# disanda/Deep-GAN-Encoders

Measured on AMD Instinct MI355X. Metric: encoder-train images/sec (E_align_s2 step, StyleGAN2 FFHQ-1024), higher is better.
Workload: dtype bf16; 1 GPU; E_align_s2 two-phase step, StyleGAN2-1024 G (train mode) + BE(startf=16, L=9) + LPIPS-VGG16 (seeded stand-in weights), batch 8/GPU; global_batch=8, img_size=1024, parallelism=dp1

## Files before the change

### deep-gan-encoders_amd/_lib.py

```python
import ctypes as C
import os

_HERE = os.path.dirname(os.path.abspath(__file__))
LIB_PATH = os.environ.get("DGE_LIB_PATH", os.path.join(_HERE, "libdge_hip.so"))


class DgeError(RuntimeError):
    pass


class ConvDesc(C.Structure):
    _fields_ = [
        ("x", C.c_void_p), ("w_packed", C.c_void_p), ("y", C.c_void_p), ("addend", C.c_void_p), ("dot_src", C.c_void_p),
        ("in_scale", C.c_void_p), ("in_shift", C.c_void_p), ("out_scale", C.c_void_p),
        ("bias", C.c_void_p), ("noise", C.c_void_p), ("noise_w", C.c_void_p), ("stats", C.c_void_p),
        ("B", C.c_int), ("H", C.c_int), ("W", C.c_int), ("Cin", C.c_int), ("Cout", C.c_int),
        ("ksize", C.c_int), ("up", C.c_int), ("in_s2d", C.c_int), ("noise_batch", C.c_int), ("noise_w_per_channel", C.c_int),
        ("act", C.c_int), ("bias_scale", C.c_float), ("gain", C.c_float), ("add_scale", C.c_float),
        ("dtype", C.c_int), ("in_up2", C.c_int), ("in_relu", C.c_int), ("stats_slots", C.c_int), ("w_layout", C.c_int),
        ("prep", C.c_int), ("prep_gain", C.c_float), ("prep_noise", C.c_void_p), ("prep_ns", C.c_void_p), ("prep_noise_batch", C.c_int),
        ("prep_stats", C.c_void_p), ("mask_relu", C.c_int), ("in_t2d", C.c_int),
        ("rgb_w", C.c_void_p), ("rgb_style", C.c_void_p), ("rgb_bias", C.c_void_p), ("rgb_out", C.c_void_p), ("rgb_wscale", C.c_float),
        ("rgb_skip_y", C.c_int), ("pool_out", C.c_int), ("pool_mask", C.c_void_p),
        ("prefetch_w", C.c_void_p), ("prefetch_ntot", C.c_int), ("prefetch_cin", C.c_int), ("in_bwd_coef", C.c_void_p),
        ("in_bwd_extra", C.c_void_p), ("in_bwd_extra_scale", C.c_float), ("fr_img4", C.c_void_p), ("fr_out", C.c_void_p),
    ]


class ConvPPDesc(C.Structure):
    _fields_ = [
        ("x", C.c_void_p), ("w_pp", C.c_void_p), ("y", C.c_void_p), ("w_bstride", C.c_longlong),
        ("out_scale", C.c_void_p), ("bias", C.c_void_p), ("noise", C.c_void_p), ("noise_w", C.c_void_p),
        ("B", C.c_int), ("H", C.c_int), ("W", C.c_int), ("Cin", C.c_int), ("Cout", C.c_int),
        ("noise_batch", C.c_int), ("noise_w_per_channel", C.c_int), ("act", C.c_int), ("bias_scale", C.c_float), ("gain", C.c_float),
        ("dgrad", C.c_int), ("in_s2d", C.c_int), ("stats_slots", C.c_int), ("prep", C.c_int), ("prep_noise_batch", C.c_int), ("mask_relu", C.c_int),
        ("in_t2d", C.c_int), ("add_scale", C.c_float), ("prep_gain", C.c_float),
        ("dot_src", C.c_void_p), ("addend", C.c_void_p), ("stats", C.c_void_p), ("prep_stats", C.c_void_p), ("prep_noise", C.c_void_p), ("prep_ns", C.c_void_p),
    ]


class DenseLayer(C.Structure):
    _fields_ = [("w", C.c_void_p), ("bias", C.c_void_p), ("I", C.c_int), ("O", C.c_int), ("wscale", C.c_float), ("bscale", C.c_float),
                ("add", C.c_float), ("act", C.c_int), ("gain", C.c_float)]


class S2GradEntry(C.Structure):
    _fields_ = [("P", C.c_void_p), ("st", C.c_void_p), ("d", C.c_void_p), ("s", C.c_void_p), ("bias", C.c_void_p), ("wsq", C.c_void_p),
                ("gs", C.c_void_p), ("wstyle", C.c_void_p),
                ("nslot_p", C.c_int), ("nslot_s", C.c_int), ("in_c", C.c_int), ("out_c", C.c_int), ("row", C.c_int), ("bscale", C.c_float)]


class SumPlanarEntry(C.Structure):
    _fields_ = [("partial", C.c_void_p), ("out", C.c_void_p), ("nslot", C.c_int), ("C", C.c_int), ("NS", C.c_int), ("pad", C.c_int)]


_P, _I, _F = C.c_void_p, C.c_int, C.c_float
SIGNATURES = {
    "dge_conv2d": [C.POINTER(ConvDesc), _P],
    "dge_fir_t2d": [_P, _P, _P, _I, _I, _I, _I, _I, _P],
    "dge_s2_style_grads": [C.POINTER(S2GradEntry), _I, _P, _I, _I, _I, _F, _P],
    "dge_conv_small_supported": [_I, _I, _I, _I, _I, _I, _I, _I],
    "dge_torgb_bwd_prep": [_P, _P, _P, _P, _P, _P, _I, _P, _P, _P, _I, _I, _I, _F, _F, _I, _P],
    "dge_demod_bwd_prep": [_P, _I, _P, _P, _P, _I, _I, _F, _P],
    "dge_sum_slots": [_P, _P, _I, _I, _I, _P],
    "dge_sum_slots_planar": [_P, _P, _I, _I, _I, _P],
    "dge_set_deterministic": [_I],
    "dge_get_deterministic": [],
    "dge_packed_n": [_I],
    "dge_pack_conv_weight": [_P, _P, _I, _I, _I, _I, _I, _F, _P],
    "dge_pack_conv_weights_multi": [_P, _P, _I, _I, _P],
    "dge_pack_desc_bytes": [],
    "dge_weight_sumsq": [_P, _P, _I, _I, _I, _F, _P],
    "dge_linear": [_P, _I, _P, _P, _P, _I, _I, _I, _I, _F, _F, _F, _I, _F, _I, _P],
    "dge_pixelnorm": [_P, _P, _I, _I, _F, _P],
    "dge_truncation": [_P, _P, _P, _I, _I, _I, _F, _I, _I, _P],
    "dge_torgb": [_P, _P, _P, _P, _P, _P, _I, _I, _I, _I, _F, _I, _P],
    "dge_conv_rgb_supported": [_I, _I, _I, _I, _I, _I, _I],
    "dge_conv_in_bwd_supported": [_I, _I, _I, _I, _I, _I, _I],
    "dge_conv_in_bwd_fromrgb_supported": [_I, _I, _I, _I, _I, _I, _I],
    "dge_conv_in_bwd_x_supported": [_I, _I, _I, _I, _I, _I, _I],
    "dge_conv_pool_supported": [_I, _I, _I, _I, _I, _I, _I],
    "dge_rgb_upsample_add": [_P, _P, _I, _I, _I, _P],
    "dge_nchw_to_nhwc": [_P, _P, _I, _I, _I, _I, _I, _P],
    "dge_nhwc_to_nchw": [_P, _P, _I, _I, _I, _I, _P],
    "dge_fromrgb": [_P, _P, _P, _P, _P, _I, _I, _I, _I, _P],
    "dge_fromrgb2": [_P, _P, _P, _P, _P, _P, _I, _I, _I, _I, _P],
    "dge_stats_finalize": [_P, _P, _P, _P, _I, _I, _I, _F, _P],
    "dge_stats_finalize_slots": [_P, _I, _P, _P, _P, _I, _I, _I, _F, _P],
    "dge_blend": [_P, _P, _P, _P, _P, _P, _I, _I, _I, _I, _I, _F, _F, _I, _P],
    "dge_loss_reduce": [_P, _P, _P, _I, _I, _I, _I, _I, _I, _I, _I, _P],
    "dge_crop_pool": [_P, _P, _I, _I, _I, _I, _I, _I, _I, _I, _P],
    "dge_ssim_fwd": [_P, _P, _P, _P, _I, _I, _I, _P],
    "dge_ssim_box7": [_P, _P, _P, _I, _I, _I, _F, _F, _F, _P],
    "dge_ssim_bwd": [_P, _P, _P, _P, _I, _I, _I, _F, _I, _P],
    "dge_space_loss_finalize": [_P, _P, _P, _P, _F, _F, _I, _P],
    "dge_space_loss_bwd": [_P, _P, _P, _P, _P, _I, _I, _I, _I, _I, _I, _I, _I, _F, _F, _I, _P],
    "dge_axpy_scalar": [_P, _P, _P, C.c_long, _F, _I, _P],
    "dge_lreq_adam_multi": [_I, _P, _P, _P, _P, _P, _F, _F, _P, _P, _P],
    "dge_modconv_bwd_prep": [_P, _P, _P, _P, _P, _P, _I, _I, _I, _I, _F, _I, _P],
    "dge_demod_bwd": [_P, _P, _P, _P, _P, _I, _I, _F, _P],
    "dge_linear_t": [_P, _I, _I, _P, _P, _P, _I, _I, _I, _I, _I, _F, _I, _P],
    "dge_torgb_bwd": [_P, _P, _P, _P, _P, _P, _I, _I, _I, _F, _I, _P],
    "dge_up2_bwd": [_P, _P, _I, _I, _I, _P],
    "dge_conv_wgrad": [_P, _P, _P, _P, _P, _I, _I, _I, _I, _I, _I, _I, _P],
    "dge_act_bwd": [_P, _P, _P, _P, _P, _I, _I, _I, _I, _I, _I, _F, _F, _I, _P],
    "dge_in_bwd_coef": [_P, _P, _P, _P, _P, _P, _I, _I, _I, _P],
    "dge_in_bwd_coef_slots": [_P, _I, _P, _P, _P, _P, _P, _I, _I, _I, _P],
    "dge_in_bwd": [_P, _P, _P, _P, _P, _P, _P, _I, _I, _I, _I, _I, _F, _I, _I, _P],
    "dge_chan_sum": [_P, _P, _I, _I, _I, _F, _I, _P],
    "dge_fromrgb_bwd": [_P, _P, _P, _P, _I, _I, _I, _I, _P],
    "dge_head_entry_size": [],
    "dge_heads_bwd": [_P, _I, _I, _P, _I, _P, _P, _P, _P, _I, _I, _P],
    "dge_dense_wgrad": [_P, _I, _P, _I, _P, _P, _I, _I, _I, _I, _P],
    "dge_lpips_prep": [_P, _P, _I, _I, _I, _P, _P, _I, _P],
    "dge_lpips_prep_bwd": [_P, _P, _I, _I, _I, _P, _F, _I, _I, _P],
    "dge_maxpool2": [_P, _P, _I, _I, _I, _I, _I, _P],
    "dge_maxpool2_bwd": [_P, _P, _P, _P, _I, _I, _I, _I, _I, _P],
    "dge_lpips_head": [_P, _P, _P, _P, _I, _I, _I, _F, _I, _P],
    "dge_mean": [_P, _P, _I, _P],
    "dge_blur_noise_act": [_P, _P, _P, _P, _P, _P, _I, _I, _I, _I, _I, _I, _I, _I, _P],
    "dge_affine_compose": [_P, _P, _P, _P, _P, _I, _I, _P],
    "dge_lerp_layers": [_P, _P, _I, _P, _P, _I, _I, _I, _P],
    "dge_linear_rows": [_P, _I, _P, _P, _P, _P, _P, _P, _I, _I, _I, _F, _F, _F, _P],
    "dge_demod_rows": [_P, _P, _P, _P, _P, _P, _P, _P, _I, _I, _F, _P],
    "dge_fromrgb_dgrad": [_P, _P, _P, _P, _I, _I, _I, _I, _P],
    "dge_nearest_up2": [_P, _P, _I, _I, _I, _I, _F, _I, _P],
    "dge_sg1_in_bwd_coef": [_P, _P, _P, _P, _P, _P, _I, _I, _I, _P],
    "dge_dot_stats": [_P, _P, _P, _I, _I, _I, _I, _P],
    "dge_nearest_up2_bwd": [_P, _P, _P, _P, _I, _I, _I, _I, _I, _P],
    "dge_pixelnorm_nhwc": [_P, _P, C.c_long, _I, _F, _I, _P],
    "dge_pixelnorm_nhwc_bwd": [_P, _P, _P, C.c_long, _I, _F, _I, _P],
    "dge_affine_relu_bwd": [_P, _P, _P, _P, _P, _P, _I, _I, _I, _I, _P],
    "dge_slice_up_bwd": [_P, _P, _I, _I, _I, _I, _I, _I, _I, _P],
    "dge_softmax_rows": [_P, C.c_long, _I, _I, _P],
    "dge_softmax_rows_bwd": [_P, _P, C.c_long, _I, _I, _P],
    "dge_rgb_tanh_bwd": [_P, _P, _P, _I, _I, _I, _I, _P],
    "dge_sn_group": [_P, _I, _I, _I, _P, _F, _I, _P],
    "dge_sn_entry_size": [],
    "dge_cbn_sn_wgrad_entry_size": [],
    "dge_cbn_sn_wgrad_group": [_P, _I, C.c_longlong, _I, _P, _I, _I, _P, _P],
    "dge_upconv_supported": [_I, _I, _I],
    "dge_pack_upconv_weight": [_P, _P, _I, _I, _F, _I, _P],
    "dge_upconv_fir": [_P, _P, _P, _P, _P, _P, _I, _P, _I, _P, _F, _F, _I, _I, _I, _I, _I, _I, _I, _P],
    "dge_cbn_affine": [_P, _P, _I, _P, _P, _F, _P, _P, _I, _I, _P],
    "dge_slice_up": [_P, _P, _I, _I, _I, _I, _I, _I, _I, _P],
    "dge_attention": [_P, _P, _P, _P, _I, _I, _I, _I, _I, _I, _P],
    "dge_rgb_tanh": [_P, _P, _I, _I, _I, _I, _P],
    "dge_guided_relu_bwd": [_P, _P, _P, C.c_long, _I, _I, _P],
    "dge_maxpool2_relu_bwd": [_P, _P, _P, _I, _I, _I, _I, _I, _I, _P],
    "dge_maxpool2_bwd_relu": [_P, _P, _P, _P, _I, _I, _I, _I, _I, _P],
    "dge_adaptive_pool7": [_P, _P, _I, _I, _I, _I, _I, _P],
    "dge_adaptive_pool7_bwd": [_P, _P, _I, _I, _I, _I, _I, _P],
    "dge_class_target": [_P, _P, _P, _P, _I, _I, _P],
    "dge_gather_row": [_P, _P, _P, _I, _I, _F, _P],
    "dge_campp_map": [_P, _P, _P, _P, _P, _I, _I, _I, _I, _I, _P],
    "dge_cam_resize": [_P, _P, _P, _I, _I, _I, _I, _I, _P],
    "dge_mask2cam_blocks": [_I],
    "dge_mask2cam": [_P, _P, _P, _P, _P, _P, _P, _I, _I, _P],
    "dge_randn": [_P, _I, _P, _P, _P, _P, C.c_ulonglong, _P, _P],
    "dge_version": [],
# ... 59 lines not shown
```

### deep-gan-encoders_amd/autograd_s2.py

```python
import math

import torch

from . import ops
from .stylegan2_generator import _dt
from .weight_cache import lookup, store, version


def _layer_fwd(L, x, w_row, randomize_noise):
    dt = ops.dtype_of(x)
    packed, wsq = L._prepared(dt)
    s = L.style(w_row)
    d = ops.linear(s, wsq, None, 1.0, 1.0, L.eps, ops.LIN_RSQRT, 1.0, square_input=True)
    if randomize_noise:
        noise = ops.randn((x.shape[0], L.res, L.res), x.device)
    else:
        noise = L.noise.reshape(1, L.res, L.res)
    y = ops.conv2d(x, packed, L.out_c, 3, up=L.up, in_scale=s, out_scale=d, bias=L.bias, bias_scale=L.bscale,
                   noise=noise, noise_w=L.noise_strength.detach().reshape(1), act=L.act, gain=L.gain)
    return y, s, d, noise


def _style_tables(mod, B, dt):
    nl = mod.num_layers
    groups = [(getattr(mod, f"layer{i}"), i) for i in range(nl - 1)] + [(getattr(mod, f"output{k}"), 2 * k + 1) for k in range(nl // 2)]
    key = (B, str(dt)) + tuple(version(p) for L, _ in groups for p in (L.style.weight, L.style.bias, L.weight))
    hit = mod.__dict__.get("_style_tab")
    if hit is not None and hit[0] == key:
        return hit[1]
    dev = groups[0][0].weight.device
    K = mod.w_space_dim
    Wc = torch.cat([L.style.weight.detach() for L, _ in groups]).contiguous()
    bc = torch.cat([L.style.bias.detach() for L, _ in groups]).contiguous()
    xoff, ybase, ybs, s_off = [], [], [], []
    off = 0
    for L, row in groups:
        C = L.in_c
        s_off.append(B * off)
        xoff += [row * K] * C
        ybase += [B * off + c for c in range(C)]
        ybs += [C] * C
        off += C
    woff, sbase, cin, dbase, dbs, d_off, wsq = [], [], [], [], [], [], []
    doff, wpos = 0, 0
    for gi, (L, _) in enumerate(groups[:nl - 1]):
        _, wq = L._prepared(dt)
        wsq.append(wq.reshape(-1))
        d_off.append(B * doff)
        for o in range(L.out_c):
            woff.append(wpos + o * L.in_c); sbase.append(s_off[gi]); cin.append(L.in_c)
            dbase.append(B * doff + o); dbs.append(L.out_c)
        doff += L.out_c
        wpos += L.out_c * L.in_c
    i32 = lambda v: torch.tensor(v, dtype=torch.int32, device=dev)
    st0 = groups[0][0].style
    for L, _ in groups:
        assert L.style.wscale == st0.wscale and L.style.bscale == st0.bscale and L.style.additional_bias == st0.additional_bias
    tab = dict(groups=groups, Wc=Wc, bc=bc, xoff=i32(xoff), ybase=i32(ybase), ybs=i32(ybs), s_off=s_off, s_total=B * off,
               wsq=torch.cat(wsq).contiguous(), woff=i32(woff), sbase=i32(sbase), cin=i32(cin), dbase=i32(dbase), dbs=i32(dbs),
               d_off=d_off, d_total=B * doff, wscale=st0.wscale, bscale=st0.bscale, add=st0.additional_bias, eps=groups[0][0].eps)
    mod.__dict__["_style_tab"] = (key, tab)
    return tab


def synthesis_run(mod, wp, randomize_noise=False, save=False):
    dt = _dt(mod.compute_dtype)
    B = wp.shape[0]
    results = {"wp": wp}
    nl = mod.num_layers
    tab = _style_tables(mod, B, dt)
    wpc = wp if (wp.dtype == torch.float32 and wp.is_contiguous()) else wp.float().contiguous()
    s_all = torch.empty(tab["s_total"], dtype=torch.float32, device=wp.device)
    ops.linear_rows(wpc, nl * mod.w_space_dim, tab["xoff"], tab["Wc"], tab["bc"], s_all, tab["ybase"], tab["ybs"], B,
                    tab["wscale"], tab["bscale"], tab["add"])
    d_all = torch.empty(tab["d_total"], dtype=torch.float32, device=wp.device)
    ops.demod_rows(s_all, tab["wsq"], tab["woff"], tab["sbase"], tab["cin"], d_all, tab["dbase"], tab["dbs"], B, tab["eps"])
    s_of = lambda g, C: s_all[tab["s_off"][g]:tab["s_off"][g] + B * C].view(B, C)
    x = ops.nchw_to_nhwc(mod.early_layer.const.detach(), B, dt)
    saved = {"const": x, "layers": [], "rgb": []} if save else None
    image = None
    for i in range(nl - 1):
        L = getattr(mod, f"layer{i}")
        s = s_of(i, L.in_c)
        d = d_all[tab["d_off"][i]:tab["d_off"][i] + B * L.out_c].view(B, L.out_c)
        if randomize_noise:
            noise = ops.randn((x.shape[0], L.res, L.res), x.device)
        else:
            noise = L.noise.reshape(1, L.res, L.res)
        fuse_rgb = (i % 2 == 0 and image is not None and not L.up and L.bias is not None and
                    ops.conv_rgb_supported(B, L.res, L.res, L.in_c, L.out_c, 3, dt))
        rgb = None
        if fuse_rgb:
            O_ = getattr(mod, f"output{i // 2}")
            srgb = s_of(nl - 1 + i // 2, O_.in_c)
            rgb = dict(w=O_.weight.detach().reshape(3, -1), style=srgb, bias=O_.bias.detach(), wscale=O_.wscale,
                       out=torch.empty((B, 3, L.res, L.res), dtype=torch.float32, device=x.device), skip_y=(not save) and i == nl - 2)
        y = L.conv(x, s, d, noise, dt, rgb=rgb)
        results[f"style{i:02d}"] = s
        if save:
            saved["layers"].append(dict(y=y, s=s, d=d, noise=noise))
        x = y
        if fuse_rgb:
            image = ops.rgb_upsample_add(rgb["out"], image)
            results[f"output_style{i // 2}"] = srgb
            if save:
                saved["rgb"].append(dict(s=srgb))
        elif i % 2 == 0:
            O_ = getattr(mod, f"output{i // 2}")
            srgb = s_of(nl - 1 + i // 2, O_.in_c)
            image = ops.torgb(x, O_.weight, srgb, O_.bias, image, O_.wscale)
            results[f"output_style{i // 2}"] = srgb
            if save:
                saved["rgb"].append(dict(s=srgb))
    results["image"] = image
    return results, saved


def _up_phase_form(L):
    import os
    return L.up and 32 <= L.res // 2 <= 128 and L.in_c >= 64 and L.in_c % 32 == 0 and L.out_c % 8 == 0 and not os.environ.get("DGE_NO_T2D")


def _dgrad_weight(L, dtype):
    hg = L.res // 2 if L.up else L.res
    if _up_phase_form(L):
        mode = ops.PACK_UPT2D_DGRAD
    else:
        mode = ops.pack_mode_for(L.weight, ops.PACK_UPFOLD_DGRAD if L.up else ops.PACK_DGRAD, hg, hg, dtype)
    c = lookup(L._cache, ("dg", dtype, mode), L.weight)
    return c if c is not None else store(L._cache, ("dg", dtype, mode), L.weight, ops.pack_conv_weight(L.weight, mode, dtype, L.wscale))


def _pp_dgrad(L, B, hg, dtype):
    import os
    K = 4 * L.out_c if L.up else L.out_c
    return (not L.up or L.out_c % 32 == 0) and ops.conv_pp_supported(B, hg, hg, K, L.in_c, dtype) and not os.environ.get("DGE_NO_PP_DG")


def _dgrad_weight_pp(L, d, t2d=False):
    if not L.up:
        return ops.pack_conv_pp(L.weight, L.wscale, in_scale=d, dgrad=True)
    name = "dgpp_t2d" if t2d else "dgpp"
    c = lookup(L._cache, name, L.weight)
    if c is None:
        rows = ops.pack_conv_weight(L.weight, ops.PACK_UPT2D_DGRAD if t2d else ops.PACK_UPFOLD_DGRAD, ops.F32, L.wscale)
        c = store(L._cache, name, L.weight, ops.pack_conv_pp_rows(rows, L.in_c, t2d=True) if t2d else rows)
    return c if t2d else ops.pack_conv_pp_rows(c, L.in_c, in_scale=d, in_period=L.out_c)


def synthesis_backward(mod, wp, saved, g_image):
    B = wp.shape[0]
    dev = wp.device
    nl = mod.num_layers
    g_wp = ops.zeros((B, nl, mod.w_space_dim), dev)
    layers = saved["layers"]
    dt = ops.dtype_of(saved["const"])
    g_img = g_image.float().contiguous()
    fused = not ops.is_deterministic()
    top = nl - 2
    Lt, Ot = getattr(mod, f"layer{top}"), getattr(mod, f"output{top // 2}")
    P = None
    if fused:
        g_x, g_srgb, P = ops.torgb_bwd_prep(g_img, layers[top]["y"], Ot.weight.detach().reshape(3, -1), saved["rgb"][top // 2]["s"], Ot.wscale,
                                            layers[top]["noise"], Lt.noise_strength.detach().reshape(1), Lt.gain)
    else:
        g_x, g_srgb = ops.torgb_bwd(g_img, layers[top]["y"], Ot.weight.detach().reshape(3, -1), saved["rgb"][top // 2]["s"], Ot.wscale)
    blocks = [] if fused else None
    if fused:
        blocks.append(dict(gs=g_srgb, wstyle=Ot.style.weight.detach(), row=top + 1))
    else:
        ops.linear_t(g_srgb, Ot.style.weight.detach(), g_wp[:, top + 1], scale=Ot.style.wscale, accumulate=True)
    if top // 2 > 0:
        g_img = ops.up2_bwd(g_img)
    for i in range(top, -1, -1):
        L = getattr(mod, f"layer{i}")
        rec = layers[i]
        if P is not None:
            g_y, d_in = g_x, rec["d"]
        else:
            R = ops.zeros((B, L.out_c, 3), dev)
            g_y, d_in = ops.modconv_bwd_prep(g_x, rec["y"], rec["d"], rec["noise"], L.gain, R), None
        x_in = saved["const"] if i == 0 else layers[i - 1]["y"]
        addend = None
        if i >= 1 and (i - 1) % 2 == 0:
            kp = (i - 1) // 2
            Op = getattr(mod, f"output{kp}")
            addend, g_srgb = ops.torgb_bwd(g_img, x_in, Op.weight.detach().reshape(3, -1), saved["rgb"][kp]["s"], Op.wscale)
            if fused:
                blocks.append(dict(gs=g_srgb, wstyle=Op.style.weight.detach(), row=i))
            else:
                ops.linear_t(g_srgb, Op.style.weight.detach(), g_wp[:, i], scale=Op.style.wscale, accumulate=True)
            if kp > 0:
                g_img = ops.up2_bwd(g_img)
        st = ops.SlotStats(B, L.in_c, dev) if fused else ops.zeros((B, L.in_c, 2), dev)
        prep, P_next = None, None
        t2d = _up_phase_form(L)
        if fused and i >= 1 and (t2d or not (L.up and L.in_c < 128)):
            Lp = getattr(mod, f"layer{i - 1}")
            P_next = ops.SlotStats(B, L.in_c, dev)
            prep = dict(gain=Lp.gain, noise=layers[i - 1]["noise"], ns=Lp.noise_strength.detach().reshape(1), stats=P_next)
        hg = L.res // 2 if L.up else L.res
        if fused and d_in is not None and not t2d and _pp_dgrad(L, B, hg, dt):
            g_xprev = ops.conv_pp(g_y, _dgrad_weight_pp(L, d_in), L.in_c, dgrad=True, in_s2d=L.up, out_scale=rec["s"], addend=addend,
                                  add_scale=1.0, stats=st, dot_src=x_in, prep=prep)
        elif t2d and fused and prep is not None and _pp_dgrad(L, B, hg, dt):
            g_xprev = ops.conv_pp(ops.fir_t2d(g_y, d_in), _dgrad_weight_pp(L, None, t2d=True), L.in_c, dgrad=True, in_t2d=True, out_scale=rec["s"],
                                  addend=addend, add_scale=1.0, stats=st, dot_src=x_in, prep=prep)
        elif t2d:
            g_xprev = ops.conv2d(ops.fir_t2d(g_y, d_in), _dgrad_weight(L, dt), L.in_c, 3, in_t2d=True, out_scale=rec["s"], addend=addend,
                                 add_scale=1.0, stats=st, dot_src=x_in, prep=prep)
        else:
            g_xprev = ops.conv2d(g_y, _dgrad_weight(L, dt), L.in_c, 3, in_s2d=L.up, in_scale=d_in, out_scale=rec["s"], addend=addend,
                                 add_scale=1.0, stats=st, dot_src=x_in, prep=prep)
        _, wsq = L._prepared(dt)
        if fused and P is not None:
            blocks.append(dict(P=P, st=st, d=rec["d"], s=rec["s"], bias=L.bias.detach(), wsq=wsq, bscale=L.bscale,
                               wstyle=L.style.weight.detach(), row=i))
            g_x, P = g_xprev, P_next
            continue
        if fused:
            st_t = ops.zeros((B, L.in_c, 2), dev)
            ops.check(ops.lib().dge_sum_slots(ops._p(st.buf), ops._p(st_t), st.nslot, st_t.numel(), 0, ops._stream()), "dge_sum_slots")
            st = st_t
        if P is not None:
            t = ops.demod_bwd_prep(P, rec["d"], L.bias.detach(), L.bscale)
        else:
            t = ops.demod_bwd(R, rec["d"], L.bias.detach(), L.noise_strength.detach().reshape(1), L.bscale)
        gs_view = st.view(B, -1)
        ops.linear_t(t, wsq, gs_view, mul=rec["s"], accumulate=True, incy=2, ldy=2 * L.in_c)
        ops.linear_t(gs_view, L.style.weight.detach(), g_wp[:, i], scale=L.style.wscale, accumulate=True, incx=2,
                     ldx=2 * L.in_c, O=L.in_c)
        g_x, P = g_xprev, P_next
    if blocks:
        ops.s2_style_grads(blocks, g_wp, getattr(mod, "layer0").style.wscale)
    return g_wp


class SynthesisFunction(torch.autograd.Function):
    @staticmethod
    def forward(ctx, mod, wp, randomize_noise):
        need = ctx.needs_input_grad[1]
        results, saved = synthesis_run(mod, wp.detach(), randomize_noise, save=need)
        ctx.mod, ctx.saved_acts, ctx.wp = mod, saved, wp.detach()
        ctx.keys = [k for k in results if k not in ("wp", "image")]
        outs = [results[k] for k in ctx.keys]
        ctx.mark_non_differentiable(*outs)
        return (results["image"], *outs)

    @staticmethod
    def backward(ctx, g_image, *unused):
        if ctx.saved_acts is None:
            raise RuntimeError("synthesis was run without saved activations")
        g_wp = synthesis_backward(ctx.mod, ctx.wp, ctx.saved_acts, g_image)
        return None, g_wp, None


def synthesis_forward(mod, wp, randomize_noise=False):
    wp = wp if (wp.dtype == torch.float32 and wp.is_contiguous()) else wp.float().contiguous()
    if wp.requires_grad and torch.is_grad_enabled():
        outs = SynthesisFunction.apply(mod, wp, randomize_noise)
        keys = [f"style{i:02d}" for i in range(mod.num_layers - 1)]
        results = {"wp": wp}
        names = []
        for i in range(mod.num_layers - 1):
            names.append(f"style{i:02d}")
            if i % 2 == 0:
                names.append(f"output_style{i // 2}")
        for n, t in zip(names, outs[1:]):
            results[n] = t
        results["image"] = outs[0]
        return results
    results, _ = synthesis_run(mod, wp, randomize_noise, save=False)
    return results
```

### deep-gan-encoders_amd/csrc/capi.hip

```cpp
#include <stdarg.h>
#include <stdio.h>
#include "common.h"
#include "conv_params.h"
#include "../../include/dge_hip.h"

static thread_local char g_err[512] = "";
void dge_set_error(const char* fmt, ...) {
    va_list ap; va_start(ap, fmt); vsnprintf(g_err, sizeof(g_err), fmt, ap); va_end(ap);
}
extern "C" const char* dge_last_error(void) { return g_err; }
static thread_local char g_kernel[160] = "";
void dge_note_kernel(const char* fmt, ...) {
    va_list ap; va_start(ap, fmt); vsnprintf(g_kernel, sizeof(g_kernel), fmt, ap); va_end(ap);
}
extern "C" const char* dge_last_kernel(void) { return g_kernel; }
extern "C" int dge_version(void) { return 100; }

#include <vector>
static std::vector<void (*)(const DgeDet*)>& det_setters() { static std::vector<void (*)(const DgeDet*)> v; return v; }
void dge_det_register(void (*setter)(const DgeDet*)) { det_setters().push_back(setter); }
static DgeDet g_det_host = {0, nullptr, nullptr, 0, 0};
int dge_det_upload_failed = 0;
bool dge_det_fits(long long ndomains, long long nslots, long long L) {
    return !g_det_host.enabled || (ndomains * nslots * L <= g_det_host.ws_floats && ndomains <= (long long)g_det_host.ncounters);
// ... 17 lines not shown
}
extern "C" int dge_get_deterministic(void) { return g_det_host.enabled; }

static DgeEnv g_env;
static bool g_env_loaded = false;
static int env_int(const char* name, int dflt) { const char* e = getenv(name); return e ? atoi(e) : dflt; }
static void env_load() {
    g_env.force_stream = getenv("DGE_FORCE_STREAM") ? 1 : 0;
    g_env.no_stream = getenv("DGE_NO_STREAM") ? 1 : 0;
    g_env.no_pw = getenv("DGE_NO_PW") ? 1 : 0;
    g_env.stream_nseg = env_int("DGE_STREAM_NSEG", 0);
    g_env.conv_dbg = env_int("DGE_CONV_DBG", 0);
    g_env.conv_bn = env_int("DGE_CONV_BN", 0);
    g_env.conv_kc = env_int("DGE_CONV_KC", 0);
    g_env.conv_small = env_int("DGE_CONV_SMALL", -1);
    g_env.conv_nok4 = getenv("DGE_CONV_NOK4") ? 1 : 0;
    g_env.conv_nok2 = getenv("DGE_CONV_NOK2") ? 1 : 0;
    g_env.torgb_thread = getenv("DGE_TORGB_THREAD") ? 1 : 0;
    g_env.wgrad_th8 = getenv("DGE_WGRAD_TH8") ? 1 : 0;
    g_env.wgrad_groups = env_int("DGE_WGRAD_GROUPS", 0);
    if (g_env.wgrad_groups < 0) g_env.wgrad_groups = 0;
    g_env.up_dbg = env_int("DGE_UP_DBG", 0);
    { const char* v = getenv("DGE_UP_VARIANT"); g_env.up_variant = !v ? 0 : (v[0] == 's' ? 2 : 1); }
    g_env_loaded = true;
}
#include <mutex>
static std::once_flag g_env_once;
const DgeEnv& dge_env() { std::call_once(g_env_once, [] { if (!g_env_loaded) env_load(); }); return g_env; }
extern "C" void dge_env_reload(void) { env_load(); }

extern "C" int dge_conv2d(const dge_conv_desc* d, hipStream_t s) {
    DGE_CHECK(d && d->x && d->w_packed && d->y, "conv2d: null tensor");
    DGE_CHECK(d->B > 0 && d->H > 0 && d->W > 0 && d->Cin > 0 && d->Cout > 0, "conv2d: bad shape");
    DGE_CHECK(d->dtype == DGE_F32 || d->dtype == DGE_BF16, "conv2d: bad dtype %d", d->dtype);
    DGE_CHECK(!(d->up && d->stats), "conv2d: stats are not available in up mode");
    DGE_CHECK(!(d->up && d->in_s2d), "conv2d: up and in_s2d are exclusive");
    DGE_CHECK(!d->in_up2 || (!d->in_s2d && d->H % 2 == 0 && d->W % 2 == 0), "conv2d: in_up2 needs even H, W and no in_s2d");
    DGE_CHECK(!d->in_s2d || d->Cin % 4 == 0, "conv2d: in_s2d needs Cin %% 4 == 0");
    DGE_CHECK(!d->dot_src || d->stats || d->mask_relu || d->in_bwd_coef, "conv2d: dot_src needs a stats buffer");
    DGE_CHECK(!d->mask_relu || (d->dot_src && !d->prep && !d->up), "conv2d: mask_relu needs dot_src and excludes prep / up");
    DGE_CHECK(!d->in_relu || d->in_scale || d->in_shift, "conv2d: in_relu is applied together with the prologue affine");
    DGE_CHECK(d->gain > 0.f, "conv2d: gain must be positive (it is folded through the activation)");
    DGE_CHECK((((uintptr_t)d->in_scale | (uintptr_t)d->in_shift) & 15) == 0, "conv2d: in_scale/in_shift must be 16-byte aligned");
    DGE_CHECK(!d->noise || d->noise_w, "conv2d: noise without noise_w");
    ConvParams p;
    p.x = d->x; p.w = d->w_packed; p.y = d->y; p.addend = d->addend; p.dot_src = d->dot_src;
    p.in_scale = d->in_scale; p.in_shift = d->in_shift; p.out_scale = d->out_scale;
    p.bias = d->bias; p.noise = d->noise; p.noise_w = d->noise_w; p.stats = d->stats;
    p.B = d->B; p.H = d->H; p.W = d->W; p.Cin = d->Cin; p.Cout = d->Cout;
    p.Ntot_valid = d->up ? 4 * d->Cout : d->Cout;
    p.Ntot = dge_packed_n(p.Ntot_valid);
    p.up = d->up; p.in_s2d = d->in_s2d; p.in_up2 = d->in_up2; p.in_relu = d->in_relu;
    const int OH = d->up ? 2 * d->H : d->H, OW = d->up ? 2 * d->W : d->W;
    p.noise_bstride = d->noise_batch > 1 ? OH * OW : 0;
    p.noise_w_stride = d->noise_w_per_channel ? 1 : 0;
    p.act = d->act; p.bias_scale = d->bias_scale; p.gain = d->gain; p.add_scale = d->add_scale;
    p.tiles_x = p.tiles_y = 0;
    p.w_frag = d->w_layout == 1 ? 1 : 0;
    p.prep = d->prep ? 1 : 0;
    p.mask_relu = d->mask_relu ? 1 : 0;
    p.in_t2d = d->in_t2d ? 1 : 0;
    DGE_CHECK(!d->in_t2d || (d->ksize == 3 && !d->up && !d->in_s2d && !d->in_up2 && !d->in_scale && !d->in_shift && d->w_layout == 0),
              "conv2d: in_t2d is a plain 3x3 launch (no other read mode, no prologue affine, row-major weights)");
    p.prep_gain = d->prep_gain; p.prep_noise = d->prep_noise; p.prep_ns = d->prep_ns; p.prep_stats = d->prep_stats;
    p.prep_noise_bstride = d->prep_noise_batch > 1 ? OH * OW : 0;
    DGE_CHECK(!d->prep || (d->dot_src && d->prep_stats && d->prep_gain > 0.f && !d->up), "conv2d: prep needs dot_src, prep_stats, a positive prep_gain and no up mode");
    DGE_CHECK(!d->prep || !dge_get_deterministic(), "conv2d: the fused tail backward (prep) is not offered in deterministic mode; run dge_modconv_bwd_prep");
    DGE_CHECK(d->w_layout == 0 || d->w_layout == 1, "conv2d: bad w_layout %d", d->w_layout);
    p.stats_slots = d->stats_slots > 0 ? d->stats_slots : 1;
    p.rgb_w = d->rgb_out ? d->rgb_w : nullptr; p.rgb_style = d->rgb_style; p.rgb_bias = d->rgb_bias; p.rgb_out = d->rgb_out;
    p.rgb_wscale = d->rgb_wscale; p.rgb_skip_y = (d->rgb_out && d->rgb_skip_y) ? 1 : 0;
    p.pool_out = d->pool_out ? 1 : 0; p.pool_mask = d->pool_out ? (unsigned*)d->pool_mask : nullptr;
    const bool pf = d->w_layout == 1 && d->prefetch_w && d->prefetch_ntot >= 64 && d->prefetch_ntot % 64 == 0 &&
                    (d->prefetch_cin == 512 || d->prefetch_cin == 256);
    p.pf_w = pf ? d->prefetch_w : nullptr; p.pf_ntot = pf ? d->prefetch_ntot : 0; p.pf_cin = pf ? d->prefetch_cin : 0;
    p.in_coef = d->in_bwd_coef;
    p.in_extra = d->in_bwd_coef ? d->in_bwd_extra : nullptr; p.in_extra_scale = d->in_bwd_extra_scale;
    p.fr_img4 = d->in_bwd_coef ? d->fr_img4 : nullptr; p.fr_out = d->in_bwd_coef ? d->fr_out : nullptr;
    if (d->in_bwd_coef) {
        DGE_CHECK(!dge_get_deterministic(), "conv2d: in_bwd_coef is not offered in deterministic mode; run dge_in_bwd");
        DGE_CHECK(d->ksize == 3 && !d->up && dge_conv_stream_eligible(p, d->dtype, d->ksize), "conv2d: in_bwd_coef is offered where "
                  "dge_conv_in_bwd_supported() says so, with dot_src and prep_stats, without stats / prep");
    }
    if (d->pool_out)
        DGE_CHECK(!d->up && dge_conv_pool_ok(p, d->dtype, d->ksize), "conv2d: the pooled epilogue is offered where dge_conv_pool_supported() "
                  "says so (conv_2 of the first encoder blocks on the streaming kernel)");
    if (d->rgb_out) {
        DGE_CHECK(d->rgb_w && d->rgb_style && d->rgb_bias, "conv2d: rgb_out needs rgb_w, rgb_style, rgb_bias");
        DGE_CHECK(dge_conv_rgb_ok(p, d->dtype, d->ksize), "conv2d: the fused toRGB is offered where dge_conv_rgb_supported() says so "
                  "(bf16 3x3 32 -> 32 launches of the streaming kernel)");
    }
    return dge_conv_launch(p, d->dtype, d->ksize, s);
}

extern "C" int dge_conv_pool_supported(int B, int H, int W, int Cin, int Cout, int ksize, int dtype) {
    ConvParams p = {};
    p.B = B; p.H = H; p.W = W; p.Cin = Cin; p.Cout = Cout; p.Ntot_valid = Cout; p.Ntot = dge_packed_n(Cout);
    p.in_shift = (const float*)16; p.noise_w_stride = 1;
    return dge_conv_pool_ok(p, dtype, ksize) ? 1 : 0;
}

extern "C" int dge_conv_in_bwd_supported(int B, int H, int W, int Cin, int Cout, int ksize, int dtype) {
    ConvParams p = {};
    p.B = B; p.H = H; p.W = W; p.Cin = Cin; p.Cout = Cout; p.Ntot_valid = Cout; p.Ntot = dge_packed_n(Cout);
    p.dot_src = (const void*)16; p.prep_stats = (float*)16; p.in_coef = (const float*)16;
    return (ksize == 3 && !dge_get_deterministic() && dge_conv_stream_eligible(p, dtype, ksize)) ? 1 : 0;
}
extern "C" int dge_conv_in_bwd_x_supported(int B, int H, int W, int Cin, int Cout, int ksize, int dtype) {
    ConvParams p = {};
    p.B = B; p.H = H; p.W = W; p.Cin = Cin; p.Cout = Cout; p.Ntot_valid = Cout; p.Ntot = dge_packed_n(Cout);
    p.dot_src = (const void*)16; p.in_coef = (const float*)16;
    return (ksize == 3 && !dge_get_deterministic() && dge_conv_stream_eligible(p, dtype, ksize)) ? 1 : 0;
}
extern "C" int dge_conv_in_bwd_fromrgb_supported(int B, int H, int W, int Cin, int Cout, int ksize, int dtype) {
    ConvParams p = {};
    p.B = B; p.H = H; p.W = W; p.Cin = Cin; p.Cout = Cout; p.Ntot_valid = Cout; p.Ntot = dge_packed_n(Cout);
    p.dot_src = (const void*)16; p.in_coef = (const float*)16; p.fr_img4 = (const float*)16; p.fr_out = (float*)16;
    return (ksize == 3 && !dge_get_deterministic() && dge_conv_stream_eligible(p, dtype, ksize)) ? 1 : 0;
}

extern "C" int dge_conv_rgb_supported(int B, int H, int W, int Cin, int Cout, int ksize, int dtype) {
    ConvParams p = {};
    p.B = B; p.H = H; p.W = W; p.Cin = Cin; p.Cout = Cout; p.Ntot_valid = Cout; p.Ntot = dge_packed_n(Cout);
    return dge_conv_rgb_ok(p, dtype, ksize) ? 1 : 0;
}

__global__ void sum_slots_kernel(const float* __restrict__ partial, float* __restrict__ out, int nslot, int n, int accumulate) {
    const int i = blockIdx.x * blockDim.x + threadIdx.x;
    if (i >= n) return;
    float s = 0.f;
    int k = 0;
    for (; k + 8 <= nslot; k += 8) {
        float v[8];
#pragma unroll
        for (int j = 0; j < 8; j++) v[j] = partial[(size_t)(k + j) * n + i];
#pragma unroll
        for (int j = 0; j < 8; j++) s += v[j];
    }
    for (; k < nslot; k++) s += partial[(size_t)k * n + i];
    out[i] = accumulate ? out[i] + s : s;
}
__global__ void sum_slots_planar_kernel(const float* __restrict__ partial, float* __restrict__ out, int nslot, int C, int NS) {
    const int i = blockIdx.x * blockDim.x + threadIdx.x;
    if (i >= C * NS) return;
    float s = 0.f;
    int k = 0;
    for (; k + 8 <= nslot; k += 8) {
        float v[8];
#pragma unroll
        for (int j = 0; j < 8; j++) v[j] = partial[(size_t)(k + j) * C * NS + i];
#pragma unroll
        for (int j = 0; j < 8; j++) s += v[j];
    }
    for (; k < nslot; k++) s += partial[(size_t)k * C * NS + i];
    out[(size_t)(i % NS) * C + i / NS] = s;
}
extern "C" int dge_sum_slots_planar(const float* partial, float* out, int nslot, int C, int NS, hipStream_t s) {
    DGE_CHECK(nslot >= 1 && C >= 1 && NS >= 1, "sum_slots_planar: bad sizes");
    hipLaunchKernelGGL(sum_slots_planar_kernel, dim3((C * NS + 255) / 256), dim3(256), 0, s, partial, out, nslot, C, NS);
    DGE_LAUNCH_CHECK("sum_slots_planar");
    return 0;
}
struct SumPlanarTable { dge_sum_planar_entry e[32]; };
__global__ void sum_slots_planar_multi_kernel(SumPlanarTable tab) {
    const dge_sum_planar_entry e = tab.e[blockIdx.y];
    const int n = e.C * e.NS;
    for (int i = blockIdx.x * blockDim.x + threadIdx.x; i < n; i += gridDim.x * blockDim.x) {
        float s = 0.f;
        int k = 0;
        for (; k + 8 <= e.nslot; k += 8) {
            float v[8];
#pragma unroll
            for (int j = 0; j < 8; j++) v[j] = e.partial[(size_t)(k + j) * n + i];
#pragma unroll
            for (int j = 0; j < 8; j++) s += v[j];
        }
        for (; k < e.nslot; k++) s += e.partial[(size_t)k * n + i];
        e.out[(size_t)(i % e.NS) * e.C + i / e.NS] = s;
    }
}
extern "C" int dge_sum_slots_planar_multi(const dge_sum_planar_entry* entries, int n, hipStream_t s) {
    DGE_CHECK(entries && n >= 1 && n <= 32, "sum_slots_planar_multi: 1..32 entries");
    SumPlanarTable tab;
    int maxn = 1;
    for (int i = 0; i < n; i++) {
        const dge_sum_planar_entry& e = entries[i];
        DGE_CHECK(e.partial && e.out && e.nslot >= 1 && e.C >= 1 && e.NS >= 1, "sum_slots_planar_multi: bad entry %d", i);
        tab.e[i] = e;
        if (e.C * e.NS > maxn) maxn = e.C * e.NS;
    }
    hipLaunchKernelGGL(sum_slots_planar_multi_kernel, dim3((maxn + 255) / 256, n), dim3(256), 0, s, tab);
    DGE_LAUNCH_CHECK("sum_slots_planar_multi");
    return 0;
}
extern "C" int dge_sum_slots(const float* partial, float* out, int nslot, int n, int accumulate, hipStream_t s) {
    hipLaunchKernelGGL(sum_slots_kernel, dim3((n + 255) / 256), dim3(256), 0, s, partial, out, nslot, n, accumulate);
    DGE_LAUNCH_CHECK("sum_slots");
    return 0;
}
```

### deep-gan-encoders_amd/csrc/common.h

```cpp
#pragma once
#include <hip/hip_runtime.h>
#include <stdint.h>

typedef uint16_t bf16_t;
typedef __attribute__((ext_vector_type(8))) __bf16 bf16x8_t;
typedef __attribute__((ext_vector_type(16))) float f32x16_t;
typedef __attribute__((ext_vector_type(4))) float f32x4_t;

enum { DGE_F32 = 0, DGE_BF16 = 1 };
enum { DGE_ACT_NONE = 0, DGE_ACT_LRELU = 1, DGE_ACT_RELU = 2 };

__device__ __forceinline__ float bf2f(bf16_t h) { return __uint_as_float(((uint32_t)h) << 16); }
__device__ __forceinline__ bf16_t f2bf(float f) {
    uint32_t u = __float_as_uint(f);
    if ((u & 0x7fffffffu) > 0x7f800000u) return (bf16_t)((u >> 16) | 0x40);
    u += 0x7fffu + ((u >> 16) & 1u);
    return (bf16_t)(u >> 16);
}
typedef __attribute__((ext_vector_type(2))) __bf16 bf16x2_t;
typedef __attribute__((ext_vector_type(2))) float f32x2_t;
__device__ __forceinline__ uint32_t pack2bf(float lo, float hi) {
#ifdef DGE_SOFT_BF16
    return (uint32_t)f2bf(lo) | ((uint32_t)f2bf(hi) << 16);
#endif
    f32x2_t v = {lo, hi};
    bf16x2_t h = __builtin_convertvector(v, bf16x2_t);
    return *(uint32_t*)&h;
}

#include <type_traits>
template <int N, int I = 0> struct StaticFor {
    template <class F> __device__ static __forceinline__ void run(F&& f) { f(std::integral_constant<int, I>{}); StaticFor<N, I + 1>::run(f); }
};
template <int N> struct StaticFor<N, N> { template <class F> __device__ static __forceinline__ void run(F&&) {} };

template <typename T> struct Elem;
template <> struct Elem<float> {
    static constexpr int PER16 = 4;
    __device__ static float ld(const float* p) { return *p; }
    __device__ static void st(float* p, float v) { *p = v; }
};
template <> struct Elem<bf16_t> {
    static constexpr int PER16 = 8;
    __device__ static float ld(const bf16_t* p) { return bf2f(*p); }
    __device__ static void st(bf16_t* p, float v) { *p = f2bf(v); }
};

__device__ __forceinline__ void unpack16(const uint4& v, float (&f)[4], float*) {
    f[0] = __uint_as_float(v.x); f[1] = __uint_as_float(v.y); f[2] = __uint_as_float(v.z); f[3] = __uint_as_float(v.w);
}
__device__ __forceinline__ void unpack16(const uint4& v, float (&f)[8], bf16_t*) {
    f[0] = __uint_as_float(v.x << 16); f[1] = __uint_as_float(v.x & 0xffff0000u);
    f[2] = __uint_as_float(v.y << 16); f[3] = __uint_as_float(v.y & 0xffff0000u);
    f[4] = __uint_as_float(v.z << 16); f[5] = __uint_as_float(v.z & 0xffff0000u);
    f[6] = __uint_as_float(v.w << 16); f[7] = __uint_as_float(v.w & 0xffff0000u);
}
__device__ __forceinline__ uint4 pack16(const float (&f)[4], float*) {
    return make_uint4(__float_as_uint(f[0]), __float_as_uint(f[1]), __float_as_uint(f[2]), __float_as_uint(f[3]));
}
__device__ __forceinline__ uint4 pack16(const float (&f)[8], bf16_t*) {
    return make_uint4(pack2bf(f[0], f[1]), pack2bf(f[2], f[3]), pack2bf(f[4], f[5]), pack2bf(f[6], f[7]));
}

__device__ __forceinline__ float act_apply(float v, int act) {
    if (act == DGE_ACT_LRELU) return v > 0.f ? v : 0.2f * v;
    if (act == DGE_ACT_RELU) return v > 0.f ? v : 0.f;
    return v;
}

__device__ __forceinline__ float wave_sum(float v) {
#pragma unroll
    for (int o = 32; o > 0; o >>= 1) v += __shfl_xor(v, o, 64);
    return v;
}

struct DgeDet {
    int enabled;
    float* ws;
    unsigned* counters;
    long long ws_floats;
    int ncounters;
};
static __device__ DgeDet g_det = {0, nullptr, nullptr, 0, 0};
void dge_det_register(void (*setter)(const DgeDet*));
extern int dge_det_upload_failed;
bool dge_det_fits(long long ndomains, long long nslots, long long L);
static void dge_det_set_this_tu(const DgeDet* v) {
    if (hipMemcpyToSymbol(HIP_SYMBOL(g_det), v, sizeof(DgeDet), 0, hipMemcpyHostToDevice) != hipSuccess) dge_det_upload_failed = 1;
}
namespace { struct DgeDetReg { DgeDetReg() { dge_det_register(&dge_det_set_this_tu); } }; static DgeDetReg dge_det_reg_instance; }

__device__ __forceinline__ bool det_on() { return g_det.enabled != 0; }
__device__ __forceinline__ float* det_slot(int domain, int ndomains, int slot, int nslots, int L) {
    if ((long long)ndomains * nslots * L > g_det.ws_floats || ndomains > g_det.ncounters) __builtin_trap();
    return g_det.ws + ((size_t)domain * nslots + slot) * L;
}
__device__ __forceinline__ bool det_arrive_wg(int domain, int arrivals) {
    __shared__ int s_last;
    asm volatile("s_waitcnt vmcnt(0)" ::: "memory");
    __syncthreads();
    if (threadIdx.x == 0) {
        __builtin_amdgcn_fence(__ATOMIC_RELEASE, "agent");
        asm volatile("s_waitcnt vmcnt(0)" ::: "memory");
        const unsigned t = atomicAdd(&g_det.counters[domain], 1u);
        const int last = (t == (unsigned)(arrivals - 1));
        if (last) { __builtin_amdgcn_fence(__ATOMIC_ACQUIRE, "agent"); g_det.counters[domain] = 0u; }
        s_last = last;
    }
    __syncthreads();
    return s_last != 0;
}
__device__ __forceinline__ bool det_arrive_wave(int domain, int arrivals) {
    int last = 0;
// ... 107 lines not shown
```

### deep-gan-encoders_amd/csrc/conv_params.h

```cpp
#pragma once
#include <hip/hip_runtime.h>

struct ConvParams {
    const void* x;
    const void* w;
    void* y;
    const void* addend;
    const void* dot_src;
    const float* in_scale;
    const float* in_shift;
    const float* out_scale;
    const float* bias;
    const float* noise;
    const float* noise_w;
    float* stats;
    int stats_slots;
    int B, H, W, Cin, Cout;
    int Ntot;
    int Ntot_valid;
    int up;
    int in_s2d;
    int in_relu;
    int in_up2;
    int noise_bstride;
    int noise_w_stride;
    int act;
    float bias_scale, gain, add_scale;
    int tiles_x, tiles_y;
    int dbg;
    int w_frag;
    int prep;
    float prep_gain;
    const float* prep_noise;
    const float* prep_ns;
    int prep_noise_bstride;
    float* prep_stats;
    int mask_relu;
    int in_t2d;
    const float* rgb_w;
    const float* rgb_style;
    const float* rgb_bias;
    float* rgb_out;
    float rgb_wscale;
    int rgb_skip_y;
    int pool_out;
    unsigned* pool_mask;
    const void* pf_w;
    int pf_ntot, pf_cin;
    const float* in_coef;
    const void* in_extra; float in_extra_scale; const float* fr_img4; float* fr_out;
};

int dge_conv_launch(const ConvParams& p, int dtype, int ksize, hipStream_t s);
extern "C" int dge_conv_ntile(int ntot);

bool dge_conv_stream_eligible(const ConvParams& p, int dtype, int ksize);
int dge_conv_stream_launch(const ConvParams& p, hipStream_t s);
bool dge_conv_rgb_ok(const ConvParams& p, int dtype, int ksize);
bool dge_conv_pool_ok(const ConvParams& p, int dtype, int ksize);
bool dge_conv_small_shape_ok(int H, int W, int cin, int ntot, int ksize, int in_s2d, int in_up2, int dtype);
int dge_conv_small_launch(const ConvParams& p, hipStream_t s);
bool dge_conv_pw_eligible(const ConvParams& p, int dtype, int ksize);
int dge_conv_pw_launch(const ConvParams& p, hipStream_t s);
```

### deep-gan-encoders_amd/csrc/conv_stream.hip

```cpp
#include <type_traits>
#include "common.h"
#include <stdlib.h>
#include "conv_params.h"

namespace {

typedef __attribute__((ext_vector_type(4))) unsigned rsrc_t;
#define DGE_LDS " lds\n\t"

__device__ __forceinline__ unsigned rfl(unsigned v) { return __builtin_amdgcn_readfirstlane(v); }
__device__ __forceinline__ unsigned lds_off(const void* p) {
    return (unsigned)(size_t)(const __attribute__((address_space(3))) unsigned char*)p;
}
constexpr int ilog2(int v) { return v <= 1 ? 0 : 1 + ilog2(v >> 1); }

__device__ __forceinline__ rsrc_t make_rsrc(unsigned long long base, unsigned bytes) {
    rsrc_t r;
    r[0] = rfl((unsigned)base); r[1] = rfl((unsigned)(base >> 32) & 0xffffu); r[2] = rfl(bytes); r[3] = 0x00020000u;
    return r;
}

#define DGE_P(off) "buffer_load_dwordx4 %1, %3, 0 offen offset:" #off " lds\n\t"
#define DGE_PB(off) "buffer_load_dwordx4 %4, %3, 0 offen offset:" #off " lds\n\t"
#define DGE_M0 "s_mov_b32 m0, %2\n\ts_nop 0\n\t"
#define DGE_MASK(m) "s_mov_b64 %0, exec\n\ts_mov_b64 exec, " #m "\n\t"
#define DGE_UNMASK "s_mov_b64 exec, %0"
template <int CIN, int TEAM>
__device__ __forceinline__ void dma_row(int wave, unsigned voff, unsigned voff_b, unsigned voff_c, rsrc_t rs, rsrc_t rs_null,
                                        unsigned m0v, unsigned m0_dummy) {
    unsigned long long keep;
    if constexpr (CIN == 16 && TEAM == 1) {
        asm volatile(DGE_M0 DGE_P(0) DGE_MASK(0xf) DGE_P(1024) DGE_UNMASK : "=&s"(keep) : "v"(voff), "s"(m0v), "s"(rs) : "memory");
    } else if constexpr (CIN == 16 && TEAM == 2) {
        if (wave == 0) asm volatile(DGE_M0 DGE_P(0) : "=&s"(keep) : "v"(voff), "s"(m0v), "s"(rs) : "memory");
        else asm volatile(DGE_M0 DGE_MASK(0xf) DGE_P(1024) DGE_UNMASK : "=&s"(keep) : "v"(voff), "s"(m0v), "s"(rs) : "memory");
    } else if constexpr (CIN == 32 && TEAM == 1) {
        asm volatile(DGE_M0 DGE_P(0) DGE_P(1024) DGE_MASK(0xff) DGE_P(2048) DGE_UNMASK : "=&s"(keep) : "v"(voff), "s"(m0v), "s"(rs) : "memory");
    } else if constexpr (CIN == 32 && TEAM == 2) {
        if (wave == 0) asm volatile(DGE_M0 DGE_P(0) DGE_MASK(0xff) DGE_P(2048) DGE_UNMASK : "=&s"(keep) : "v"(voff), "s"(m0v), "s"(rs) : "memory");
        else asm volatile(DGE_M0 DGE_P(1024) "s_mov_b32 m0, %5\n\ts_nop 0\n\tbuffer_load_dwordx4 %1, %4, 0 offen lds"
                          : "=&s"(keep) : "v"(voff), "s"(m0v), "s"(rs), "s"(rs_null), "s"(m0_dummy) : "memory");
    } else if constexpr (CIN == 64 && TEAM == 1) {
        asm volatile(DGE_M0 DGE_P(0) DGE_PB(1024) DGE_P(2048) DGE_PB(3072)
                     "s_mov_b32 m0, %6\n\t" DGE_MASK(0xffff) "buffer_load_dwordx4 %5, %3, 0 offen lds\n\t" DGE_UNMASK
                     : "=&s"(keep) : "v"(voff), "s"(m0v), "s"(rs), "v"(voff_b), "v"(voff_c), "s"(m0v + 4096u) : "memory");
    } else {
        if (wave == 0)
            asm volatile(DGE_M0 DGE_P(0) DGE_P(2048)
                         "s_mov_b32 m0, %5\n\t" DGE_MASK(0xffff) "buffer_load_dwordx4 %4, %3, 0 offen lds\n\t" DGE_UNMASK
                         : "=&s"(keep) : "v"(voff), "s"(m0v), "s"(rs), "v"(voff_c), "s"(m0v + 4096u) : "memory");
        else
            asm volatile(DGE_M0 DGE_P(1024) DGE_P(3072) "s_mov_b32 m0, %5\n\ts_nop 0\n\tbuffer_load_dwordx4 %1, %4, 0 offen lds"
                         : "=&s"(keep) : "v"(voff_b), "s"(m0v), "s"(rs), "s"(rs_null), "s"(m0_dummy) : "memory");
    }
}
__device__ __forceinline__ void dma_piece(unsigned voff, rsrc_t rs, unsigned m0v) {
    asm volatile("s_mov_b32 m0, %1\n\ts_nop 0\n\tbuffer_load_dwordx4 %0, %2, 0 offen lds" : : "v"(voff), "s"(m0v), "s"(rs) : "memory");
}
template <int NP> __device__ __forceinline__ void dma_dot(unsigned voff, unsigned voff1, rsrc_t rs, unsigned m0v) {
    if constexpr (NP == 1)
        asm volatile("s_mov_b32 m0, %1\n\ts_nop 0\n\tbuffer_load_dwordx4 %0, %2, 0 offen lds" : : "v"(voff), "s"(m0v), "s"(rs) : "memory");
    else
        asm volatile("s_mov_b32 m0, %1\n\ts_nop 0\n\tbuffer_load_dwordx4 %0, %2, 0 offen lds\n\t"
                     "buffer_load_dwordx4 %3, %2, 0 offen offset:1024 lds" : : "v"(voff), "s"(m0v), "s"(rs), "v"(voff1) : "memory");
}

enum { FL_GEN = 0, FL_ENC = 1, FL_ENC_STATS = 2, FL_DOT = 3, FL_DOT_PREP = 4, FL_GEN_RGB = 5, FL_ENC_POOL = 6, FL_DOT_IN = 7, FL_DOT_FR = 8, FL_DOT_INX = 9 };

template <int CIN, int COUT, int FL>
struct SC {
    static constexpr int PXB = CIN * 2, CH = PXB / 16, LOGCH = ilog2(CH), KS = CIN / 16;
    static constexpr int TEAM = COUT == 64 ? 2 : 1;
    static constexpr int TPW = 4 / TEAM;
    static constexpr int MT = COUT / 32 > 0 ? COUT / 32 : 1;
    static constexpr int MTW = MT / TEAM;
    static constexpr int HW = 34, RB = HW * PXB;
    static constexpr int PIECES = (RB + 1023) / 1024;
    static constexpr bool PREP = FL == FL_DOT_PREP, RGB = FL == FL_GEN_RGB, POOL = FL == FL_ENC_POOL, FRB = FL == FL_DOT_FR, INX = FL == FL_DOT_INX, INB = FL == FL_DOT_IN || FRB || INX;
    static_assert(!RGB || COUT == 32 || (COUT == 64 && TEAM == 2), "fused toRGB: 32 output channels per wave, one wave or a 2-wave team per pixel");
    static constexpr bool DOT = FL == FL_DOT || PREP || INB, STATS = FL == FL_ENC_STATS, ENC = FL == FL_ENC || FL == FL_ENC_STATS || POOL;
    static constexpr bool NOISE = !DOT || PREP || (INB && !FRB && !INX);
    static constexpr int NR = 6;
    static constexpr int dot_depth(int nr) { for (int d = 4; d >= 1; d--) if (d <= nr - 3 && nr % (d + 1) == 0) return d; return 1; }
    static constexpr int D = DOT ? dot_depth(6) : 2;
    static constexpr int DR = DOT ? D + 1 : NR;
    static_assert(NR % DR == 0, "dot ring period");
    static constexpr int CPB = COUT * 2;
    static constexpr int CW = COUT / TEAM >= 32 ? 32 : 16;
    static constexpr int DCH = CW * MTW * 2 / 16;
    static constexpr int LOGDCH = ilog2(DCH);
    static constexpr int DROWB = 32 * DCH * 16, DPIECES = DROWB / 1024;
    static_assert(!DOT || MTW == 1, "data-gradient mode: one M tile per wave");
    static constexpr int XPW = TEAM == 2 ? (PIECES + 1) / 2 : PIECES;
    static constexpr int LPR = XPW + (DOT ? DPIECES : 0) + (FRB ? 2 : 0) + (INX ? 1 : 0);
    static constexpr int X_OFF = 0;
    static constexpr int XRING = NR * RB;
    static constexpr int N_OFF = (XRING + 1023) / 1024 * 1024;
    static constexpr int NRING = NOISE ? 2048 : 0;
    static_assert(NR <= 8, "a noise piece holds 8 rows");
    static constexpr int D_OFF = N_OFF + TEAM * NRING;
    static constexpr int DRING = DOT ? DR * DROWB : 0;
    static constexpr int E_OFF = D_OFF + TEAM * DRING;
    static constexpr int ERING = FRB ? 2 * DR * 512 : (INX ? DR * 1024 : 0);
    static_assert(!INX || (CIN == COUT && CIN >= 32), "block-input flavour: 32 -> 32, 64 -> 64");
    static_assert(!FRB || (CIN == 16 && COUT == 16 && TEAM == 1), "FromRGB reduction flavour: 16 -> 16");
    static constexpr int T_OFF = E_OFF + TEAM * ERING;
    static constexpr int TBYTES = 32 * MTW * 16 * 4;
    static constexpr int DUMMY_OFF = T_OFF + TEAM * TBYTES;
    static constexpr int RGBX_OFF = DUMMY_OFF + (TEAM == 2 ? 1024 : 0);
    static constexpr int LDS_BYTES = RGBX_OFF + (RGB && TEAM == 2 ? 1024 : 0);
    static constexpr int NEED = 4 * 9 * KS * MTW + 32 * MTW + 16 + (ENC ? 16 * MTW : 0) + (STATS || DOT ? 32 * MTW : 0) + (DOT ? 16 : 0) + (PREP ? 16 : 0) + (RGB ? 11 : 0) + (POOL ? 20 * MTW : 0) + 36;
    static constexpr int WPE = ((PREP || INB) && CIN == 64) ? 1 : (NEED <= 128 ? 4 : (NEED <= 168 ? 3 : 2));
    static_assert(D <= NR - 3, "the slot of the row being fetched must be dead");
    static_assert((D - 1) * LPR + 1 < 64, "vmcnt range");
};

template <int LOGC> __device__ __forceinline__ int chunk_swz(int px) { return (px >> (4 - LOGC)) & ((1 << LOGC) - 1); }

template <int CW> __device__ __forceinline__ int chan_of_row(int m) {
    const int j = m >> 3, k = (m >> 2) & 1, i = m & 3;
    if (CW == 16) return j < 2 ? 8 * k + 4 * j + i : -1;
    return 16 * (j >> 1) + 8 * k + 4 * (j & 1) + i;
}

template <int CIN, int COUT, int FL>
__global__ __launch_bounds__((64 * SC<CIN, COUT, FL>::TEAM * SC<CIN, COUT, FL>::TPW), (SC<CIN, COUT, FL>::WPE))
void conv_stream_kernel(ConvParams p, int nstrips, int nseg, int seg_rows, int njobs, int jobs_per_xcd) {
    using C = SC<CIN, COUT, FL>;
    extern __shared__ __attribute__((aligned(1024))) unsigned char lds_all[];
#ifdef DGE_SC_TIMING
    const long long tj0 = __builtin_readcyclecounter();
#endif
    const int lane = threadIdx.x & 63;
    const int wid = (int)rfl(threadIdx.x >> 6);
    const int team = wid / C::TEAM;
    const int wave = wid % C::TEAM;
    unsigned char* __restrict__ lds = lds_all + team * C::LDS_BYTES;
    const unsigned lds0 = lds_off(lds_all) + team * C::LDS_BYTES;
    const int n31 = lane & 31, kh = lane >> 5;

    int job = ((blockIdx.x & 7) * jobs_per_xcd + (blockIdx.x >> 3)) * C::TPW + team;
    if ((blockIdx.x >> 3) >= jobs_per_xcd || job >= njobs) return;
    const int strip = job % nstrips; job /= nstrips;
    const int seg = job % nseg;
    const int b = job / nseg;
    const int x0 = strip * 32;
    const int r0 = seg * seg_rows;
    const int rows = min(seg_rows, p.H - r0);
    const bool full_strip = x0 + 32 <= p.W;
    const bool edge_strip = x0 == 0 || x0 + 32 >= p.W;

    const unsigned xrow_bytes = (unsigned)p.W * C::PXB, yrow_bytes = (unsigned)p.W * C::CPB;
    const unsigned long long Xb = (unsigned long long)p.x + (unsigned long long)b * p.H * xrow_bytes;
    unsigned char* __restrict__ Yb = (unsigned char*)p.y + (size_t)b * p.H * yrow_bytes;
    const float* __restrict__ nzsrc = (C::PREP || C::INB) ? p.prep_noise : p.noise;
    const unsigned long long NZb = nzsrc ? (unsigned long long)(nzsrc + (size_t)b * ((C::PREP || C::INB) ? p.prep_noise_bstride : p.noise_bstride)) : Xb;
    const unsigned nzrow_bytes = nzsrc ? (unsigned)p.W * 4 : 0;
    const unsigned long long DOTb = C::DOT ? (unsigned long long)p.dot_src + (unsigned long long)b * p.H * yrow_bytes : Xb;

    unsigned voff, voff_b = 0, voff_c = 0;
    {
        const int px = lane >> C::LOGCH, cs = lane & (C::CH - 1);
        const int gx = x0 - 1 + px;
        voff = (unsigned)(gx * C::PXB + ((cs ^ chunk_swz<C::LOGCH>(px)) << 4));
        if constexpr (CIN == 64) {
            voff_b = (unsigned)(gx * C::PXB + ((cs ^ chunk_swz<C::LOGCH>(px + 8)) << 4));
            voff_c = voff + 4096;
        }
    }
    const unsigned nvoff = (unsigned)(((lane >> 3) * p.W + x0 + (lane & 7) * 4) * 4);
    unsigned dvoff = 0, dvoff1 = 0;
    if constexpr (C::DOT) {
        const int px = lane >> C::LOGDCH, cs = lane & (C::DCH - 1);
        const int chunk0 = wave * 4;
        dvoff = (unsigned)((x0 + px) * C::CPB + ((chunk0 + (cs ^ chunk_swz<C::LOGDCH>(px))) << 4));
        constexpr int PPP = 64 / C::DCH;
        dvoff1 = (unsigned)((x0 + px + PPP) * C::CPB + ((chunk0 + (cs ^ chunk_swz<C::LOGDCH>(px + PPP))) << 4)) - 1024u;
    }
    const rsrc_t rs_null = make_rsrc(Xb, 0);
    const unsigned exrow_bytes = (C::FRB || C::INX) ? (unsigned)(p.W >> 1) * C::CPB : 0u, imrow_bytes = C::FRB ? (unsigned)p.W * 16u : 0u;
    const unsigned long long EXb = ((C::FRB || C::INX) && p.in_extra) ? (unsigned long long)p.in_extra + (unsigned long long)b * (p.H >> 1) * exrow_bytes : Xb;
    const unsigned long long IMb = C::FRB ? (unsigned long long)p.fr_img4 + (unsigned long long)b * p.H * imrow_bytes : Xb;
    const unsigned evoff = C::INX ? (unsigned)(((x0 >> 1) + (lane >> 2)) * C::CPB + wave * 64 + (((lane & 3) ^ chunk_swz<2>(lane >> 2)) << 4))
                                  : (unsigned)((x0 >> 1) * 32 + (lane & 31) * 16);
    const unsigned ivoff = (unsigned)((x0 + (lane & 31)) * 16);

    unsigned long long xptr = Xb + (unsigned long long)(long long)(r0 - 1) * xrow_bytes;
    unsigned long long dptr = DOTb + (unsigned long long)(long long)(r0 - 2) * yrow_bytes;
    auto issue = [&](int h, int slot, int slot_d) {
        const int gy = r0 - 1 + h;
        const bool xv = (unsigned)gy < (unsigned)p.H && h <= rows + 1;
        const rsrc_t rx = make_rsrc(xptr, xv ? xrow_bytes : 0u);
        xptr += xrow_bytes;
        const unsigned m0x = lds0 + C::X_OFF + slot * C::RB;
        dma_row<CIN, C::TEAM>(wave, voff, voff_b, voff_c, rx, rs_null, m0x, lds0 + C::DUMMY_OFF);
        const bool ov = h >= 2 && h <= rows + 1;
        if constexpr (C::DOT) {
            const rsrc_t rd = make_rsrc(dptr, ov ? yrow_bytes : 0u);
            dptr += yrow_bytes;
            dma_dot<C::DPIECES>(dvoff, dvoff1, rd, lds0 + C::D_OFF + wave * C::DRING + slot_d * C::DROWB);
        }
        if constexpr (C::INX) {
            const int oy = gy - 1;
            const rsrc_t re = make_rsrc(EXb + (unsigned long long)(ov ? (oy >> 1) : 0) * exrow_bytes, (ov && p.in_extra) ? exrow_bytes : 0u);
            dma_piece(evoff, re, lds0 + C::E_OFF + wave * C::ERING + slot_d * 1024);
        }
        if constexpr (C::FRB) {
            const int oy = gy - 1;
            const rsrc_t re = make_rsrc(EXb + (unsigned long long)(ov ? (oy >> 1) : 0) * exrow_bytes, (ov && p.in_extra) ? exrow_bytes : 0u);
            const rsrc_t ri = make_rsrc(IMb + (unsigned long long)(ov ? oy : 0) * imrow_bytes, ov ? imrow_bytes : 0u);
            unsigned long long keep;
            asm volatile(DGE_MASK(0xffffffff) "s_mov_b32 m0, %2\n\ts_nop 0\n\tbuffer_load_dwordx4 %1, %3, 0 offen lds\n\t"
                         "s_mov_b32 m0, %4\n\ts_nop 0\n\tbuffer_load_dwordx4 %5, %6, 0 offen lds\n\t" DGE_UNMASK
                         : "=&s"(keep) : "v"(evoff), "s"(lds0 + C::E_OFF + slot_d * 512), "s"(re), "s"(lds0 + C::E_OFF + C::DR * 512 + slot_d * 512), "v"(ivoff), "s"(ri) : "memory");
        }
    };
    auto issue_noise = [&](int q, unsigned buf_off) {
        const int gy = r0 + q;
        const bool v = nzsrc != nullptr && gy < p.H && q < rows;
        const rsrc_t rn = make_rsrc(NZb + (unsigned long long)(v ? gy : 0) * nzrow_bytes, v ? (unsigned)(p.H - gy) * nzrow_bytes : 0u);
        dma_piece(nvoff, rn, lds0 + C::N_OFF + wave * C::NRING + buf_off);
    };
    asm volatile("s_waitcnt vmcnt(0)" ::: "memory");
    if constexpr (C::NOISE) issue_noise(0, 0u);
    StaticFor<C::D + 2>::run([&](auto hc) { constexpr int h = decltype(hc)::value; issue(h, h % C::NR, (h + C::NR - 2) % C::NR % C::DR); });

    uint4 wf[C::MTW][9][C::KS];
    float* __restrict__ TT = (float*)(lds + C::T_OFF + wave * C::TBYTES);
    {
        const bf16_t* __restrict__ Wp = (const bf16_t*)p.w;
        float sc[C::KS][8], rt[C::KS][8];
#pragma unroll
        for (int ks = 0; ks < C::KS; ks++) {
            const int k0 = ks * 16 + kh * 8;
#pragma unroll
            for (int e = 0; e < 8; e++) {
                sc[ks][e] = p.in_scale ? p.in_scale[b * CIN + k0 + e] : 1.f;
                const float sh = (C::ENC && p.in_shift) ? p.in_shift[b * CIN + k0 + e] : 0.f;
                rt[ks][e] = sc[ks][e] != 0.f ? sh / sc[ks][e] : 0.f;
            }
        }
#pragma unroll
        for (int mt = 0; mt < C::MTW; mt++) {
            const int cl = chan_of_row<C::CW>(n31);
            const int o = (wave * C::MTW + mt) * 32 + cl;
            const bool ov = cl >= 0 && o < COUT;
            float osc = p.gain;
            if (!C::DOT && p.out_scale && ov) osc *= p.out_scale[b * COUT + o];
            if (C::INB && ov) osc *= p.in_coef[((size_t)b * COUT + o) * 3];
            const int oc = ov ? o : 0;
            float c_bias = (!C::DOT && p.bias) ? p.bias[oc] : 0.f;
            float c_nw = (C::NOISE && p.noise) ? p.noise_w[oc * p.noise_w_stride] : 0.f;
            float c_osc = (C::DOT && !C::INB && p.out_scale) ? p.out_scale[b * COUT + oc] : 1.f;
            float c_in1 = 0.f, c_in2 = 0.f;
            if constexpr (C::INB) { c_in1 = p.in_coef[((size_t)b * COUT + oc) * 3 + 1]; c_in2 = p.in_coef[((size_t)b * COUT + oc) * 3 + 2]; }
            float tall = 0.f, tleft = 0.f, tright = 0.f;
            {
                const bf16_t* __restrict__ wrow = Wp + (size_t)(ov ? o : 0) * CIN + kh * 8;
#pragma unroll
                for (int tap = 0; tap < 9; tap++)
#pragma unroll
                    for (int ks = 0; ks < C::KS; ks++) wf[mt][tap][ks] = *(const uint4*)(wrow + (size_t)tap * p.Ntot * CIN + ks * 16);
            }
#pragma unroll
            for (int tap = 0; tap < 9; tap++) {
                float tt = 0.f;
#pragma unroll
                for (int ks = 0; ks < C::KS; ks++) {
                    uint4 v = ov ? wf[mt][tap][ks] : make_uint4(0, 0, 0, 0);
                    float f[8];
                    unpack16(v, f, (bf16_t*)nullptr);
#pragma unroll
                    for (int e = 0; e < 8; e++) f[e] *= sc[ks][e] * osc;
                    v = pack16(f, (bf16_t*)nullptr);
                    if constexpr (C::ENC) {
                        unpack16(v, f, (bf16_t*)nullptr);
#pragma unroll
                        for (int e = 0; e < 8; e++) tt += f[e] * rt[ks][e];
                    }
                    wf[mt][tap][ks] = v;
                }
                if constexpr (C::ENC) {
                    tt += __shfl_xor(tt, 32, 64);
// ... 40 lines not shown
    const float slope = p.act == DGE_ACT_LRELU ? 0.2f : (p.act == DGE_ACT_RELU ? 0.f : 1.f);

    uint4 rgbA[C::RGB ? 2 : 1];
    float rgbb[3] = {0.f, 0.f, 0.f};
    if constexpr (C::RGB) {
        const int row = n31 & 7, part = n31 >> 3;
        const bool live = row < 3 && part < 2;
#pragma unroll
        for (int ks = 0; ks < 2; ks++) {
            float f[8];
#pragma unroll
            for (int e = 0; e < 8; e++) {
                const int c = wave * 32 + 16 * ks + 8 * kh + e;
                const float wv = live ? p.rgb_w[row * COUT + c] * p.rgb_wscale * p.rgb_style[b * COUT + c] : 0.f;
                const float hi = __uint_as_float(__float_as_uint(wv) & 0xffff0000u);
                f[e] = part == 0 ? hi : wv - hi;
            }
            rgbA[ks] = pack16(f, (bf16_t*)nullptr);
        }
#pragma unroll
        for (int k = 0; k < 3; k++) rgbb[k] = wave == 0 ? p.rgb_bias[k] : 0.f;
    }
    float rgbh[3] = {0.f, 0.f, 0.f};
    typedef __attribute__((address_space(3))) float* lds_wfp;
    auto rgb_flush = [&](int srow) {
        if (kh == 0 && x0 + n31 < p.W) {
            const unsigned a = lds0 + C::RGBX_OFF + (unsigned)(srow & 1) * 384 + n31 * 4;
            float* __restrict__ ro = p.rgb_out + ((size_t)b * 3 * p.H + (r0 + srow)) * p.W + x0 + n31;
            const size_t plane = (size_t)p.H * p.W;
#pragma unroll
            for (int k = 0; k < 3; k++) ro[k * plane] = rgbh[k] + *(const __attribute__((address_space(3))) float*)(a + k * 128);
        }
    };

    unsigned loff[3][C::KS];
#pragma unroll
    for (int dx = 0; dx < 3; dx++)
#pragma unroll
        for (int ks = 0; ks < C::KS; ks++) {
            const int px = n31 + dx;
            loff[dx][ks] = lds0 + C::X_OFF + px * C::PXB + (((ks * 2 + kh) ^ chunk_swz<C::LOGCH>(px)) << 4);
        }
    const unsigned nzoff = lds0 + C::N_OFF + wave * C::NRING + n31 * 4;
    unsigned doff[2] = {0, 0};
    if constexpr (C::DOT) {
#pragma unroll
        for (int q = 0; q < 2; q++)
            doff[q] = lds0 + C::D_OFF + wave * C::DRING + n31 * C::DCH * 16 + (((2 * q + kh) ^ chunk_swz<C::LOGDCH>(n31)) << 4);
    }
    typedef unsigned u32x4_t __attribute__((ext_vector_type(4)));
    typedef const __attribute__((address_space(3))) u32x4_t* lds_u4p;
    typedef const __attribute__((address_space(3))) float* lds_fp;
    auto lds_u4 = [&](unsigned a) { const u32x4_t t = *(lds_u4p)a; return make_uint4(t[0], t[1], t[2], t[3]); };
    auto lds_f = [&](unsigned a) { return *(lds_fp)a; };

    const int gx = x0 + n31;
    const bool pv = gx < p.W;
    const unsigned yoff = (unsigned)gx * C::CPB + (unsigned)(wave * C::MTW * 32 * 2) + kh * 16;
    const bool pool_lane = C::POOL && (n31 & 1) == 0 && pv;
    const unsigned py_voff = pool_lane ? (unsigned)(gx >> 1) * C::CPB + (unsigned)(wave * C::MTW * 64) + kh * 16 : 0x80000000u;
    const unsigned pm_voff = pool_lane ? ((unsigned)(gx >> 1) * (COUT / 8) + (unsigned)(wave * C::MTW * 4) + kh) * 4u : 0x80000000u;
    const unsigned pool_px = C::POOL ? (unsigned)(p.H >> 1) * (unsigned)(p.W >> 1) : 0u;
    const __amdgpu_buffer_rsrc_t rs_pool = __builtin_amdgcn_make_buffer_rsrc((unsigned char*)p.y + (size_t)b * pool_px * C::CPB, 0, (int)(pool_px * C::CPB), 0x00020000);
    const __amdgpu_buffer_rsrc_t rs_mask = __builtin_amdgcn_make_buffer_rsrc((C::POOL && p.pool_mask) ? (unsigned char*)p.pool_mask + (size_t)b * pool_px * (COUT / 8) * 4 : (unsigned char*)p.y, 0,
                                                                               (C::POOL && p.pool_mask) ? (int)(pool_px * (COUT / 8) * 4) : 0, 0x00020000);

    float s0[C::MTW][(C::STATS || C::DOT) ? 16 : 1], s1[C::MTW][(C::STATS || C::DOT) ? 16 : 1], s2[(C::PREP || C::INB) ? 16 : 1];
    if constexpr (C::STATS || C::DOT) {
#pragma unroll
        for (int mt = 0; mt < C::MTW; mt++)
#pragma unroll
            for (int r = 0; r < 16; r++) { s0[mt][r] = 0.f; s1[mt][r] = 0.f; }
    }
    if constexpr (C::PREP || C::INB) {
#pragma unroll
        for (int r = 0; r < 16; r++) s2[r] = 0.f;
    }
    float prow[C::POOL ? C::MTW : 1][C::POOL ? 16 : 1];
    unsigned psign[C::POOL ? C::MTW : 1];
    const float pg_pos = p.prep_gain, pg_neg = 0.2f * p.prep_gain, pz_pos = 1.f / p.prep_gain, pz_neg = 1.f / (0.2f * p.prep_gain);
    const float pns = (C::PREP && p.prep_noise && p.prep_ns) ? p.prep_ns[0] : 0.f;
    const float fr_es = (C::FRB || C::INX) ? p.in_extra_scale : 0.f;

#define DGE_T(k)
    auto step = [&](auto ic, int s, unsigned npar) {
        constexpr int I = decltype(ic)::value;
        DGE_T(0);
        constexpr int NAFTER = (C::D - 1) * C::LPR + ((C::NOISE && I >= 1 && I <= C::D - 1) ? 1 : 0);
        asm volatile("s_waitcnt vmcnt(%0)" :: "i"(NAFTER) : "memory");
        if constexpr (C::RGB && C::TEAM == 2) asm volatile("s_waitcnt lgkmcnt(0)" ::: "memory");
        if constexpr (C::TEAM == 2) __builtin_amdgcn_s_barrier();
        if constexpr (C::RGB && C::TEAM == 2) { if (wave == 0 && s > 0) rgb_flush(s - 1); }
        DGE_T(1);
        if constexpr (C::NOISE && I == 0) issue_noise(s + C::NR, npar ^ 1024u);
        issue(s + 2 + C::D, (I + 2 + C::D) % C::NR, (I + C::D) % C::DR);
        DGE_T(2);

        const int gy = r0 + s;
        constexpr int NQ = 9 * C::KS;
        constexpr int PF = NQ < 6 ? NQ : 6;
        auto frag_addr = [&](auto qc) {
            constexpr int q = decltype(qc)::value;
            constexpr int tap = q / C::KS, ks = q % C::KS, dy = tap / 3, dx = tap % 3;
            return loff[dx][ks] + (unsigned)(((I + dy) % C::NR) * C::RB);
        };
        float nz = 0.f;
        if constexpr (C::NOISE) nz = lds_f(nzoff + npar + I * 128);
        uint4 bq[PF];
        StaticFor<PF>::run([&](auto qc) { bq[decltype(qc)::value] = lds_u4(frag_addr(qc)); });
        f32x16_t acc[C::MTW];
        StaticFor<NQ>::run([&](auto qc) {
            constexpr int q = decltype(qc)::value;
            constexpr int tap = q / C::KS, ks = q % C::KS;
            const bf16x8_t bf = *(const bf16x8_t*)&bq[q % PF];
#pragma unroll
            for (int mt = 0; mt < C::MTW; mt++) {
                acc[mt] = __builtin_amdgcn_mfma_f32_32x32x16_bf16(*(const bf16x8_t*)&wf[mt][tap][ks], bf, q == 0 ? ((C::DOT && !C::INB) ? zero16 : biasv[mt]) : acc[mt], 0, 0, 0);
            }
            if constexpr (q + PF < NQ) bq[q % PF] = lds_u4(frag_addr(std::integral_constant<int, q + PF>{}));
        });

        __builtin_amdgcn_sched_group_barrier(0x100, PF + (C::NOISE ? 1 : 0), 0);
        StaticFor<NQ - PF>::run([&](auto) {
            __builtin_amdgcn_sched_group_barrier(0x008, C::MTW, 0);
            __builtin_amdgcn_sched_group_barrier(0x100, 1, 0);
        });
        __builtin_amdgcn_sched_group_barrier(0x008, PF * C::MTW, 0);
        DGE_T(3);
        unsigned char* __restrict__ yrow = Yb + (size_t)gy * yrow_bytes;
#pragma unroll
        for (int mt = 0; mt < C::MTW; mt++) {
            float v[16];
#pragma unroll
            for (int r = 0; r < 16; r++) v[r] = acc[mt][r];
            if constexpr (C::ENC) {
                const bool top = gy == 0, bot = gy == p.H - 1;
                if (top | bot) {
                    const float cl = gx == 0 ? 1.f : 0.f, cr = gx == p.W - 1 ? 1.f : 0.f;
#pragma unroll
                    for (int r = 0; r < NREG; r++) {
                        const float* __restrict__ T = TT + chan_of_reg(mt, r) * 16;
                        float corr = 0.f;
                        if (top) corr += T[0] + T[1] + T[2] - cl * T[0] - cr * T[2];
                        if (bot) corr += T[6] + T[7] + T[8] - cl * T[6] - cr * T[8];
                        v[r] -= corr;
                    }
                }
            }
            if constexpr (C::DOT) {
                uint4 dd[2];
                dd[0] = lds_u4(doff[0] + (I % C::DR) * C::DROWB);
                if constexpr (NREG == 16) dd[1] = lds_u4(doff[1] + (I % C::DR) * C::DROWB);
                const float nzs = C::PREP ? pns * nz : 0.f;
                float exf[8], exx[C::INX ? 2 : 1][8];
                if constexpr (C::INX) {
#pragma unroll
                    for (int q = 0; q < NREG / 8; q++)
                        unpack16(lds_u4(lds0 + C::E_OFF + wave * C::ERING + (I % C::DR) * 1024 + (n31 >> 1) * 64 + (((2 * q + kh) ^ chunk_swz<2>(n31 >> 1)) << 4)), exx[q], (bf16_t*)nullptr);
                }
                float4 fr_im = make_float4(0.f, 0.f, 0.f, 0.f);
                if constexpr (C::FRB) {
                    unpack16(lds_u4(lds0 + C::E_OFF + (I % C::DR) * 512 + (n31 >> 1) * 32 + kh * 16), exf, (bf16_t*)nullptr);
                    const uint4 t4 = lds_u4(lds0 + C::E_OFF + C::DR * 512 + (I % C::DR) * 512 + n31 * 16);
                    fr_im = make_float4(__uint_as_float(t4.x), __uint_as_float(t4.y), __uint_as_float(t4.z), __uint_as_float(t4.w));
                }
#pragma unroll
                for (int q = 0; q < NREG / 8; q++) {
                    float d[8];
                    unpack16(dd[q], d, (bf16_t*)nullptr);
#pragma unroll
                    for (int e = 0; e < 8; e++) {
                        const int r = 8 * q + e;
                        if constexpr (C::INX) {
                            v[r] = fmaf(fr_es, exx[C::INX ? q : 0][e], fmaf(oscv[r], d[e], v[r]));
                            continue;
                        }
                        if constexpr (C::FRB) {
                            const float gp = (fmaf(oscv[r], d[e], v[r]) + fr_es * exf[e]) * (d[e] > 0.f ? 1.f : 0.2f);
// ... 29 lines not shown
                    v[r] = fmaxf(t, t * slope);
                }
                if constexpr (C::STATS) {
#pragma unroll
                    for (int r = 0; r < NREG; r++) { s0[mt][r] += v[r]; s1[mt][r] = fmaf(v[r], v[r], s1[mt][r]); }
                }
            }
            if constexpr (C::POOL) {
                unsigned sb = 0;
#pragma unroll
                for (int r = 0; r < NREG; r++) sb |= (v[r] > 0.f ? 1u : 0u) << r;
                static_assert(!C::POOL || C::NR % 2 == 0, "pooled flavour: even ring period");
                if constexpr ((I & 1) == 0) {
#pragma unroll
                    for (int r = 0; r < NREG; r++) prow[mt][r] = v[r];
                    psign[mt] = sb;
                    continue;
                }
#pragma unroll
                for (int r = 0; r < NREG; r++) {
                    const float cs = prow[mt][r] + v[r];
                    v[r] = 0.25f * (cs + __builtin_bit_cast(float, __builtin_amdgcn_mov_dpp(__builtin_bit_cast(unsigned, cs), 0xB1, 0xf, 0xf, true)));
                }
                const unsigned prow_i = (unsigned)(gy >> 1);
                if (p.pool_mask) {
                    const unsigned own = (psign[mt] & 0xffffu) | (sb << 16);
                    const unsigned nbr = __builtin_amdgcn_mov_dpp(own, 0xB1, 0xf, 0xf, true);
                    const unsigned msoff = prow_i * (unsigned)(p.W >> 1) * (unsigned)(COUT / 8) * 4u;
                    __builtin_amdgcn_raw_buffer_store_b32((own & 0xffu) | ((nbr & 0xffu) << 8) | (((own >> 16) & 0xffu) << 16) | (((nbr >> 16) & 0xffu) << 24),
                                                          rs_mask, pm_voff + (unsigned)mt * 16u, msoff, 0);
                    if constexpr (NREG == 16)
                        __builtin_amdgcn_raw_buffer_store_b32(((own >> 8) & 0xffu) | (((nbr >> 8) & 0xffu) << 8) | (((own >> 24) & 0xffu) << 16) | (((nbr >> 24) & 0xffu) << 24),
                                                              rs_mask, pm_voff + (unsigned)mt * 16u + 8u, msoff, 0);
                }
                {
                    const unsigned ysoff = prow_i * (unsigned)(p.W >> 1) * (unsigned)C::CPB;
                    u32x4_t q0, q1;
                    q0[0] = pack2bf(v[0], v[1]); q0[1] = pack2bf(v[2], v[3]); q0[2] = pack2bf(v[4], v[5]); q0[3] = pack2bf(v[6], v[7]);
                    __builtin_amdgcn_raw_buffer_store_b128(q0, rs_pool, py_voff + (unsigned)mt * 64u, ysoff, 0);
                    if constexpr (NREG == 16) {
                        q1[0] = pack2bf(v[8], v[9]); q1[1] = pack2bf(v[10], v[11]); q1[2] = pack2bf(v[12], v[13]); q1[3] = pack2bf(v[14], v[15]);
                        __builtin_amdgcn_raw_buffer_store_b128(q1, rs_pool, py_voff + (unsigned)mt * 64u + 32u, ysoff, 0);
                    }
                }
                continue;
            }
            if constexpr (C::FRB) continue;
            uint4 o0 = make_uint4(pack2bf(v[0], v[1]), pack2bf(v[2], v[3]), pack2bf(v[4], v[5]), pack2bf(v[6], v[7]));
            uint4 o1 = make_uint4(pack2bf(v[8], v[9]), pack2bf(v[10], v[11]), pack2bf(v[12], v[13]), pack2bf(v[14], v[15]));
            unsigned char* dst = yrow + yoff + mt * 64;
            if constexpr (C::RGB) {
                f32x16_t t = __builtin_amdgcn_mfma_f32_32x32x16_bf16(*(const bf16x8_t*)&rgbA[0], *(const bf16x8_t*)&o0, zero16, 0, 0, 0);
                t = __builtin_amdgcn_mfma_f32_32x32x16_bf16(*(const bf16x8_t*)&rgbA[1], *(const bf16x8_t*)&o1, t, 0, 0, 0);
                if constexpr (C::TEAM == 2) {
                    if (wave == 0) { rgbh[0] = t[0] + t[4] + rgbb[0]; rgbh[1] = t[1] + t[5] + rgbb[1]; rgbh[2] = t[2] + t[6] + rgbb[2]; }
                    else if (kh == 0) {
                        const unsigned a = lds0 + C::RGBX_OFF + (unsigned)(s & 1) * 384 + n31 * 4;
                        *(lds_wfp)(a) = t[0] + t[4]; *(lds_wfp)(a + 128) = t[1] + t[5]; *(lds_wfp)(a + 256) = t[2] + t[6];
                    }
                } else if (kh == 0 && pv) {
                    float* __restrict__ ro = p.rgb_out + ((size_t)b * 3 * p.H + gy) * p.W + gx;
                    const size_t plane = (size_t)p.H * p.W;
                    ro[0] = t[0] + t[4] + rgbb[0]; ro[plane] = t[1] + t[5] + rgbb[1]; ro[2 * plane] = t[2] + t[6] + rgbb[2];
                }
                if (p.rgb_skip_y) continue;
            }
            if (full_strip) {
                *(uint4*)dst = o0;
                if constexpr (NREG == 16) *(uint4*)(dst + 32) = o1;
            } else if (pv) {
                *(uint4*)dst = o0;
                if constexpr (NREG == 16) *(uint4*)(dst + 32) = o1;
            }
        }
        DGE_T(4);
    };

#ifdef DGE_SC_TIMING
    const int tjob_id = ((blockIdx.x & 7) * jobs_per_xcd + (blockIdx.x >> 3)) * C::TPW + team;
    __builtin_amdgcn_sched_barrier(0);
    const long long tj1 = __builtin_readcyclecounter();
    __builtin_amdgcn_sched_barrier(0);
#endif
    unsigned npar = 0;
    for (int s0_ = 0; s0_ < rows; s0_ += C::NR, npar ^= 1024u) {
        bool done = false;
        StaticFor<C::NR>::run([&](auto ic) {
            constexpr int I = decltype(ic)::value;
            if (!done) {
                if ((C::POOL && (I & 1)) || s0_ + I < rows) step(ic, s0_ + I, npar);
                else done = true;
            }
        });
    }
    if constexpr (C::RGB && C::TEAM == 2) {
        asm volatile("s_waitcnt lgkmcnt(0)" ::: "memory");
        __builtin_amdgcn_s_barrier();
        if (wave == 0 && rows > 0) rgb_flush(rows - 1);
    }
    asm volatile("s_waitcnt vmcnt(0)" ::: "memory");
#ifdef DGE_SC_TIMING
    if (lane == 0 && wave == 0) {
        long long* tl = (long long*)p.y + (size_t)tjob_id * 4;
        tl[0] = tj0; tl[1] = tj1; tl[2] = __builtin_readcyclecounter(); tl[3] = ((long long)rows << 40) | (long long)(__builtin_amdgcn_s_memrealtime() & 0xffffffffffll);
    }
#endif

    if constexpr (C::FRB) {
        float va = 0.f, vc = 0.f;
#pragma unroll
        for (int r = 0; r < 16; r++) {
            float a = pv ? s0[0][r] : 0.f, c = pv ? s1[0][r] : 0.f;
#pragma unroll
            for (int m = 1; m < 32; m <<= 1) { a += __shfl_xor(a, m, 64); c += __shfl_xor(c, m, 64); }
            if (n31 == r) { va = a; vc = c; }
        }
        if (n31 < 16) {
            float* __restrict__ FR = p.fr_out + ((size_t)(blockIdx.x % p.stats_slots) * p.B + b) * COUT * 4 + (8 * kh + (n31 & 7)) * 4 + (n31 >> 3);
            atomicAdd(FR, va); atomicAdd(FR + 2, vc);
        }
    } else
    if constexpr (C::STATS || C::DOT) {
        if (p.stats || (C::INB && p.prep_stats)) {
#pragma unroll
            for (int mt = 0; mt < C::MTW; mt++)
#pragma unroll
                for (int r = 0; r < 16; r++) { if (!pv) { s0[mt][r] = 0.f; s1[mt][r] = 0.f; if constexpr (C::PREP || C::INB) s2[r] = 0.f; } }
            float* __restrict__ ST = p.stats ? p.stats + (size_t)(blockIdx.x % p.stats_slots) * p.B * COUT * 2 + (size_t)b * COUT * 2 : nullptr;
            float* __restrict__ PST = ((C::PREP || C::INB) && p.prep_stats) ? p.prep_stats + (size_t)(blockIdx.x % p.stats_slots) * p.B * COUT * 2 + (size_t)b * COUT * 2 : nullptr;
            const bool det = det_on();
            float* dvec = det ? det_slot(b, p.B, seg * nstrips + strip, nseg * nstrips, COUT * 2) : nullptr;
#pragma unroll
            for (int mt = 0; mt < C::MTW; mt++) {
                float va = 0.f, vc = 0.f, vt = 0.f;
#pragma unroll
                for (int r = 0; r < NREG; r++) {
                    float a = s0[mt][r], c = s1[mt][r], t2 = (C::PREP || C::INB) ? s2[r] : 0.f;
#pragma unroll
                    for (int m = 1; m < 32; m <<= 1) {
                        a += __shfl_xor(a, m, 64); c += __shfl_xor(c, m, 64);
                        if constexpr (C::PREP || C::INB) t2 += __shfl_xor(t2, m, 64);
                    }
                    if (n31 == r) { va = a; vc = c; vt = t2; }
                }
                if (n31 < NREG) {
                    const int ch = wave * C::MTW * 32 + chan_of_reg(mt, n31);
                    if constexpr (C::INB) {
                        if (PST) { atomicAdd(PST + ch * 2, vc); atomicAdd(PST + ch * 2 + 1, vt); }
                    } else if constexpr (C::PREP) {
                        atomicAdd(ST + ch * 2, va);
                        if (PST) { atomicAdd(PST + ch * 2, vt); atomicAdd(PST + ch * 2 + 1, vc); }
                    } else if (det) { dvec[ch * 2] = va; dvec[ch * 2 + 1] = vc; }
                    else { atomicAdd(ST + ch * 2, va); atomicAdd(ST + ch * 2 + 1, vc); }
                }
            }
            if (!C::PREP && !C::INB && det && det_arrive_wave(b, nseg * nstrips * C::TEAM)) {
                for (int idx = lane; idx < COUT * 2; idx += 64)
                    p.stats[(size_t)b * COUT * 2 + idx] = det_sum(b, nseg * nstrips, COUT * 2, idx);
            }
        }
    }
}

template <int CIN, int COUT, int FL>
int launch_stream(const ConvParams& p0, hipStream_t s) {
    using C = SC<CIN, COUT, FL>;
    ConvParams p = p0;
    auto kern = conv_stream_kernel<CIN, COUT, FL>;
    static int caps[16] = {0};
    int dev = 0;
    (void)hipGetDevice(&dev);
    int& cap = caps[dev >= 0 && dev < 16 ? dev : 0];
    if (!cap) {
        (void)hipFuncSetAttribute((const void*)kern, hipFuncAttributeMaxDynamicSharedMemorySize, C::LDS_BYTES * C::TPW);
        int occ = 0, ncu = 256;
        (void)hipDeviceGetAttribute(&ncu, hipDeviceAttributeMultiprocessorCount, dev);
        if (hipOccupancyMaxActiveBlocksPerMultiprocessor(&occ, (const void*)kern, 64 * C::TEAM * C::TPW, C::LDS_BYTES * C::TPW) != hipSuccess || occ < 1) occ = 1;
        cap = occ * ncu * C::TPW;
    }
    const int nstrips = (p.W + 31) / 32;
    int nseg = cap / (p.B * nstrips);
    if (dge_env().stream_nseg > 0) nseg = dge_env().stream_nseg;
    int maxseg = p.H / 16; if (maxseg < 1) maxseg = 1;
    if (nseg > maxseg) nseg = maxseg;
    if (nseg < 1) nseg = 1;
    int seg_rows = (p.H + nseg - 1) / nseg;
    if (C::POOL) seg_rows += seg_rows & 1;
    nseg = (p.H + seg_rows - 1) / seg_rows;
    const int njobs = p.B * nstrips * nseg;
    const int nwg = (njobs + C::TPW - 1) / C::TPW;
    const int jobs_per_xcd = (nwg + 7) / 8;
    const char* fl = FL == FL_GEN ? "gen" : (FL == FL_ENC ? "enc" : (FL == FL_ENC_STATS ? "enc_stats" : (FL == FL_DOT ? "dot" : (FL == FL_DOT_PREP ? "dot_prep" : (FL == FL_GEN_RGB ? "gen_rgb" : (FL == FL_DOT_IN ? "dot_in" : (FL == FL_DOT_FR ? "dot_fromrgb" : (FL == FL_DOT_INX ? "dot_inx" : "enc_pool"))))))));
    dge_note_kernel("conv_stream<bf16,%d,%d,%s>", CIN, COUT, fl);
    hipLaunchKernelGGL(kern, dim3((unsigned)(jobs_per_xcd * 8)), dim3(64 * C::TEAM * C::TPW), C::LDS_BYTES * C::TPW, s, p, nstrips, nseg, seg_rows, njobs, jobs_per_xcd);
    DGE_LAUNCH_CHECK("conv_stream");
    return 0;
}

template <int CIN, int COUT>
int launch_flavour(const ConvParams& p, hipStream_t s) {
    if (p.in_coef && p.fr_out) {
        if constexpr (CIN == 16 && COUT == 16) return launch_stream<CIN, COUT, FL_DOT_FR>(p, s);
        dge_set_error("conv_stream: the FromRGB reduction epilogue is built for 16 -> 16 only");
        return -1;
    }
    if (p.in_coef && !p.prep_stats) {
        if constexpr (CIN == COUT && CIN >= 32) return launch_stream<CIN, COUT, FL_DOT_INX>(p, s);
        dge_set_error("conv_stream: the block-input instance-norm backward epilogue is built for 32 -> 32 and 64 -> 64 only");
        return -1;
    }
    if (p.in_coef) {
        if constexpr ((CIN == 32 && COUT == 16) || (CIN == 64 && COUT == 32)) return launch_stream<CIN, COUT, FL_DOT_IN>(p, s);
        dge_set_error("conv_stream: the instance-norm backward epilogue is built for 32 -> 16 and 64 -> 32 only");
        return -1;
    }
    if (p.dot_src) {
        if constexpr (CIN == COUT && CIN >= 32) {
            if (p.prep) return launch_stream<CIN, COUT, FL_DOT_PREP>(p, s);
        }
        if (p.prep) { dge_set_error("conv_stream: the fused tail backward is built for 32->32 and 64->64 only"); return -1; }
        return launch_stream<CIN, COUT, FL_DOT>(p, s);
    }
    const bool enc = p.stats || p.in_shift || (p.noise && p.noise_w_stride != 0);
    if (p.rgb_out) {
        if constexpr ((CIN == 32 && COUT == 32) || (CIN == 64 && COUT == 64)) { if (!enc) return launch_stream<CIN, COUT, FL_GEN_RGB>(p, s); }
        dge_set_error("conv_stream: the fused toRGB is built for the generator flavour of 32 -> 32 and 64 -> 64 only");
        return -1;
    }
    if (p.pool_out) {
        if constexpr ((CIN == 16 && COUT == 32) || (CIN == 32 && COUT == 64)) { if (!p.stats) return launch_stream<CIN, COUT, FL_ENC_POOL>(p, s); }
        dge_set_error("conv_stream: the pooled epilogue is built for the encoder's 16 -> 32 and 32 -> 64 layers without statistics");
        return -1;
    }
    if constexpr (CIN == 64) {
        if (enc) { dge_set_error("conv_stream: encoder flavour with Cin = 64 is not built"); return -1; }
    } else {
        if (p.stats) return launch_stream<CIN, COUT, FL_ENC_STATS>(p, s);
        if (enc) return launch_stream<CIN, COUT, FL_ENC>(p, s);
    }
    return launch_stream<CIN, COUT, FL_GEN>(p, s);
}

}

bool dge_conv_stream_eligible(const ConvParams& p, int dtype, int ksize) {
    if (dtype != DGE_BF16 || ksize != 3 || p.up || p.in_s2d || p.in_up2 || p.in_relu || p.addend || p.mask_relu || p.in_t2d) return false;
    if (!(p.Cin == 16 || p.Cin == 32 || p.Cin == 64) || !(p.Cout == 16 || p.Cout == 32 || p.Cout == 64)) return false;
    if (p.W % 4 != 0 || p.W < 64 || p.H < 32) return false;
    if ((long)p.H * p.W < 128L * 128) return false;
    {
        const long px = (long)p.B * p.H * p.W;
        const bool enc = p.stats || p.in_shift || (p.noise && p.noise_w_stride != 0);
        if (!dge_env().force_stream) {
            if (!p.dot_src && px < (enc ? (1L << 20) : (1L << 18))) return false;
            if (p.dot_src && px < (1L << 16)) return false;
        }
    }
    if ((long)p.W * p.Cin * 2 >= (1L << 31) || (long)p.H * p.W * 64 * 2 >= (1L << 40)) return false;
    if (p.dot_src && !p.stats && !p.in_coef) return false;
    if (p.in_coef && !p.fr_out && p.prep_stats && !(p.dot_src && !p.prep && !p.stats && ((p.Cin == 32 && p.Cout == 16) || (p.Cin == 64 && p.Cout == 32)))) return false;
    if (p.in_coef && !p.fr_out && !p.prep_stats && !(p.dot_src && !p.prep && !p.stats && p.Cin == p.Cout && p.Cin >= 32 && p.H % 2 == 0 && p.W % 2 == 0)) return false;
    if (p.fr_out && !(p.in_coef && p.dot_src && p.fr_img4 && !p.prep && !p.stats && p.Cin == 16 && p.Cout == 16 && p.H % 2 == 0 && p.W % 2 == 0)) return false;
    if (p.prep && !(p.Cin == p.Cout && p.Cin >= 32)) return false;
    if (p.Cin == 64 && !p.dot_src && (p.stats || p.in_shift || (p.noise && p.noise_w_stride != 0))) return false;
    if (p.dot_src && (p.bias || p.noise || p.in_shift || p.act != DGE_ACT_NONE)) return false;
    if (p.noise && p.noise_w == nullptr) return false;
    if (dge_env().no_stream) return false;
    return true;
}

bool dge_conv_pool_ok(const ConvParams& p, int dtype, int ksize) {
    return ((p.Cin == 16 && p.Cout == 32) || (p.Cin == 32 && p.Cout == 64)) && !p.dot_src && !p.stats && !p.rgb_out && p.H % 2 == 0 && p.W % 2 == 0 &&
           dge_conv_stream_eligible(p, dtype, ksize);
}

bool dge_conv_rgb_ok(const ConvParams& p, int dtype, int ksize) {
    return ((p.Cin == 32 && p.Cout == 32) || (p.Cin == 64 && p.Cout == 64)) && !p.dot_src && !p.stats && !p.in_shift && !(p.noise && p.noise_w_stride != 0) &&
           dge_conv_stream_eligible(p, dtype, ksize);
}

int dge_conv_stream_launch(const ConvParams& p, hipStream_t s) {
#define GO(CI, CO) if (p.Cin == CI && p.Cout == CO) return launch_flavour<CI, CO>(p, s)
#ifdef DGE_SC_ONLY
#define GO2(...) GO(__VA_ARGS__)
    GO2(DGE_SC_ONLY);
#undef GO2
#else
    GO(16, 16); GO(16, 32); GO(16, 64); GO(32, 16); GO(32, 32); GO(32, 64); GO(64, 16); GO(64, 32); GO(64, 64);
#endif
#undef GO
    dge_set_error("conv_stream: unsupported channel configuration %d -> %d", p.Cin, p.Cout);
    return -1;
}
```

### deep-gan-encoders_amd/csrc/s2_bwd_kernels.hip

```cpp
#include "common.h"
#include "../../include/dge_hip.h"

template <typename T>
__global__ __launch_bounds__(256) void modconv_bwd_prep_kernel(const T* __restrict__ gx, const T* __restrict__ x,
                                                                const float* __restrict__ d, const float* __restrict__ noise,
                                                                T* __restrict__ gy, float* __restrict__ R, int HW, int C,
                                                                int noise_bstride, float gain) {
    constexpr int EP = Elem<T>::PER16;
    __shared__ float red[256 * 3 * EP];
    const int b = blockIdx.y;
    const int cpt = C / EP, ppi = 256 / cpt;
    const int chunk = threadIdx.x % cpt, slot = threadIdx.x / cpt;
    float s[3][EP], dd[EP];
#pragma unroll
    for (int e = 0; e < EP; e++) { s[0][e] = s[1][e] = s[2][e] = 0.f; dd[e] = d ? d[(size_t)b * C + chunk * EP + e] : 1.f; }
    for (int p0 = blockIdx.x * ppi; p0 < HW; p0 += gridDim.x * ppi) {
        const int p = p0 + slot;
        if (slot < ppi && p < HW) {
            const size_t o = ((size_t)b * HW + p) * C + chunk * EP;
            float g[EP], xv[EP];
            unpack16(*(const uint4*)(gx + o), g, (T*)nullptr);
            unpack16(*(const uint4*)(x + o), xv, (T*)nullptr);
            const float nz = noise ? noise[(size_t)b * noise_bstride + p] : 0.f;
#pragma unroll
            for (int e = 0; e < EP; e++) {
                const bool pos = xv[e] > 0.f;
                const float gz = g[e] * gain * (pos ? 1.f : 0.2f);
                const float z = pos ? xv[e] / gain : xv[e] / (0.2f * gain);
                s[0][e] += gz * z; s[1][e] += gz * nz; s[2][e] += gz;
                g[e] = gz * dd[e];
            }
            *(uint4*)(gy + o) = pack16(g, (T*)nullptr);
        }
    }
    if (R) block_chan_flush<EP, 3>(s, cpt, ppi, R + (size_t)b * C * 3, C, red);
}

__global__ void demod_bwd_kernel(const float* __restrict__ R, const float* __restrict__ d, const float* __restrict__ bias,
                                 const float* __restrict__ ns, float* __restrict__ t, int B, int C, float bscale) {
    const int idx = blockIdx.x * blockDim.x + threadIdx.x;
    if (idx >= B * C) return;
    const int o = idx % C;
    const float dv = d[idx];
    t[idx] = -(R[(size_t)idx * 3] - (ns ? ns[0] : 0.f) * R[(size_t)idx * 3 + 1] - bias[o] * bscale * R[(size_t)idx * 3 + 2]) * dv * dv;
}

__global__ void demod_bwd_prep_kernel(const float* __restrict__ P, int nslot, const float* __restrict__ d, const float* __restrict__ bias,
                                      float* __restrict__ t, int B, int C, float bscale) {
    const int idx = blockIdx.x * blockDim.x + threadIdx.x;
    if (idx >= B * C) return;
    const float2 pp = sum_slot_pairs(P + (size_t)idx * 2, (size_t)B * C * 2, nslot);
    const float dv = d[idx];
    t[idx] = -(pp.x - bias[idx % C] * bscale * pp.y) * dv * dv;
}

template <typename T>
__global__ __launch_bounds__(256) void torgb_bwd_prep_kernel(const float* __restrict__ gimg, const T* __restrict__ x,
                                                              const float* __restrict__ wrgb, const float* __restrict__ sty,
                                                              const float* __restrict__ noise, const float* __restrict__ nsp,
                                                              T* __restrict__ gz_out, float* __restrict__ gs, float* __restrict__ P,
                                                              int HW, int C, float wscale, float gain, int noise_bstride) {
    constexpr int EP = Elem<T>::PER16;
    __shared__ float red[256 * 2 * EP];
    const int b = blockIdx.y;
    const int cpt = C / EP, ppi = 256 / cpt;
    const int chunk = threadIdx.x % cpt, slot = threadIdx.x / cpt;
    float w0[EP], w1[EP], w2[EP], sv[EP], sg[1][EP], sp[2][EP];
#pragma unroll
    for (int e = 0; e < EP; e++) {
        const int i = chunk * EP + e;
        w0[e] = wrgb[i] * wscale; w1[e] = wrgb[C + i] * wscale; w2[e] = wrgb[2 * C + i] * wscale;
        sv[e] = sty[(size_t)b * C + i]; sg[0][e] = 0.f; sp[0][e] = 0.f; sp[1][e] = 0.f;
    }
    const float ns = (noise && nsp) ? nsp[0] : 0.f;
    const float gpos = gain, gneg = 0.2f * gain, zpos = 1.f / gain, zneg = 1.f / (0.2f * gain);
    const float* gb = gimg + (size_t)b * 3 * HW;
    for (int p0 = blockIdx.x * ppi; p0 < HW; p0 += gridDim.x * ppi) {
        const int p = p0 + slot;
        if (slot < ppi && p < HW) {
            const float g0 = gb[p], g1 = gb[HW + p], g2 = gb[2 * HW + p];
            const float nzs = noise ? ns * noise[(size_t)b * noise_bstride + p] : 0.f;
            const size_t o = ((size_t)b * HW + p) * C + chunk * EP;
            float xv[EP], out[EP];
            unpack16(*(const uint4*)(x + o), xv, (T*)nullptr);
#pragma unroll
            for (int e = 0; e < EP; e++) {
                const float t = g0 * w0[e] + g1 * w1[e] + g2 * w2[e];
                sg[0][e] += t * xv[e];
                const bool pos = xv[e] > 0.f;
                const float gz = t * sv[e] * (pos ? gpos : gneg);
                const float zt = xv[e] * (pos ? zpos : zneg) - nzs;
                sp[0][e] = fmaf(gz, zt, sp[0][e]); sp[1][e] += gz;
                out[e] = gz;
            }
            *(uint4*)(gz_out + o) = pack16(out, (T*)nullptr);
        }
    }
    block_chan_flush<EP, 1>(sg, cpt, ppi, gs + (size_t)b * C, C, red);
    block_chan_flush<EP, 2>(sp, cpt, ppi, P + (size_t)b * C * 2, C, red);
}

__global__ __launch_bounds__(1024) void linear_t_kernel(const float* __restrict__ x, int ldx, int incx, const float* __restrict__ W,
                                const float* __restrict__ mul, float* __restrict__ y, int ldy, int incy, int B, int O, int K,
                                float scale, int accumulate) {
    __shared__ float part[16][64];
    const int lane = threadIdx.x & 63, wave = threadIdx.x >> 6;
    const int k = blockIdx.x * 64 + lane, b = blockIdx.y;
    const int per = (O + 15) / 16, o0 = wave * per, o1 = min(O, o0 + per);
    float acc[8];
#pragma unroll
    for (int j = 0; j < 8; j++) acc[j] = 0.f;
    if (k < K) {
        const float* xr = x + (size_t)b * ldx;
        int o = o0;
        for (; o + 7 < o1; o += 8) {
#pragma unroll
            for (int j = 0; j < 8; j++) acc[j] += xr[(size_t)(o + j) * incx] * W[(size_t)(o + j) * K + k];
        }
        for (; o < o1; o++) acc[0] += xr[(size_t)o * incx] * W[(size_t)o * K + k];
    }
    part[wave][lane] = ((acc[0] + acc[1]) + (acc[2] + acc[3])) + ((acc[4] + acc[5]) + (acc[6] + acc[7]));
    __syncthreads();
    if (wave == 0 && k < K) {
        float s = 0.f;
#pragma unroll
        for (int j = 0; j < 16; j++) s += part[j][lane];
        s *= scale;
        if (mul) s *= mul[(size_t)b * K + k];
        float* yp = y + (size_t)b * ldy + (size_t)k * incy;
        *yp = accumulate ? *yp + s : s;
    }
}

template <typename T>
__global__ __launch_bounds__(256) void torgb_bwd_kernel(const float* __restrict__ gimg, const T* __restrict__ x,
                                                         const float* __restrict__ wrgb, const float* __restrict__ sty,
                                                         T* __restrict__ gx, float* __restrict__ gs, int HW, int C, float wscale) {
    constexpr int EP = Elem<T>::PER16;
    __shared__ float red[256 * EP];
    const int b = blockIdx.y;
    const int cpt = C / EP, ppi = 256 / cpt;
    const int chunk = threadIdx.x % cpt, slot = threadIdx.x / cpt;
    float w0[EP], w1[EP], w2[EP], sv[EP], s[1][EP];
#pragma unroll
    for (int e = 0; e < EP; e++) {
        const int i = chunk * EP + e;
        w0[e] = wrgb[i] * wscale; w1[e] = wrgb[C + i] * wscale; w2[e] = wrgb[2 * C + i] * wscale;
        sv[e] = sty[(size_t)b * C + i]; s[0][e] = 0.f;
    }
    const float* gb = gimg + (size_t)b * 3 * HW;
    for (int p0 = blockIdx.x * ppi; p0 < HW; p0 += gridDim.x * ppi) {
        const int p = p0 + slot;
        if (slot < ppi && p < HW) {
            const float g0 = gb[p], g1 = gb[HW + p], g2 = gb[2 * HW + p];
            const size_t o = ((size_t)b * HW + p) * C + chunk * EP;
            float xv[EP], out[EP];
            unpack16(*(const uint4*)(x + o), xv, (T*)nullptr);
#pragma unroll
            for (int e = 0; e < EP; e++) {
                const float t = g0 * w0[e] + g1 * w1[e] + g2 * w2[e];
                s[0][e] += t * xv[e];
                out[e] = t * sv[e];
            }
            *(uint4*)(gx + o) = pack16(out, (T*)nullptr);
        }
    }
    block_chan_flush<EP, 1>(s, cpt, ppi, gs + (size_t)b * C, C, red);
}

__global__ void up2_bwd_kernel(const float* __restrict__ g, float* __restrict__ gprev, int BC, int h, int w) {
// ... 260 lines not shown
```

### deep-gan-encoders_amd/ops.py

```python
import ctypes as C
import math

import torch

from ._lib import lib, check, ConvDesc, ConvPPDesc, DgeError, last_kernel

F32, BF16 = 0, 1
ACT_NONE, ACT_LRELU, ACT_RELU, LIN_RSQRT = 0, 1, 2, 3
PACK_FWD, PACK_UPFOLD, PACK_DGRAD, PACK_UPFOLD_DGRAD, PACK_SG1_UP, PACK_SG1_UP_DGRAD, PACK_UPT2D_DGRAD = 0, 1, 2, 3, 4, 5, 6
PACK_FRAG = 0x100
import os as _os
import weakref as _weakref
_PF = {"on": not _os.environ.get("DGE_NO_PREFETCH"), "prev": {}, "next": {}}
KERNEL_LOG = None
PROFILE = None


class _ZeroArena:

    def __init__(self):
        self.buf, self.off, self.high, self.active = None, 0, 0, False


_ARENA = _ZeroArena()
# ... 215 lines not shown
    check(lib().dge_weight_sumsq(_f32(w.detach().contiguous()), _p(out), cout, cin, k, float(scale), _stream()),
          "dge_weight_sumsq")
    return out


def linear(x, w, bias=None, wscale=1.0, bscale=1.0, add=0.0, act=ACT_NONE, gain=1.0, square_input=False, out=None):
    B, I = x.shape
    O = w.shape[0]
    if x.stride(1) != 1:
        raise DgeError("linear: inner stride must be 1")
    if out is None:
        out = torch.empty((B, O), dtype=torch.float32, device=x.device)
    if not x.is_cuda:
        raise DgeError("tensor is not on the GPU: the HIP path has no CPU fallback")
    check(lib().dge_linear(C.c_void_p(x.data_ptr()), x.stride(0), _f32(w), _f32(bias), C.c_void_p(out.data_ptr()),
                           out.stride(0), B, I, O, float(wscale), float(bscale), float(add), act, float(gain),
                           1 if square_input else 0, _stream()), "dge_linear")
    return out


def _dense_layers(layers):
    from ._lib import DenseLayer
    arr = (DenseLayer * len(layers))()
    for e, L in zip(arr, layers):
        e.w, e.bias = _p(L.weight.detach()), _p(L.bias.detach())
        e.O, e.I = L.weight.shape
        e.wscale, e.bscale, e.add, e.act, e.gain = float(L.wscale), float(L.bscale), float(L.additional_bias), int(L.act), float(L.gain)
    return arr


def mapping_bwd(z, layers, g, coefs=None, acts=None, pixelnorm=True, eps=1e-8):
    B, L = g.shape[0], g.shape[1]
    if not z.is_cuda or z.stride(1) != 1:
        raise DgeError("mapping_bwd: z must be a CUDA tensor with unit inner stride")
    if z.shape[1] != layers[0].weight.shape[1] or z.shape[0] != B:
        raise DgeError(f"mapping_bwd: z {tuple(z.shape)} does not match B = {B}, first layer width {layers[0].weight.shape[1]}")
    g = g.float().contiguous()
    if g.shape[2] != layers[-1].weight.shape[0]:
        raise DgeError(f"mapping_bwd: gradient width {g.shape[2]} != last layer width {layers[-1].weight.shape[0]}")
    if coefs is not None and coefs.numel() != L:
        raise DgeError(f"mapping_bwd: {coefs.numel()} coefficients for {L} rows")
    arr = arr_p = None
    if acts is not None:
        if len(acts) != len(layers) or any(tuple(a.shape) != (B, Ly.weight.shape[0]) for a, Ly in zip(acts, layers)):
            raise DgeError("mapping_bwd: acts must hold one [B, O_l] output per layer")
        arr = (C.c_void_p * len(acts))(*[_f32(a).value for a in acts])
        arr_p = C.cast(arr, C.c_void_p)
    dz = torch.empty((B, z.shape[1]), dtype=torch.float32, device=z.device)
    check(lib().dge_mapping_bwd(_f32(z), z.stride(0), _dense_layers(layers), len(layers), arr_p, _p(g), L,
                                _f32(None if coefs is None else coefs.contiguous()), _p(dz), dz.stride(0), B, 1 if pixelnorm else 0,
                                float(eps), _stream()), "dge_mapping_bwd")
    return dz


def dense_chain(x, layers, pixelnorm=False, eps=1e-8):
    B = x.shape[0]
    arr = _dense_layers(layers)
    y = torch.empty((B, layers[-1].weight.shape[0]), dtype=torch.float32, device=x.device)
    if not x.is_cuda or x.stride(1) != 1:
        raise DgeError("dense_chain: x must be a CUDA tensor with unit inner stride")
    check(lib().dge_dense_chain(_f32(x), x.stride(0), arr, len(layers), _p(y), y.stride(0), B, 1 if pixelnorm else 0, float(eps), _stream()),
          "dge_dense_chain")
    return y


def pixelnorm(x, eps=1e-8):
    y = torch.empty_like(x)
    check(lib().dge_pixelnorm(_f32(x), _p(y), x.shape[0], x.shape[1], eps, _stream()), "dge_pixelnorm")
    return y


def truncation(w, w_avg, num_layers, psi, layers):
    w_is_wp = (w.ndim == 3)
    B, D = w.shape[0], w.shape[-1]
    wp = torch.empty((B, num_layers, D), dtype=torch.float32, device=w.device)
    check(lib().dge_truncation(_f32(w.contiguous()), _f32(w_avg), _p(wp), B, num_layers, D, float(psi), int(layers),
                               1 if w_is_wp else 0, _stream()), "dge_truncation")
    return wp


def conv2d(x, w_packed, cout, ksize=3, up=False, in_scale=None, in_shift=None, out_scale=None, bias=None,
           bias_scale=1.0, noise=None, noise_w=None, act=ACT_NONE, gain=1.0, addend=None, add_scale=1.0, stats=None,
           out=None, in_s2d=False, dot_src=None, in_up2=False, in_relu=False, prep=None, relu_mask=None, in_t2d=False, rgb=None, pool_out=False, pool_mask=False,
           in_bwd=None):
    B, H, W, Cin = x.shape
    if in_s2d:
        H, W, Cin = H // 2, W // 2, Cin * 4
    if in_up2:
        H, W = 2 * H, 2 * W
    if in_t2d:
        H, W = H - 1, W - 1
    dt = dtype_of(x)
    OH, OW = (2 * H, 2 * W) if up else (H, W)
    mask = None
    if pool_out:
        if out is not None or up:
            raise DgeError("conv2d: pool_out allocates its own result and excludes up")
        out = torch.empty((B, OH // 2, OW // 2, cout), dtype=x.dtype, device=x.device)
        if pool_mask:
            mask = torch.empty((B, (OH // 2) * (OW // 2), cout // 8), dtype=torch.int32, device=x.device)
    if out is None:
        out = torch.empty((B, OH, OW, cout), dtype=x.dtype, device=x.device)
    d = ConvDesc()
    d.pool_out, d.pool_mask = 1 if pool_out else 0, _p(mask)
    if relu_mask is not None:
        if dot_src is not None or prep is not None:
            raise DgeError("conv2d: relu_mask excludes dot_src / prep")
        dot_src = relu_mask
    d.mask_relu = 0 if relu_mask is None else 1
    d.in_t2d = 1 if in_t2d else 0
    d.x, d.w_packed, d.y, d.addend, d.dot_src = _p(x), _p(w_packed), _p(out), _p(addend), _p(dot_src)
    d.in_scale, d.in_shift, d.out_scale = _f32(in_scale), _f32(in_shift), _f32(out_scale)
    partial, nslot = None, 1
    lazy = isinstance(stats, SlotStats)
    if stats is not None:
        nblk = ((H + 15) // 16) * ((W + 15) // 16) * B
        nslot = max(1, min(64, nblk // 16))
        if lazy:
            partial = stats.alloc(nslot)
        elif nslot > 1:
            partial = zeros((nslot,) + tuple(stats.shape), x.device)
    d.bias, d.noise, d.noise_w, d.stats = _f32(bias), _f32(noise), _f32(noise_w), _f32(partial if partial is not None else stats)
    d.stats_slots = nslot
    d.B, d.H, d.W, d.Cin, d.Cout = B, H, W, Cin, cout
    d.ksize, d.up, d.in_s2d, d.in_up2 = ksize, 1 if up else 0, 1 if in_s2d else 0, 1 if in_up2 else 0
    d.in_relu = 1 if in_relu else 0
    d.w_layout = 1 if getattr(w_packed, "_dge_frag", False) else 0
    if d.w_layout and _PF["on"]:
        sk = (_stream().value or 0)
        key = w_packed.data_ptr()
        prev = _PF["prev"].get(sk) if isinstance(_PF["prev"], dict) else None
        if not isinstance(_PF["prev"], dict):
            _PF["prev"] = {}
        if prev is not None and prev != key:
            if len(_PF["next"]) > 512:
                _PF["next"].clear()
            _PF["next"][(sk, prev)] = (key, w_packed.shape[1], w_packed.shape[2], _weakref.ref(w_packed))
        _PF["prev"][sk] = key
        nxt = _PF["next"].get((sk, key))
        if nxt is not None:
            t = nxt[3]()
            if t is None or t.data_ptr() != nxt[0]:
                del _PF["next"][(sk, key)]
            else:
                d.prefetch_w, d.prefetch_ntot, d.prefetch_cin = C.c_void_p(nxt[0]), int(nxt[1]), int(nxt[2])
    if prep is not None:
        if stats is None or dot_src is None:
            raise DgeError("conv2d: prep needs stats and dot_src")
        pn = prep.get("noise")
        d.prep, d.prep_gain = 1, float(prep["gain"])
        d.prep_noise, d.prep_ns = _f32(pn), _f32(prep.get("ns") if pn is not None else None)
        d.prep_noise_batch = 1 if pn is None else pn.shape[0]
        d.prep_stats = _f32(prep["stats"].alloc(nslot))
    if in_bwd is not None:
        if dot_src is None or stats is not None or prep is not None:
            raise DgeError("conv2d: in_bwd needs dot_src and excludes stats / prep")
        nblk = ((H + 15) // 16) * ((W + 15) // 16) * B
        d.stats_slots = max(1, min(64, nblk // 16))
        pn = in_bwd.get("noise")
        d.in_bwd_coef = _f32(in_bwd["coef"])
        d.prep_noise, d.prep_noise_batch = _f32(pn), 1 if pn is None else pn.shape[0]
        if in_bwd.get("fr") is not None:
            d.fr_img4, d.in_bwd_extra, d.in_bwd_extra_scale = _f32(in_bwd["img4"]), _p(in_bwd.get("extra")), float(in_bwd.get("extra_scale", 1.0))
            in_bwd["fr"].buf = zeros((d.stats_slots, B, cout, 4), x.device)
            d.fr_out = _f32(in_bwd["fr"].buf)
        elif in_bwd.get("red") is not None:
            d.prep_stats = _f32(in_bwd["red"].alloc(d.stats_slots))
        else:
            d.prep_noise = None
            d.in_bwd_extra, d.in_bwd_extra_scale = _p(in_bwd.get("extra")), float(in_bwd.get("extra_scale", 1.0))
    if rgb is not None:
        d.rgb_w, d.rgb_style, d.rgb_bias, d.rgb_out = _f32(rgb["w"]), _f32(rgb["style"]), _f32(rgb["bias"]), _f32(rgb["out"])
        d.rgb_wscale, d.rgb_skip_y = float(rgb["wscale"]), 1 if rgb.get("skip_y") else 0
    d.noise_batch = 1 if noise is None else noise.shape[0]
    d.noise_w_per_channel = 0 if (noise_w is None or noise_w.numel() == 1) else 1
    d.act, d.bias_scale, d.gain, d.add_scale, d.dtype = act, bias_scale, gain, add_scale, dt
    if w_packed.dtype != x.dtype:
        raise DgeError("conv2d: packed weight dtype differs from activation dtype")
    if PROFILE is not None:
        e0, e1 = torch.cuda.Event(enable_timing=True), torch.cuda.Event(enable_timing=True)
        e0.record()
        check(lib().dge_conv2d(C.byref(d), _stream()), "dge_conv2d")
        e1.record()
        if up:
            macs = 9.0 * Cin * cout * H * W
        elif in_s2d or in_t2d:
            macs = 9.0 * (Cin // 4) * cout * H * W
        else:
            macs = float(ksize * ksize) * Cin * cout * H * W
        skip_y = rgb is not None and rgb.get("skip_y")
        abytes = sum(t.numel() * t.element_size() for t in (x, None if skip_y else out, addend, dot_src, w_packed,
                                                            rgb["out"] if rgb is not None else None) if t is not None)
        PROFILE.append((e0, e1, 2.0 * macs * B, (B, H, W, Cin, cout, ksize, up, in_s2d), abytes))
    else:
        check(lib().dge_conv2d(C.byref(d), _stream()), "dge_conv2d")
    if partial is not None and not lazy:
        check(lib().dge_sum_slots(_p(partial), _p(stats), nslot, stats.numel(), 1, _stream()), "dge_sum_slots")
    if rgb is not None and rgb.get("skip_y"):
        return None
    if pool_out and pool_mask:
        return out, mask
    return out


def conv_in_bwd_supported(B, H, W, cin, cout, dtype):
    return bool(lib().dge_conv_in_bwd_supported(int(B), int(H), int(W), int(cin), int(cout), 3, int(dtype)))


def conv_in_bwd_x_supported(B, H, W, cin, cout, dtype):
    return bool(lib().dge_conv_in_bwd_x_supported(int(B), int(H), int(W), int(cin), int(cout), 3, int(dtype)))


def conv_in_bwd_fromrgb_supported(B, H, W, cin, cout, dtype):
    return bool(lib().dge_conv_in_bwd_fromrgb_supported(int(B), int(H), int(W), int(cin), int(cout), 3, int(dtype)))


def up_pp_supported(B, H, W, cin, cout, dtype):
    return bool(lib().dge_up_pp_supported(int(B), int(H), int(W), int(cin), int(cout), int(dtype)))


def pack_up_pp(w_units, cout, cin, in_scale=None, out_scale=None, gain=1.0, out=None):
    if w_units.dtype != torch.bfloat16:
        raise DgeError("pack_up_pp: expects the bf16 units of pack_upconv_weight")
    nb = 1
    for t in (in_scale, out_scale):
        if t is not None:
            nb = t.shape[0]
    if out is None:
        out = torch.empty((nb, 9 * cin * cout), dtype=torch.bfloat16, device=w_units.device)
    check(lib().dge_pack_up_pp(_p(w_units), _p(out), int(cout), int(cin), _f32(in_scale), _f32(out_scale), float(gain), nb, _stream()),
          "dge_pack_up_pp")
    return out


def up_pp(x, w_img, cout, bias=None, bias_scale=1.0, noise=None, noise_w=None, act=ACT_NONE, gain=1.0):
    B, H, W, Cin = x.shape
    if x.dtype != torch.bfloat16 or not x.is_cuda:
        raise DgeError("up_pp: bf16 CUDA activations only (the HIP path has no CPU fallback)")
    y = torch.empty((B, 2 * H, 2 * W, cout), dtype=x.dtype, device=x.device)
    nbs = 0 if (noise is None or noise.shape[0] == 1) else 4 * H * W
    if noise_w is not None and noise_w.numel() != 1:
        raise DgeError("up_pp: one noise strength per layer (stylegan2_generator.py:911-916)")
    wbs = 0 if w_img.shape[0] == 1 else w_img.stride(0)

    def launch():
        check(lib().dge_up_pp(_p(x), _p(w_img), int(wbs), _p(y), _f32(noise), nbs, _f32(noise_w), _f32(bias), float(bias_scale),
                              float(gain), int(act), B, H, W, Cin, int(cout), _stream()), "dge_up_pp")
    if PROFILE is not None:
        e0, e1 = torch.cuda.Event(enable_timing=True), torch.cuda.Event(enable_timing=True)
        e0.record(); launch(); e1.record()
        abytes = sum(t.numel() * t.element_size() for t in (x, y)) + 18 * Cin * cout * B
        PROFILE.append((e0, e1, 2.0 * 9.0 * Cin * cout * H * W * B, (B, H, W, Cin, cout, 3, "upfir", False), abytes))
    else:
        launch()
    if KERNEL_LOG is not None:
        KERNEL_LOG.append((last_kernel(), _stream()))
    return y


def conv_pp_supported(B, H, W, cin, cout, dtype):
    return bool(lib().dge_conv_pp_supported(int(B), int(H), int(W), int(cin), int(cout), int(dtype)))


def pack_conv_pp(w, wscale=1.0, in_scale=None, out_scale=None, gain=1.0, dgrad=False, out=None):
    cout, cin = w.shape[0], w.shape[1]
    N, K = (cin, cout) if dgrad else (cout, cin)
    nb = 1
    for t in (in_scale, out_scale):
        if t is not None:
            nb = t.shape[0]
    if out is None:
        out = torch.empty((nb, 9 * N * K), dtype=torch.bfloat16, device=w.device)
    check(lib().dge_pack_conv_pp(_f32(w.detach().contiguous()), _p(out), N, K, float(wscale), _f32(in_scale), _f32(out_scale), float(gain),
                                 nb, 1 if dgrad else 0, _stream()), "dge_pack_conv_pp")
    return out


def pack_conv_pp_rows(w_rows, N, in_scale=None, in_period=None, out_scale=None, gain=1.0, out=None, t2d=False):
# ... 58 lines not shown
        e0, e1 = torch.cuda.Event(enable_timing=True), torch.cuda.Event(enable_timing=True)
        e0.record()
        check(lib().dge_conv_pp(C.byref(d), _stream()), "dge_conv_pp")
        e1.record()
        abytes = sum(t.numel() * t.element_size() for t in (x, out, w_pp, dot_src, addend) if t is not None)
        macs = 9.0 * (Cin // 4 if (in_s2d or in_t2d) else Cin) * cout * H * W
        PROFILE.append((e0, e1, 2.0 * macs * B, (B, H, W, Cin, cout, 3, False, bool(in_s2d or in_t2d)), abytes))
    else:
        check(lib().dge_conv_pp(C.byref(d), _stream()), "dge_conv_pp")
    if KERNEL_LOG is not None:
        KERNEL_LOG.append((last_kernel(), _stream()))
    return out


def torgb(x, wrgb, style, bias, prev, wscale):
    B, H, W, Cin = x.shape
    img = torch.empty((B, 3, H, W), dtype=torch.float32, device=x.device)
    check(lib().dge_torgb(_p(x), _f32(wrgb), _f32(style), _f32(bias), _f32(prev), _p(img), B, H, W, Cin, float(wscale),
                          dtype_of(x), _stream()), "dge_torgb")
    return img


def nchw_to_nhwc(src, B, dtype):
    sB, Cc, H, W = src.shape
    dst = torch.empty((B, H, W, Cc), dtype=tdtype(dtype), device=src.device)
    check(lib().dge_nchw_to_nhwc(_f32(src.contiguous()), _p(dst), B, Cc, H * W, sB, dtype, _stream()), "dge_nchw_to_nhwc")
    return dst


def nhwc_to_nchw(src):
    B, H, W, Cc = src.shape
    dst = torch.empty((B, Cc, H, W), dtype=torch.float32, device=src.device)
    check(lib().dge_nhwc_to_nchw(_p(src), _p(dst), B, Cc, H * W, dtype_of(src), _stream()), "dge_nhwc_to_nchw")
    return dst


def fromrgb(img, w, bias, dtype, stats=None, img4=False):
    B, _, H, W = img.shape
    Cc = w.shape[0]
    y = torch.empty((B, H, W, Cc), dtype=tdtype(dtype), device=img.device)
    i4 = torch.empty((B, H, W, 4), dtype=torch.float32, device=img.device) if img4 else None
    check(lib().dge_fromrgb2(_f32(img.contiguous()), _f32(w.reshape(Cc, 3)), _f32(bias), _p(y), _f32(stats), _f32(i4), B, H * W, Cc,
                             dtype, _stream()), "dge_fromrgb")
    return (y, i4) if img4 else y


def stats_finalize(stats, npix, eps=1e-8, musig_out=None):
    nslot = 1
    if isinstance(stats, SlotStats):
        B, Cc, nslot, stats = stats.B, stats.C, stats.nslot, stats.buf
    else:
        B, Cc, _ = stats.shape
    musig = torch.empty((B, 2 * Cc), dtype=torch.float32, device=stats.device) if musig_out is None else musig_out
    sc = torch.empty((B, Cc), dtype=torch.float32, device=stats.device)
    sh = torch.empty((B, Cc), dtype=torch.float32, device=stats.device)
    check(lib().dge_stats_finalize_slots(_f32(stats), nslot, _p(musig), _p(sc), _p(sh), B, Cc, int(npix), float(eps), _stream()),
          "dge_stats_finalize")
    return musig, sc, sh


def blend(x, z=None, sc=None, sh=None, pool=False, alpha=1.0, beta=0.0, stats=None, mask=False):
    B, H, W, Cc = x.shape
    OH, OW = (H // 2, W // 2) if pool else (H, W)
    y = torch.empty((B, OH, OW, Cc), dtype=x.dtype, device=x.device)
    if mask:
        if not pool or sc is not None or sh is not None:
            raise DgeError("blend: the sign mask is offered for the plain pooling blend")
        ep = 8 if x.dtype == torch.bfloat16 else 4
        m = torch.empty((B, OH * OW, Cc // ep), dtype=torch.int32, device=x.device)
        check(lib().dge_blend_pool_mask(_p(x), _p(z), _p(y), _f32(stats), _p(m), B, OH, OW, Cc, float(alpha), float(beta), dtype_of(x),
                                        _stream()), "dge_blend_pool_mask")
        return y, m
    check(lib().dge_blend(_p(x), _p(z), _p(y), _f32(sc), _f32(sh), _f32(stats), B, OH, OW, Cc, 1 if pool else 0,
                          float(alpha), float(beta), dtype_of(x), _stream()), "dge_blend")
    return y


def modconv_bwd_prep(gx, x, d, noise, gain, R=None):
    B, H, W, Cc = x.shape
    gy = torch.empty_like(x)
    check(lib().dge_modconv_bwd_prep(_p(gx), _p(x), _f32(d), _f32(noise), _p(gy), _f32(R), B, H * W, Cc,
                                     1 if noise is None else noise.shape[0], float(gain), dtype_of(x), _stream()),
          "dge_modconv_bwd_prep")
    return gy


def torgb_bwd_prep(gimg, x, wrgb, style, wscale, noise, ns, gain):
    B, H, W, Cc = x.shape
    gz = torch.empty_like(x)
    gs = zeros((B, Cc), x.device)
    P = zeros((B, Cc, 2), x.device)
    check(lib().dge_torgb_bwd_prep(_f32(gimg), _p(x), _f32(wrgb), _f32(style), _f32(noise), _f32(ns if noise is not None else None),
                                   1 if noise is None else noise.shape[0], _p(gz), _p(gs), _p(P), B, H * W, Cc, float(wscale),
                                   float(gain), dtype_of(x), _stream()), "dge_torgb_bwd_prep")
    return gz, gs, P


def demod_bwd_prep(P, d, bias, bscale=1.0):
    B, Cc = d.shape
    nslot = 1
    if isinstance(P, SlotStats):
        nslot, P = P.nslot, P.buf
    t = torch.empty_like(d)
    check(lib().dge_demod_bwd_prep(_f32(P), nslot, _f32(d), _f32(bias), _p(t), B, Cc, float(bscale), _stream()), "dge_demod_bwd_prep")
    return t


def demod_bwd(R, d, bias, noise_strength, bscale=1.0):
    B, Cc = d.shape
    t = torch.empty_like(d)
    check(lib().dge_demod_bwd(_f32(R), _f32(d), _f32(bias), _f32(noise_strength), _p(t), B, Cc, float(bscale), _stream()),
          "dge_demod_bwd")
    return t


def linear_t(x, w, y, mul=None, scale=1.0, accumulate=False, incx=1, incy=1, ldx=None, ldy=None, B=None, O=None):
    O_, K = w.shape
    B = x.shape[0] if B is None else B
    O = O_ if O is None else O
    ldx = x.stride(0) if ldx is None else ldx
    ldy = y.stride(0) if ldy is None else ldy
    check(lib().dge_linear_t(C.c_void_p(x.data_ptr()), ldx, incx, _f32(w), _f32(mul), C.c_void_p(y.data_ptr()), ldy, incy,
                             B, O, K, float(scale), 1 if accumulate else 0, _stream()), "dge_linear_t")
    return y


def fir_t2d(g, scale=None):
    B, FH, FW, Cc = g.shape
    H, W = FH // 2, FW // 2
    z = torch.empty((B, H + 1, W + 1, 4 * Cc), dtype=g.dtype, device=g.device)
    check(lib().dge_fir_t2d(_p(g), _f32(scale), _p(z), B, H, W, Cc, dtype_of(g), _stream()), "dge_fir_t2d")
    return z


def s2_style_grads(blocks, g_wp, wscale):
    from ._lib import S2GradEntry
    arr = (S2GradEntry * len(blocks))()
    B, nrows, K = g_wp.shape
    for e, blk in zip(arr, blocks):
        e.wstyle, e.row = _f32(blk["wstyle"]), int(blk["row"])
        if "gs" in blk:
            e.gs, e.in_c = _f32(blk["gs"]), blk["gs"].shape[1]
            continue
        P, st = blk["P"], blk["st"]
        e.nslot_p, e.nslot_s = 1, 1
        if isinstance(P, SlotStats):
            e.nslot_p, P = P.nslot, P.buf
        if isinstance(st, SlotStats):
            e.nslot_s, st = st.nslot, st.buf
        e.P, e.st, e.d, e.s, e.bias, e.wsq = _f32(P), _f32(st), _f32(blk["d"]), _f32(blk["s"]), _f32(blk["bias"]), _f32(blk["wsq"])
        e.out_c, e.in_c = blk["d"].shape[1], blk["s"].shape[1]
        e.bscale = float(blk["bscale"])
    check(lib().dge_s2_style_grads(arr, len(blocks), _p(g_wp), B, nrows, K, float(wscale), _stream()), "dge_s2_style_grads")
    return g_wp


def torgb_bwd(gimg, x, wrgb, style, wscale):
    B, H, W, Cc = x.shape
    gx = torch.empty_like(x)
    gs = zeros((B, Cc), x.device)
    check(lib().dge_torgb_bwd(_f32(gimg), _p(x), _f32(wrgb), _f32(style), _p(gx), _p(gs), B, H * W, Cc, float(wscale),
                              dtype_of(x), _stream()), "dge_torgb_bwd")
    return gx, gs


def up2_bwd(g):
    B, Cc, H, W = g.shape
    out = torch.empty((B, Cc, H // 2, W // 2), dtype=torch.float32, device=g.device)
    check(lib().dge_up2_bwd(_f32(g), _p(out), B * Cc, H // 2, W // 2, _stream()), "dge_up2_bwd")
    return out


def conv_wgrad(g, x, dw, in_scale=None, in_shift=None):
    B, H, W, Cin = x.shape
    cout, _, k, _ = dw.shape
    check(lib().dge_conv_wgrad(_p(g), _p(x), _f32(in_scale), _f32(in_shift), _f32(dw), B, H, W, cout, Cin, k, dtype_of(x),
                               _stream()), "dge_conv_wgrad")
# ... 46 lines not shown
    check(lib().dge_sum_slots_planar(_p(part), _p(red), B, Cc, NS, _stream()), "dge_sum_slots_planar")
    return red


def act_bwd(gup, a, noise=None, pool=False, scale=1.0, red=None, slope=0.2, planar=False, defer=None):
    B, H, W, Cc = a.shape
    gpre = torch.empty_like(a)
    ncol = 2 if red is None else (red.shape[0] if planar else red.shape[-1])
    part = zeros((B, Cc, ncol), a.device) if red is not None else None
    check(lib().dge_act_bwd(_p(gup), _p(a), _f32(noise), _p(gpre), _f32(part), ncol, B, H, W, Cc,
                            1 if pool else 0, float(scale), float(slope), dtype_of(a), _stream()), "dge_act_bwd")
    if red is not None:
        _sum_planar(part, red, defer) if planar else _sum_over_batch(part, red)
    return gpre


def act_bwd_mask(gup, mask, noise, scale=1.0, red=None, slope=0.2, planar=False, defer=None):
    B, UH, UW, Cc = gup.shape
    H, W = 2 * UH, 2 * UW
    gpre = torch.empty((B, H, W, Cc), dtype=gup.dtype, device=gup.device)
    ncol = 2 if red is None else (red.shape[0] if planar else red.shape[-1])
    part = zeros((B, Cc, ncol), gup.device) if red is not None else None
    check(lib().dge_act_bwd_mask(_p(gup), _p(mask), _f32(noise), _p(gpre), _f32(part), ncol, B, H, W, Cc, float(scale), float(slope),
                                 dtype_of(gup), _stream()), "dge_act_bwd_mask")
    if red is not None:
        _sum_planar(part, red, defer) if planar else _sum_over_batch(part, red)
    return gpre


def in_bwd_coef(dots, gms, musig, sc, sh, npix):
    B, Cc = sc.shape
    coef = torch.empty((B, Cc, 3), dtype=torch.float32, device=sc.device)
    nslot = 1
    if isinstance(dots, SlotStats):
        nslot, dots = dots.nslot, dots.buf
    check(lib().dge_in_bwd_coef_slots(_f32(dots), nslot, _f32(gms), _f32(musig), _f32(sc), _f32(sh), _p(coef), B, Cc, int(npix),
                                      _stream()), "dge_in_bwd_coef")
    return coef


def in_bwd(gy, x, coef, extra=None, extra_pool=False, extra_scale=1.0, noise=None, act=False, red=None, planar=False, defer=None):
    B, H, W, Cc = x.shape
    gout = torch.empty_like(x)
    part = zeros((B, Cc, 2), x.device) if red is not None else None
    if isinstance(coef, tuple) and Cc > 512:
        coef = in_bwd_coef(*coef)
    if isinstance(coef, tuple):
        dots, gms, musig, sc, sh, npix = coef
        nslot = 1
        if isinstance(dots, SlotStats):
            nslot, dots = dots.nslot, dots.buf
        check(lib().dge_in_bwd_fused(_p(gy), _p(x), _f32(dots), nslot, _f32(gms), _f32(musig), _f32(sc), _f32(sh), int(npix), _p(extra),
                                     _f32(noise), _p(gout), _f32(part), B, H, W, Cc, 1 if extra_pool else 0, float(extra_scale),
                                     1 if act else 0, dtype_of(x), _stream()), "dge_in_bwd_fused")
    else:
        check(lib().dge_in_bwd(_p(gy), _p(x), _f32(coef), _p(extra), _f32(noise), _p(gout), _f32(part), B, H, W, Cc,
                               1 if extra_pool else 0, float(extra_scale), 1 if act else 0, dtype_of(x), _stream()), "dge_in_bwd")
    if red is not None:
        _sum_planar(part, red, defer) if planar else _sum_over_batch(part, red)
    return gout


def in_bwd_fromrgb(gy, x0, coef, img, extra=None, extra_pool=False, extra_scale=1.0, defer=None):
    B, H, W, Cc = x0.shape
    dots, gms, musig, sc, sh, npix = coef
    nslot = 1
    if isinstance(dots, SlotStats):
        nslot, dots = dots.nslot, dots.buf
    part = zeros((B, Cc, 4), x0.device)
    check(lib().dge_in_bwd_fromrgb(_p(gy), _p(x0), _f32(dots), nslot, _f32(gms), _f32(musig), _f32(sc), _f32(sh), int(npix), _p(extra),
                                   _f32(img.contiguous()), _p(part), B, H, W, Cc, 1 if extra_pool else 0, float(extra_scale),
                                   dtype_of(x0), _stream()), "dge_in_bwd_fromrgb")
    return _sum_planar(part, torch.empty((4, Cc), dtype=torch.float32, device=x0.device), defer)


def conv_pool_supported(B, H, W, cin, cout, ksize, dtype):
    return bool(lib().dge_conv_pool_supported(B, H, W, cin, cout, ksize, dtype))


def conv_rgb_supported(B, H, W, cin, cout, ksize, dtype):
    return bool(lib().dge_conv_rgb_supported(B, H, W, cin, cout, ksize, dtype))


def rgb_upsample_add(img, prev):
    B, Cc, H, W = img.shape
    check(lib().dge_rgb_upsample_add(_p(img), _f32(prev), B * Cc, H, W, _stream()), "dge_rgb_upsample_add")
    return img


def chan_sum(x, scale=1.0):
    B, H, W, Cc = x.shape
    part = zeros((B, Cc), x.device)
    check(lib().dge_chan_sum(_p(x), _p(part), B, H * W, Cc, float(scale), dtype_of(x), _stream()), "dge_chan_sum")
    return _sum_over_batch(part)


def fromrgb_bwd(gx, x0, img, planar=False, defer=None):
    B, H, W, Cc = x0.shape
    part = zeros((B, Cc, 4), x0.device)
    check(lib().dge_fromrgb_bwd(_p(gx), _p(x0), _f32(img.contiguous()), _p(part), B, H * W, Cc, dtype_of(x0), _stream()),
          "dge_fromrgb_bwd")
    if planar:
        return _sum_planar(part, torch.empty((4, Cc), dtype=torch.float32, device=x0.device), defer)
    return _sum_over_batch(part)


def dense_wgrad(gy, x, gw, gb=None, accumulate=False):
    B, O = gy.shape
    I = x.shape[1]
    check(lib().dge_dense_wgrad(C.c_void_p(gy.data_ptr()), gy.stride(0), C.c_void_p(x.data_ptr()), x.stride(0), _f32(gw),
                                _f32(gb), B, O, I, 1 if accumulate else 0, _stream()), "dge_dense_wgrad")
    return gw, gb


def scale_(t, factor):
    check(lib().dge_axpy_scalar(_f32(t), None, _p(t), t.numel(), float(factor), 0, _stream()), "dge_axpy_scalar")
    return t


def blur_noise_act(x, noise, noise_w, bias, blur=True, stats=None, act=True):
    B, H, W, Cc = x.shape
    y = torch.empty_like(x)
    check(lib().dge_blur_noise_act(_p(x), _f32(noise), _f32(noise_w), _f32(bias), _p(y), _f32(stats), B, H, W, Cc,
                                   1 if blur else 0, 1 if noise is None else noise.shape[0], 1 if act else 0, dtype_of(x),
                                   _stream()), "dge_blur_noise_act")
    return y


def affine_compose(sc, sh, style):
    B, Cc = sc.shape
    a = torch.empty_like(sc)
    b = torch.empty_like(sc)
    check(lib().dge_affine_compose(_f32(sc), _f32(sh), _f32(style), _p(a), _p(b), B, Cc, _stream()), "dge_affine_compose")
    return a, b


def lerp_layers(w, avg, coefs):
    B, D = w.shape
    L = coefs.numel()
    out = torch.empty((B, L, D), dtype=torch.float32, device=w.device)
    stride = D if avg.numel() == L * D else 0
    check(lib().dge_lerp_layers(_f32(w), _f32(avg.contiguous()), stride, _f32(coefs.contiguous()), _p(out), B, L, D, _stream()),
          "dge_lerp_layers")
    return out


def pixelnorm_nhwc(x, eps=1e-8):
    B, H, W, Cc = x.shape
    y = torch.empty_like(x)
    check(lib().dge_pixelnorm_nhwc(_p(x), _p(y), B * H * W, Cc, float(eps), dtype_of(x), _stream()), "dge_pixelnorm_nhwc")
    return y


def cbn_affine(scale, offset, mean, var, eps):
    B, Cc = scale.shape
    a = torch.empty((B, Cc), dtype=torch.float32, device=scale.device)
    b = torch.empty_like(a)
    ld = scale.stride(0) if B > 1 else Cc
    if scale.dtype != torch.float32 or offset.dtype != torch.float32 or scale.stride(1) != 1 or offset.stride(1) != 1 or \
            (B > 1 and offset.stride(0) != ld):
        raise DgeError("cbn_affine: scale / offset must be float32 rows with unit inner stride and a common row stride")
    check(lib().dge_cbn_affine(C.c_void_p(scale.data_ptr()), C.c_void_p(offset.data_ptr()), ld, _f32(mean.contiguous()),
                               _f32(var.contiguous()), float(eps), _p(a), _p(b), B, Cc, _stream()), "dge_cbn_affine")
    return a, b


# ... 214 lines not shown
```

### include/dge_hip.h

```cpp
#ifndef DGE_HIP_H
#define DGE_HIP_H
#include <stddef.h>
#ifdef __cplusplus
extern "C" {
#endif

typedef struct ihipStream_t* dge_stream_t;

#define DGE_DTYPE_F32 0
#define DGE_DTYPE_BF16 1
#define DGE_ACT_LINEAR 0
#define DGE_ACT_LRELU02 1
#define DGE_ACT_RELU_ 2
#define DGE_LIN_RSQRT 3
#define DGE_PACK_FWD 0
#define DGE_PACK_UPFOLD 1
#define DGE_PACK_DGRAD 2
#define DGE_PACK_UPFOLD_DGRAD 3
#define DGE_PACK_SG1_UP 4
#define DGE_PACK_SG1_UP_DGRAD 5
#define DGE_PACK_UPT2D_DGRAD 6

const char* dge_last_error(void);
int dge_version(void);

typedef struct dge_conv_desc {
    const void* x;
    const void* w_packed;
    void* y;
    const void* addend;
    const void* dot_src;
    const float* in_scale;
    const float* in_shift;
    const float* out_scale;
    const float* bias;
    const float* noise;
    const float* noise_w;
    float* stats;
    int B, H, W, Cin, Cout;
    int ksize;
    int up;
    int in_s2d;
    int noise_batch;
    int noise_w_per_channel;
    int act;
    float bias_scale, gain, add_scale;
    int dtype;
    int in_up2;
    int in_relu;
    int stats_slots;
    int w_layout;
    int prep;
    float prep_gain;
    const float* prep_noise;
    const float* prep_ns;
    int prep_noise_batch;
    float* prep_stats;
    int mask_relu;
    int in_t2d;
    const float* rgb_w;
    const float* rgb_style;
    const float* rgb_bias;
    float* rgb_out;
    float rgb_wscale;
    int rgb_skip_y;
    int pool_out;
    void* pool_mask;
    const void* prefetch_w;
    int prefetch_ntot, prefetch_cin;
    const float* in_bwd_coef;
    const void* in_bwd_extra;
    float in_bwd_extra_scale;
    const float* fr_img4;
    float* fr_out;
} dge_conv_desc;
int dge_conv2d(const dge_conv_desc* d, dge_stream_t stream);
int dge_conv_small_supported(int H, int W, int cin, int ntot, int ksize, int in_s2d, int in_up2, int dtype);
#define DGE_PACK_FRAG 0x100
const char* dge_last_kernel(void);
void dge_env_reload(void);
int dge_sum_slots(const float* partial, float* out, int nslot, int n, int accumulate, dge_stream_t stream);
int dge_sum_slots_planar(const float* partial, float* out, int nslot, int C, int NS, dge_stream_t stream);
typedef struct dge_sum_planar_entry { const float* partial; float* out; int nslot, C, NS, pad; } dge_sum_planar_entry;
int dge_sum_slots_planar_multi(const dge_sum_planar_entry* entries, int n, dge_stream_t stream);

int dge_linear_rows(const float* x, int ldx_b, const int* row_xoff, const float* w, const float* bias, float* y,
                    const int* row_ybase, const int* row_ybstride, int B, int R, int K, float wscale, float bscale, float add,
                    dge_stream_t stream);
int dge_demod_rows(const float* s_all, const float* wsq_cat, const int* row_woff, const int* row_sbase, const int* row_cin,
                   float* d_all, const int* row_dbase, const int* row_dbstride, int B, int R, float eps, dge_stream_t stream);
int dge_set_deterministic(int on);
int dge_get_deterministic(void);
int dge_packed_n(int n_valid);
int dge_pack_conv_weight(const float* w_oihw, void* out, int cout, int cin, int ksize, int mode, int dtype,
                         float scale, dge_stream_t stream);
int dge_pack_conv_weights_multi(const long long* table_host, void* descs_dev, int n, int upload, dge_stream_t stream);
int dge_pack_desc_bytes(void);
int dge_weight_sumsq(const float* w_oihw, float* wsq, int cout, int cin, int ksize, float scale, dge_stream_t stream);

int dge_linear(const float* x, int ldx, const float* w, const float* bias, float* y, int ldy, int B, int I, int O,
               float wscale, float bscale, float add, int act, float gain, int square_input, dge_stream_t stream);
int dge_pixelnorm(const float* x, float* y, int B, int D, float eps, dge_stream_t stream);
typedef struct dge_dense_layer { const float* w; const float* bias; int I, O; float wscale, bscale, add; int act; float gain; } dge_dense_layer;
int dge_dense_chain(const float* x, int ldx, const dge_dense_layer* layers, int n, float* y, int ldy, int B, int pixelnorm, float eps,
                    dge_stream_t stream);
int dge_truncation(const float* w, const float* w_avg, float* wp, int B, int L, int D, float psi, int layers,
                   int w_is_wp, dge_stream_t stream);

int dge_torgb(const void* x, const float* wrgb, const float* style, const float* bias, const float* prev, float* img,
              int B, int H, int W, int cin, float wscale, int dtype, dge_stream_t stream);

int dge_conv_rgb_supported(int B, int H, int W, int Cin, int Cout, int ksize, int dtype);
int dge_conv_in_bwd_supported(int B, int H, int W, int Cin, int Cout, int ksize, int dtype);
int dge_conv_in_bwd_fromrgb_supported(int B, int H, int W, int Cin, int Cout, int ksize, int dtype);
int dge_conv_in_bwd_x_supported(int B, int H, int W, int Cin, int Cout, int ksize, int dtype);
int dge_conv_pool_supported(int B, int H, int W, int Cin, int Cout, int ksize, int dtype);
int dge_rgb_upsample_add(float* img, const float* prev, int BC, int H, int W, dge_stream_t stream);
int dge_nchw_to_nhwc(const float* src, void* dst, int B, int C, int HW, int src_B, int dtype, dge_stream_t stream);
int dge_nhwc_to_nchw(const void* src, float* dst, int B, int C, int HW, int dtype, dge_stream_t stream);

int dge_fromrgb(const float* img, const float* w, const float* bias, void* y, float* stats, int B, int HW, int C,
                int dtype, dge_stream_t stream);
int dge_fromrgb2(const float* img, const float* w, const float* bias, void* y, float* stats, float* img4, int B, int HW, int C,
                 int dtype, dge_stream_t stream);
int dge_stats_finalize(const float* stats, float* musig, float* sc, float* sh, int B, int C, int npix, float eps,
                       dge_stream_t stream);
int dge_stats_finalize_slots(const float* stats, int nslot, float* musig, float* sc, float* sh, int B, int C, int npix, float eps,
                             dge_stream_t stream);
int dge_blend(const void* x, const void* z, void* y, const float* sc, const float* sh, float* stats, int B, int OH,
              int OW, int C, int pool, float alpha, float beta, int dtype, dge_stream_t stream);

int dge_loss_reduce(const float* a, const float* b, float* sums7, int B, int C, int H, int W, int y0, int x0, int h, int w,
                    dge_stream_t stream);
int dge_crop_pool(const float* src, float* dst, int BC, int H, int W, int y0, int x0, int h, int w, int k, dge_stream_t stream);
int dge_ssim_fwd(const float* a, const float* b, float* ssim_sum, float* dmap, int BC, int h, int w, dge_stream_t stream);
int dge_ssim_box7(const float* a, const float* b, float* sums, int BC, int h, int w, float scale, float shift, float data_range,
                  dge_stream_t stream);
int dge_ssim_bwd(const float* a, const float* b, const float* dmap, float* g, int BC, int h, int w, float scale,
                 int accumulate, dge_stream_t stream);
int dge_space_loss_finalize(const float* sums7, const float* ssim_sum, const float* lpips, float* out8, float n,
                            float n_pooled, int image_space, dge_stream_t stream);
int dge_space_loss_bwd(const float* a, const float* b, const float* sums7, const float* g_pooled, float* g, int BC, int H,
                       int W, int y0, int x0, int h, int w, int k, float n, float weight, int accumulate, dge_stream_t stream);
int dge_loss_reduce3(const float* a, const float* b, float* sums, int B, int C, int H, int W, const int* wins, int nwin, dge_stream_t stream);
int dge_crop_pool_multi(const float* const* src, float* const* dst, const int* wins, const int* ks, int n, int BC, int H, int W,
                        dge_stream_t stream);
int dge_space_loss_bwd3(const float* a, const float* b, const float* const* sums7, const float* const* g_pooled, float* g, int BC, int H,
                        int W, const int* wins, const int* ks, const float* n, const float* weight, int nwin, dge_stream_t stream);
int dge_axpy_scalar(const float* x, const float* scalar, float* y, long n, float extra, int accumulate, dge_stream_t stream);

int dge_lreq_adam_multi(int ntensors, float* const* host_p, const float* const* host_g, float* const* host_v,
                        const long* host_n, const float* host_step, float beta2, float eps, const float* gscale,
                        const float* step_mult, dge_stream_t stream);

int dge_modconv_bwd_prep(const void* gx, const void* x, const float* d, const float* noise, void* gy, float* R, int B,
                         int HW, int C, int noise_batch, float gain, int dtype, dge_stream_t stream);
int dge_demod_bwd(const float* R, const float* d, const float* bias, const float* noise_strength, float* t, int B, int C,
                  float bscale, dge_stream_t stream);
int dge_linear_t(const float* x, int ldx, int incx, const float* w, const float* mul, float* y, int ldy, int incy, int B,
                 int O, int K, float scale, int accumulate, dge_stream_t stream);
int dge_torgb_bwd(const float* gimg, const void* x, const float* wrgb, const float* style, void* gx, float* gs, int B,
                  int HW, int C, float wscale, int dtype, dge_stream_t stream);
int dge_torgb_bwd_prep(const float* gimg, const void* x, const float* wrgb, const float* style, const float* noise,
                       const float* noise_strength, int noise_batch, void* gz, float* gs, float* P, int B, int HW, int C,
                       float wscale, float gain, int dtype, dge_stream_t stream);
int dge_fir_t2d(const void* g, const float* scale, void* z, int B, int H, int W, int C, int dtype, dge_stream_t stream);
typedef struct dge_s2_grad_entry {
    const float* P; const float* st; const float* d; const float* s; const float* bias; const float* wsq;
    const float* gs; const float* wstyle;
    int nslot_p, nslot_s, in_c, out_c, row;
    float bscale;
} dge_s2_grad_entry;
int dge_s2_style_grads(const dge_s2_grad_entry* entries, int n, float* g_wp, int B, int nrows, int K, float wscale, dge_stream_t stream);
int dge_demod_bwd_prep(const float* P, int nslot, const float* d, const float* bias, float* t, int B, int C, float bscale,
                       dge_stream_t stream);
int dge_up2_bwd(const float* g, float* gprev, int BC, int h, int w, dge_stream_t stream);

int dge_conv_wgrad(const void* g, const void* x, const float* in_scale, const float* in_shift, float* dw, int B, int H, int W,
                   int cout, int cin, int ksize, int dtype, dge_stream_t stream);
int dge_conv_wgrad_dots(const void* g, const void* x, const float* in_scale, const float* in_shift, float* dw, const float* w,
                        float* dots, int dots_slots, int B, int H, int W, int cout, int cin, int dtype, dge_stream_t stream);
int dge_act_bwd(const void* gup, const void* a, const float* noise, void* gpre, float* red, int red_cols, int B, int H, int W, int C,
                int pool, float scale, float slope, int dtype, dge_stream_t stream);
int dge_blend_pool_mask(const void* x, const void* z, void* y, float* stats, unsigned* mask, int B, int OH, int OW, int C, float alpha,
                        float beta, int dtype, dge_stream_t stream);
int dge_act_bwd_mask(const void* gup, const unsigned* mask, const float* noise, void* gpre, float* red, int red_cols, int B, int H, int W,
                     int C, float scale, float slope, int dtype, dge_stream_t stream);
int dge_fromrgb_dgrad(const void* gx, const void* x0, const float* w, float* gimg, int B, int HW, int C, int dtype, dge_stream_t stream);
int dge_nearest_up2(const void* x, void* y, int B, int H, int W, int C, float scale, int dtype, dge_stream_t stream);
int dge_in_bwd_coef(const float* dots, const float* gms, const float* musig, const float* sc, const float* sh, float* coef,
                    int B, int C, int npix, dge_stream_t stream);
int dge_in_bwd_coef_slots(const float* dots, int nslot, const float* gms, const float* musig, const float* sc, const float* sh,
                          float* coef, int B, int C, int npix, dge_stream_t stream);
int dge_in_bwd(const void* gy, const void* x, const float* coef, const void* extra, const float* noise, void* gout, float* red,
               int B, int H, int W, int C, int extra_pool, float extra_scale, int act, int dtype, dge_stream_t stream);
// ... 142 lines not shown
```

Before: 383.0 images/sec.

## Fuse toRGB backward prologue into top-layer streaming data-gradient conv

Instead of running a separate torgb_bwd_prep kernel at 1024x1024 that writes the pre-activation gradient to memory, the streaming data-gradient conv of the top synthesis layer now DMA-loads the image gradient and noise rows into LDS. It computes the toRGB adjoint and leaky-ReLU backward per pixel on the fly and accumulates the style gradient and prep statistics with atomics. This drops a full-resolution write and read of the gradient tensor plus a kernel launch. In exchange it forces one wave per EU (WPE=1) for this flavour, adds register and LDS pressure and atomics, and applies only to the 32->32 bf16 non-deterministic path.

Result: no change. 386.5 images/sec (median of 6 runs) (+0.9%).

```diff
diff --git a/deep-gan-encoders_amd/_lib.py b/deep-gan-encoders_amd/_lib.py
--- a/deep-gan-encoders_amd/_lib.py
+++ b/deep-gan-encoders_amd/_lib.py
@@ -7,6 +7,11 @@
 
 class DgeError(RuntimeError):
     pass
+
+
+class RgbBwdDesc(C.Structure):
+    _fields_ = [("gimg", C.c_void_p), ("w", C.c_void_p), ("style", C.c_void_p), ("noise", C.c_void_p), ("ns", C.c_void_p),
+                ("gs", C.c_void_p), ("stats", C.c_void_p), ("wscale", C.c_float), ("gain", C.c_float), ("noise_batch", C.c_int)]
 
 
 class ConvDesc(C.Structure):
@@ -24,6 +29,7 @@
         ("rgb_skip_y", C.c_int), ("pool_out", C.c_int), ("pool_mask", C.c_void_p),
         ("prefetch_w", C.c_void_p), ("prefetch_ntot", C.c_int), ("prefetch_cin", C.c_int), ("in_bwd_coef", C.c_void_p),
         ("in_bwd_extra", C.c_void_p), ("in_bwd_extra_scale", C.c_float), ("fr_img4", C.c_void_p), ("fr_out", C.c_void_p),
+        ("rgb_bwd", RgbBwdDesc),
     ]
 
 
@@ -76,6 +82,7 @@
     "dge_truncation": [_P, _P, _P, _I, _I, _I, _F, _I, _I, _P],
     "dge_torgb": [_P, _P, _P, _P, _P, _P, _I, _I, _I, _I, _F, _I, _P],
     "dge_conv_rgb_supported": [_I, _I, _I, _I, _I, _I, _I],
+    "dge_conv_rgb_bwd_supported": [_I, _I, _I, _I, _I, _I, _I],
     "dge_conv_in_bwd_supported": [_I, _I, _I, _I, _I, _I, _I],
     "dge_conv_in_bwd_fromrgb_supported": [_I, _I, _I, _I, _I, _I, _I],
     "dge_conv_in_bwd_x_supported": [_I, _I, _I, _I, _I, _I, _I],
diff --git a/deep-gan-encoders_amd/autograd_s2.py b/deep-gan-encoders_amd/autograd_s2.py
--- a/deep-gan-encoders_amd/autograd_s2.py
+++ b/deep-gan-encoders_amd/autograd_s2.py
@@ -1,4 +1,5 @@
 import math
+import os
 
 import torch
 
@@ -160,13 +161,21 @@
     top = nl - 2
     Lt, Ot = getattr(mod, f"layer{top}"), getattr(mod, f"output{top // 2}")
     P = None
-    if fused:
+    rgb_bwd = None
+    if (fused and top >= 1 and not Lt.up and not os.environ.get("DGE_NO_RGB_BWD") and
+            ops.conv_rgb_bwd_supported(B, Lt.res, Lt.res, Lt.out_c, Lt.in_c, 3, dt)):
+        rgb_bwd = dict(gimg=g_img, w=Ot.weight.detach().reshape(3, -1), style=saved["rgb"][top // 2]["s"], wscale=Ot.wscale,
+                       noise=layers[top]["noise"], ns=Lt.noise_strength.detach().reshape(1), gain=Lt.gain)
+        g_x, g_srgb = layers[top]["y"], None
+    elif fused:
         g_x, g_srgb, P = ops.torgb_bwd_prep(g_img, layers[top]["y"], Ot.weight.detach().reshape(3, -1), saved["rgb"][top // 2]["s"], Ot.wscale,
                                             layers[top]["noise"], Lt.noise_strength.detach().reshape(1), Lt.gain)
     else:
         g_x, g_srgb = ops.torgb_bwd(g_img, layers[top]["y"], Ot.weight.detach().reshape(3, -1), saved["rgb"][top // 2]["s"], Ot.wscale)
     blocks = [] if fused else None
-    if fused:
+    if rgb_bwd is not None:
+        pass
+    elif fused:
         blocks.append(dict(gs=g_srgb, wstyle=Ot.style.weight.detach(), row=top + 1))
     else:
         ops.linear_t(g_srgb, Ot.style.weight.detach(), g_wp[:, top + 1], scale=Ot.style.wscale, accumulate=True)
@@ -175,7 +184,8 @@
     for i in range(top, -1, -1):
         L = getattr(mod, f"layer{i}")
         rec = layers[i]
-        if P is not None:
+        rb = rgb_bwd if i == top else None
+        if P is not None or rb is not None:
             g_y, d_in = g_x, rec["d"]
         else:
             R = ops.zeros((B, L.out_c, 3), dev)
@@ -200,7 +210,12 @@
             P_next = ops.SlotStats(B, L.in_c, dev)
             prep = dict(gain=Lp.gain, noise=layers[i - 1]["noise"], ns=Lp.noise_strength.detach().reshape(1), stats=P_next)
         hg = L.res // 2 if L.up else L.res
-        if fused and d_in is not None and not t2d and _pp_dgrad(L, B, hg, dt):
+        if rb is not None:
+            g_xprev = ops.conv2d(g_y, _dgrad_weight(L, dt), L.in_c, 3, in_scale=d_in, out_scale=rec["s"], addend=addend, add_scale=1.0, stats=st,
+                                 dot_src=x_in, prep=prep, rgb_bwd=rb)
+            P = rb["P"]
+            blocks.append(dict(gs=rb["gs"], wstyle=Ot.style.weight.detach(), row=top + 1))
+        elif fused and d_in is not None and not t2d and _pp_dgrad(L, B, hg, dt):
             g_xprev = ops.conv_pp(g_y, _dgrad_weight_pp(L, d_in), L.in_c, dgrad=True, in_s2d=L.up, out_scale=rec["s"], addend=addend,
                                   add_scale=1.0, stats=st, dot_src=x_in, prep=prep)
         elif t2d and fused and prep is not None and _pp_dgrad(L, B, hg, dt):
diff --git a/deep-gan-encoders_amd/csrc/capi.hip b/deep-gan-encoders_amd/csrc/capi.hip
--- a/deep-gan-encoders_amd/csrc/capi.hip
+++ b/deep-gan-encoders_amd/csrc/capi.hip
@@ -123,8 +123,17 @@
         DGE_CHECK(d->ksize == 3 && !d->up && dge_conv_stream_eligible(p, d->dtype, d->ksize), "conv2d: in_bwd_coef is offered where "
                   "dge_conv_in_bwd_supported() says so, with dot_src and prep_stats, without stats / prep");
     }
+    p.rb_gimg = d->rgb_bwd.gimg; p.rb_w = d->rgb_bwd.w; p.rb_style = d->rgb_bwd.style; p.rb_noise = d->rgb_bwd.noise;
+    p.rb_ns = d->rgb_bwd.noise ? d->rgb_bwd.ns : nullptr; p.rb_gs = d->rgb_bwd.gs; p.rb_stats = d->rgb_bwd.stats;
+    p.rb_wscale = d->rgb_bwd.wscale; p.rb_gain = d->rgb_bwd.gain; p.rb_noise_bstride = d->rgb_bwd.noise_batch > 1 ? OH * OW : 0;
+    if (d->rgb_bwd.gimg) {
+        DGE_CHECK(d->rgb_bwd.w && d->rgb_bwd.style && d->rgb_bwd.gs && d->rgb_bwd.stats && d->rgb_bwd.gain > 0.f,
+                  "conv2d: rgb_bwd needs w, style, gs, stats and a positive gain");
+        DGE_CHECK(!dge_get_deterministic() && dge_conv_rgb_bwd_ok(p, d->dtype, d->ksize), "conv2d: the toRGB adjoint prologue is offered where "
+                  "dge_conv_rgb_bwd_supported() says so (bf16 3x3 32 -> 32 data-gradient launches with prep on the streaming kernel)");
+    }
     if (d->pool_out)
-        DGE_CHECK(!d->up && dge_conv_pool_ok(p, d->dtype, d->ksize), "conv2d: the pooled epilogue is offered where dge_conv_pool_supported() "
+        DGE_CHECK(!d->up && dge_conv_pool_ok(p, d->dtype, d->ksize),"conv2d: the pooled epilogue is offered where dge_conv_pool_supported() "
                   "says so (conv_2 of the first encoder blocks on the streaming kernel)");
     if (d->rgb_out) {
         DGE_CHECK(d->rgb_w && d->rgb_style && d->rgb_bias, "conv2d: rgb_out needs rgb_w, rgb_style, rgb_bias");
@@ -164,6 +173,13 @@
     ConvParams p = {};
     p.B = B; p.H = H; p.W = W; p.Cin = Cin; p.Cout = Cout; p.Ntot_valid = Cout; p.Ntot = dge_packed_n(Cout);
     return dge_conv_rgb_ok(p, dtype, ksize) ? 1 : 0;
+}
+
+extern "C" int dge_conv_rgb_bwd_supported(int B, int H, int W, int Cin, int Cout, int ksize, int dtype) {
+    ConvParams p = {};
+    p.B = B; p.H = H; p.W = W; p.Cin = Cin; p.Cout = Cout; p.Ntot_valid = Cout; p.Ntot = dge_packed_n(Cout);
+    p.dot_src = (const void*)16; p.stats = (float*)16; p.prep = 1; p.prep_stats = (float*)16; p.rb_gimg = (const float*)16;
+    return (!dge_get_deterministic() && dge_conv_rgb_bwd_ok(p, dtype, ksize)) ? 1 : 0;
 }
 
 __global__ void sum_slots_kernel(const float* __restrict__ partial, float* __restrict__ out, int nslot, int n, int accumulate) {
diff --git a/deep-gan-encoders_amd/csrc/common.h b/deep-gan-encoders_amd/csrc/common.h
--- a/deep-gan-encoders_amd/csrc/common.h
+++ b/deep-gan-encoders_amd/csrc/common.h
@@ -29,6 +29,10 @@
 }
 
 #include <type_traits>
+__device__ __forceinline__ float torgb_adj3(float g0, float g1, float g2, float w0, float w1, float w2) {
+    return __fmaf_rn(g2, w2, __fmaf_rn(g1, w1, __fmul_rn(g0, w0)));
+}
+
 template <int N, int I = 0> struct StaticFor {
     template <class F> __device__ static __forceinline__ void run(F&& f) { f(std::integral_constant<int, I>{}); StaticFor<N, I + 1>::run(f); }
 };
diff --git a/deep-gan-encoders_amd/csrc/conv_params.h b/deep-gan-encoders_amd/csrc/conv_params.h
--- a/deep-gan-encoders_amd/csrc/conv_params.h
+++ b/deep-gan-encoders_amd/csrc/conv_params.h
@@ -49,6 +49,14 @@
     int pf_ntot, pf_cin;
     const float* in_coef;
     const void* in_extra; float in_extra_scale; const float* fr_img4; float* fr_out;
+    const float* rb_gimg;
+    const float* rb_w;
+    const float* rb_style;
+    const float* rb_noise;
+    const float* rb_ns;
+    float* rb_gs; float* rb_stats;
+    float rb_wscale, rb_gain;
+    int rb_noise_bstride;
 };
 
 int dge_conv_launch(const ConvParams& p, int dtype, int ksize, hipStream_t s);
@@ -58,6 +66,7 @@
 int dge_conv_stream_launch(const ConvParams& p, hipStream_t s);
 bool dge_conv_rgb_ok(const ConvParams& p, int dtype, int ksize);
 bool dge_conv_pool_ok(const ConvParams& p, int dtype, int ksize);
+bool dge_conv_rgb_bwd_ok(const ConvParams& p, int dtype, int ksize);
 bool dge_conv_small_shape_ok(int H, int W, int cin, int ntot, int ksize, int in_s2d, int in_up2, int dtype);
 int dge_conv_small_launch(const ConvParams& p, hipStream_t s);
 bool dge_conv_pw_eligible(const ConvParams& p, int dtype, int ksize);
diff --git a/deep-gan-encoders_amd/csrc/conv_stream.hip b/deep-gan-encoders_amd/csrc/conv_stream.hip
--- a/deep-gan-encoders_amd/csrc/conv_stream.hip
+++ b/deep-gan-encoders_amd/csrc/conv_stream.hip
@@ -57,6 +57,9 @@
 __device__ __forceinline__ void dma_piece(unsigned voff, rsrc_t rs, unsigned m0v) {
     asm volatile("s_mov_b32 m0, %1\n\ts_nop 0\n\tbuffer_load_dwordx4 %0, %2, 0 offen lds" : : "v"(voff), "s"(m0v), "s"(rs) : "memory");
 }
+__device__ __forceinline__ void dma_dword(unsigned voff, rsrc_t rs, unsigned m0v) {
+    asm volatile("s_mov_b32 m0, %1\n\ts_nop 0\n\tbuffer_load_dword %0, %2, 0 offen lds" : : "v"(voff), "s"(m0v), "s"(rs) : "memory");
+}
 template <int NP> __device__ __forceinline__ void dma_dot(unsigned voff, unsigned voff1, rsrc_t rs, unsigned m0v) {
     if constexpr (NP == 1)
         asm volatile("s_mov_b32 m0, %1\n\ts_nop 0\n\tbuffer_load_dwordx4 %0, %2, 0 offen lds" : : "v"(voff), "s"(m0v), "s"(rs) : "memory");
@@ -65,7 +68,7 @@
                      "buffer_load_dwordx4 %3, %2, 0 offen offset:1024 lds" : : "v"(voff), "s"(m0v), "s"(rs), "v"(voff1) : "memory");
 }
 
-enum { FL_GEN = 0, FL_ENC = 1, FL_ENC_STATS = 2, FL_DOT = 3, FL_DOT_PREP = 4, FL_GEN_RGB = 5, FL_ENC_POOL = 6, FL_DOT_IN = 7, FL_DOT_FR = 8, FL_DOT_INX = 9 };
+enum { FL_GEN = 0, FL_ENC = 1, FL_ENC_STATS = 2, FL_DOT = 3, FL_DOT_PREP = 4, FL_GEN_RGB = 5, FL_ENC_POOL = 6, FL_DOT_IN = 7, FL_DOT_FR = 8, FL_DOT_INX = 9, FL_DOT_PREP_RGB = 10 };
 
 template <int CIN, int COUT, int FL>
 struct SC {
@@ -76,7 +79,7 @@
     static constexpr int MTW = MT / TEAM;
     static constexpr int HW = 34, RB = HW * PXB;
     static constexpr int PIECES = (RB + 1023) / 1024;
-    static constexpr bool PREP = FL == FL_DOT_PREP, RGB = FL == FL_GEN_RGB, POOL = FL == FL_ENC_POOL, FRB = FL == FL_DOT_FR, INX = FL == FL_DOT_INX, INB = FL == FL_DOT_IN || FRB || INX;
+    static constexpr bool RGBB = FL == FL_DOT_PREP_RGB, PREP = FL == FL_DOT_PREP || RGBB, RGB = FL == FL_GEN_RGB, POOL = FL == FL_ENC_POOL, FRB = FL == FL_DOT_FR, INX = FL == FL_DOT_INX, INB = FL == FL_DOT_IN || FRB || INX;
     static_assert(!RGB || COUT == 32 || (COUT == 64 && TEAM == 2), "fused toRGB: 32 output channels per wave, one wave or a 2-wave team per pixel");
     static constexpr bool DOT = FL == FL_DOT || PREP || INB, STATS = FL == FL_ENC_STATS, ENC = FL == FL_ENC || FL == FL_ENC_STATS || POOL;
     static constexpr bool NOISE = !DOT || PREP || (INB && !FRB && !INX);
@@ -92,7 +95,7 @@
     static constexpr int DROWB = 32 * DCH * 16, DPIECES = DROWB / 1024;
     static_assert(!DOT || MTW == 1, "data-gradient mode: one M tile per wave");
     static constexpr int XPW = TEAM == 2 ? (PIECES + 1) / 2 : PIECES;
-    static constexpr int LPR = XPW + (DOT ? DPIECES : 0) + (FRB ? 2 : 0) + (INX ? 1 : 0);
+    static constexpr int LPR = XPW + (DOT ? DPIECES : 0) + (FRB ? 2 : 0) + (INX ? 1 : 0) + (RGBB ? 4 : 0);
     static constexpr int X_OFF = 0;
     static constexpr int XRING = NR * RB;
     static constexpr int N_OFF = (XRING + 1023) / 1024 * 1024;
@@ -104,13 +107,16 @@
     static constexpr int ERING = FRB ? 2 * DR * 512 : (INX ? DR * 1024 : 0);
     static_assert(!INX || (CIN == COUT && CIN >= 32), "block-input flavour: 32 -> 32, 64 -> 64");
     static_assert(!FRB || (CIN == 16 && COUT == 16 && TEAM == 1), "FromRGB reduction flavour: 16 -> 16");
-    static constexpr int T_OFF = E_OFF + TEAM * ERING;
+    static constexpr int G_OFF = E_OFF + TEAM * ERING;
+    static constexpr int GRING = RGBB ? NR * 1024 : 0;
+    static_assert(!RGBB || (CIN == 32 && COUT == 32 && TEAM == 1), "toRGB adjoint prologue: 32 -> 32");
+    static constexpr int T_OFF = G_OFF + TEAM * GRING;
     static constexpr int TBYTES = 32 * MTW * 16 * 4;
     static constexpr int DUMMY_OFF = T_OFF + TEAM * TBYTES;
     static constexpr int RGBX_OFF = DUMMY_OFF + (TEAM == 2 ? 1024 : 0);
     static constexpr int LDS_BYTES = RGBX_OFF + (RGB && TEAM == 2 ? 1024 : 0);
     static constexpr int NEED = 4 * 9 * KS * MTW + 32 * MTW + 16 + (ENC ? 16 * MTW : 0) + (STATS || DOT ? 32 * MTW : 0) + (DOT ? 16 : 0) + (PREP ? 16 : 0) + (RGB ? 11 : 0) + (POOL ? 20 * MTW : 0) + 36;
-    static constexpr int WPE = ((PREP || INB) && CIN == 64) ? 1 : (NEED <= 128 ? 4 : (NEED <= 168 ? 3 : 2));
+    static constexpr int WPE = (((PREP || INB) && CIN == 64) || RGBB) ? 1 : (NEED <= 128 ? 4 : (NEED <= 168 ? 3 : 2));
     static_assert(D <= NR - 3, "the slot of the row being fetched must be dead");
     static_assert((D - 1) * LPR + 1 < 64, "vmcnt range");
 };
@@ -184,6 +190,10 @@
     const unsigned evoff = C::INX ? (unsigned)(((x0 >> 1) + (lane >> 2)) * C::CPB + wave * 64 + (((lane & 3) ^ chunk_swz<2>(lane >> 2)) << 4))
                                   : (unsigned)((x0 >> 1) * 32 + (lane & 31) * 16);
     const unsigned ivoff = (unsigned)((x0 + (lane & 31)) * 16);
+    const unsigned grow_bytes = C::RGBB ? (unsigned)p.W * 4u : 0u;
+    const unsigned long long GIb = C::RGBB ? (unsigned long long)(p.rb_gimg + (size_t)b * 3 * p.H * p.W) : Xb;
+    const unsigned long long GNb = (C::RGBB && p.rb_noise) ? (unsigned long long)(p.rb_noise + (size_t)b * p.rb_noise_bstride) : 0ull;
+    const unsigned gvoff = lane < C::HW ? (unsigned)((x0 - 1 + lane) * 4) : 0x80000000u;
 
     unsigned long long xptr = Xb + (unsigned long long)(long long)(r0 - 1) * xrow_bytes;
     unsigned long long dptr = DOTb + (unsigned long long)(long long)(r0 - 2) * yrow_bytes;
@@ -199,6 +209,13 @@
             const rsrc_t rd = make_rsrc(dptr, ov ? yrow_bytes : 0u);
             dptr += yrow_bytes;
             dma_dot<C::DPIECES>(dvoff, dvoff1, rd, lds0 + C::D_OFF + wave * C::DRING + slot_d * C::DROWB);
+        }
+        if constexpr (C::RGBB) {
+            const unsigned long long ro = (unsigned long long)(xv ? gy : 0) * grow_bytes, plane = (unsigned long long)p.H * grow_bytes;
+            const unsigned m0g = lds0 + C::G_OFF + slot * 1024;
+#pragma unroll
+            for (int k = 0; k < 3; k++) dma_dword(gvoff, make_rsrc(GIb + k * plane + ro, xv ? grow_bytes : 0u), m0g + k * 256);
+            dma_dword(gvoff, make_rsrc(GNb ? GNb + ro : Xb, (xv && GNb) ? grow_bytes : 0u), m0g + 768);
         }
         if constexpr (C::INX) {
             const int oy = gy - 1;
@@ -405,6 +422,55 @@
     const float pns = (C::PREP && p.prep_noise && p.prep_ns) ? p.prep_ns[0] : 0.f;
     const float fr_es = (C::FRB || C::INX) ? p.in_extra_scale : 0.f;
 
+    constexpr int RBN = C::RGBB ? 8 : 1;
+    float rw0[RBN], rw1[RBN], rw2[RBN], rsv[RBN], rsg[RBN], rp0[RBN], rp1[RBN];
+    unsigned rxa[3] = {0, 0, 0}, rga[3] = {0, 0, 0};
+    const float rgpos = C::RGBB ? p.rb_gain : 1.f, rgneg = 0.2f * rgpos, rzpos = 1.f / rgpos, rzneg = 1.f / (0.2f * rgpos);
+    const float rns = (C::RGBB && p.rb_noise && p.rb_ns) ? p.rb_ns[0] : 0.f;
+    if constexpr (C::RGBB) {
+        const int rc = lane & 3, pq = lane >> 2;
+#pragma unroll
+        for (int e = 0; e < 8; e++) {
+            const int i = rc * 8 + e;
+            rw0[e] = p.rb_w[i] * p.rb_wscale; rw1[e] = p.rb_w[CIN + i] * p.rb_wscale; rw2[e] = p.rb_w[2 * CIN + i] * p.rb_wscale;
+            rsv[e] = p.rb_style[(size_t)b * CIN + i]; rsg[e] = 0.f; rp0[e] = 0.f; rp1[e] = 0.f;
+        }
+#pragma unroll
+        for (int j = 0; j < 3; j++) {
+            const int px = j == 0 ? 1 + pq : (j == 1 ? 17 + pq : ((pq & 1) ? C::HW - 1 : 0));
+            rxa[j] = lds0 + C::X_OFF + px * C::PXB + ((rc ^ chunk_swz<C::LOGCH>(px)) << 4);
+            rga[j] = lds0 + C::G_OFF + px * 4;
+        }
+    }
+    typedef __attribute__((address_space(3))) u32x4_t* lds_u4wp;
+    auto rb_pixel = [&](int j, int slot, bool sums) __attribute__((always_inline)) {
+        const unsigned xa = rxa[j] + (unsigned)slot * C::RB, ga = rga[j] + (unsigned)slot * 1024u;
+        const float g0 = lds_f(ga), g1 = lds_f(ga + 256), g2 = lds_f(ga + 512);
+        const float nzs = rns * lds_f(ga + 768);
+        float xv[8], out[8];
+        unpack16(lds_u4(xa), xv, (bf16_t*)nullptr);
+#pragma unroll
+        for (int e = 0; e < 8; e++) {
+            const float t = torgb_adj3(g0, g1, g2, rw0[e], rw1[e], rw2[e]);
+            const bool pos = xv[e] > 0.f;
+            const float gz = t * rsv[e] * (pos ? rgpos : rgneg);
+            if (sums) {
+                rsg[e] += t * xv[e];
+                const float zt = xv[e] * (pos ? rzpos : rzneg) - nzs;
+                rp0[e] = fmaf(gz, zt, rp0[e]); rp1[e] += gz;
+            }
+            out[e] = gz;
+        }
+        const uint4 o = pack16(out, (bf16_t*)nullptr);
+        u32x4_t ov4; ov4[0] = o.x; ov4[1] = o.y; ov4[2] = o.z; ov4[3] = o.w;
+        *(lds_u4wp)(size_t)xa = ov4;
+    };
+    auto rb_row = [&](int slot, bool own) __attribute__((always_inline)) {
+        rb_pixel(0, slot, own);
+        rb_pixel(1, slot, own);
+        if (lane < 8) rb_pixel(2, slot, false);
+    };
+
 #define DGE_T(k)
     auto step = [&](auto ic, int s, unsigned npar) {
         constexpr int I = decltype(ic)::value;
@@ -417,6 +483,10 @@
         DGE_T(1);
         if constexpr (C::NOISE && I == 0) issue_noise(s + C::NR, npar ^ 1024u);
         issue(s + 2 + C::D, (I + 2 + C::D) % C::NR, (I + C::D) % C::DR);
+        if constexpr (C::RGBB) {
+            rb_row((I + 2) % C::NR, s + 2 <= rows);
+            __builtin_amdgcn_sched_barrier(0);
+        }
         DGE_T(2);
 
         const int gy = r0 + s;
@@ -612,6 +682,12 @@
     const long long tj1 = __builtin_readcyclecounter();
     __builtin_amdgcn_sched_barrier(0);
 #endif
+    if constexpr (C::RGBB) {
+        asm volatile("s_waitcnt vmcnt(%0)" :: "i"(C::D * C::LPR) : "memory");
+        rb_row(0, false);
+        rb_row(1, true);
+        __builtin_amdgcn_sched_barrier(0);
+    }
     unsigned npar = 0;
     for (int s0_ = 0; s0_ < rows; s0_ += C::NR, npar ^= 1024u) {
         bool done = false;
@@ -636,6 +712,19 @@
     }
 #endif
 
+    if constexpr (C::RGBB) {
+        float vg = 0.f, vp = 0.f;
+#pragma unroll
+        for (int e = 0; e < 8; e++) {
+            float a = rsg[e], c0 = rp0[e], c1 = rp1[e];
+#pragma unroll
+            for (int m = 4; m < 64; m <<= 1) { a += __shfl_xor(a, m, 64); c0 += __shfl_xor(c0, m, 64); c1 += __shfl_xor(c1, m, 64); }
+            if (((lane >> 2) & 7) == e) { vg = a; vp = lane < 32 ? c0 : c1; }
+        }
+        const int ch = (lane & 3) * 8 + ((lane >> 2) & 7);
+        if (lane < 32) atomicAdd(p.rb_gs + (size_t)b * CIN + ch, vg);
+        atomicAdd(p.rb_stats + ((size_t)(blockIdx.x % p.stats_slots) * p.B + b) * CIN * 2 + ch * 2 + (lane < 32 ? 0 : 1), vp);
+    }
     if constexpr (C::FRB) {
         float va = 0.f, vc = 0.f;
 #pragma unroll
@@ -720,7 +809,7 @@
     const int njobs = p.B * nstrips * nseg;
     const int nwg = (njobs + C::TPW - 1) / C::TPW;
     const int jobs_per_xcd = (nwg + 7) / 8;
-    const char* fl = FL == FL_GEN ? "gen" : (FL == FL_ENC ? "enc" : (FL == FL_ENC_STATS ? "enc_stats" : (FL == FL_DOT ? "dot" : (FL == FL_DOT_PREP ? "dot_prep" : (FL == FL_GEN_RGB ? "gen_rgb" : (FL == FL_DOT_IN ? "dot_in" : (FL == FL_DOT_FR ? "dot_fromrgb" : (FL == FL_DOT_INX ? "dot_inx" : "enc_pool"))))))));
+    const char* fl = FL == FL_GEN ? "gen" : (FL == FL_ENC ? "enc" : (FL == FL_ENC_STATS ? "enc_stats" : (FL == FL_DOT ? "dot" : (FL == FL_DOT_PREP ? "dot_prep" : (FL == FL_GEN_RGB ? "gen_rgb" : (FL == FL_DOT_IN ? "dot_in" : (FL == FL_DOT_FR ? "dot_fromrgb" : (FL == FL_DOT_INX ? "dot_inx" : (FL == FL_DOT_PREP_RGB ? "dot_prep_rgb" : "enc_pool")))))))));
     dge_note_kernel("conv_stream<bf16,%d,%d,%s>", CIN, COUT, fl);
     hipLaunchKernelGGL(kern, dim3((unsigned)(jobs_per_xcd * 8)), dim3(64 * C::TEAM * C::TPW), C::LDS_BYTES * C::TPW, s, p, nstrips, nseg, seg_rows, njobs, jobs_per_xcd);
     DGE_LAUNCH_CHECK("conv_stream");
@@ -742,6 +831,11 @@
     if (p.in_coef) {
         if constexpr ((CIN == 32 && COUT == 16) || (CIN == 64 && COUT == 32)) return launch_stream<CIN, COUT, FL_DOT_IN>(p, s);
         dge_set_error("conv_stream: the instance-norm backward epilogue is built for 32 -> 16 and 64 -> 32 only");
+        return -1;
+    }
+    if (p.rb_gimg) {
+        if constexpr (CIN == 32 && COUT == 32) { if (p.dot_src && p.prep) return launch_stream<CIN, COUT, FL_DOT_PREP_RGB>(p, s); }
+        dge_set_error("conv_stream: the toRGB adjoint prologue is built for 32 -> 32 data-gradient launches with prep only");
         return -1;
     }
     if (p.dot_src) {
@@ -797,6 +891,11 @@
     if (p.noise && p.noise_w == nullptr) return false;
     if (dge_env().no_stream) return false;
     return true;
+}
+
+bool dge_conv_rgb_bwd_ok(const ConvParams& p, int dtype, int ksize) {
+    return p.Cin == 32 && p.Cout == 32 && p.dot_src && p.stats && p.prep && p.prep_stats && !p.in_coef && !p.rgb_out && !p.pool_out &&
+           dge_conv_stream_eligible(p, dtype, ksize);
 }
 
 bool dge_conv_pool_ok(const ConvParams& p, int dtype, int ksize) {
diff --git a/deep-gan-encoders_amd/csrc/s2_bwd_kernels.hip b/deep-gan-encoders_amd/csrc/s2_bwd_kernels.hip
--- a/deep-gan-encoders_amd/csrc/s2_bwd_kernels.hip
+++ b/deep-gan-encoders_amd/csrc/s2_bwd_kernels.hip
@@ -85,7 +85,7 @@
             unpack16(*(const uint4*)(x + o), xv, (T*)nullptr);
 #pragma unroll
             for (int e = 0; e < EP; e++) {
-                const float t = g0 * w0[e] + g1 * w1[e] + g2 * w2[e];
+                const float t = torgb_adj3(g0, g1, g2, w0[e], w1[e], w2[e]);
                 sg[0][e] += t * xv[e];
                 const bool pos = xv[e] > 0.f;
                 const float gz = t * sv[e] * (pos ? gpos : gneg);
diff --git a/deep-gan-encoders_amd/ops.py b/deep-gan-encoders_amd/ops.py
--- a/deep-gan-encoders_amd/ops.py
+++ b/deep-gan-encoders_amd/ops.py
@@ -321,7 +321,7 @@
 def conv2d(x, w_packed, cout, ksize=3, up=False, in_scale=None, in_shift=None, out_scale=None, bias=None,
            bias_scale=1.0, noise=None, noise_w=None, act=ACT_NONE, gain=1.0, addend=None, add_scale=1.0, stats=None,
            out=None, in_s2d=False, dot_src=None, in_up2=False, in_relu=False, prep=None, relu_mask=None, in_t2d=False, rgb=None, pool_out=False, pool_mask=False,
-           in_bwd=None):
+           in_bwd=None, rgb_bwd=None):
     B, H, W, Cin = x.shape
     if in_s2d:
         H, W, Cin = H // 2, W // 2, Cin * 4
@@ -408,6 +408,16 @@
         else:
             d.prep_noise = None
             d.in_bwd_extra, d.in_bwd_extra_scale = _p(in_bwd.get("extra")), float(in_bwd.get("extra_scale", 1.0))
+    if rgb_bwd is not None:
+        if prep is None:
+            raise DgeError("conv2d: rgb_bwd needs prep")
+        rn = rgb_bwd.get("noise")
+        rgb_bwd["gs"], rgb_bwd["P"] = zeros((B, Cin), x.device), SlotStats(B, Cin, x.device)
+        r = d.rgb_bwd
+        r.gimg, r.w, r.style, r.noise = _f32(rgb_bwd["gimg"]), _f32(rgb_bwd["w"]), _f32(rgb_bwd["style"]), _f32(rn)
+        r.ns, r.noise_batch = _f32(rgb_bwd.get("ns") if rn is not None else None), 1 if rn is None else rn.shape[0]
+        r.gs, r.stats = _f32(rgb_bwd["gs"]), _f32(rgb_bwd["P"].alloc(nslot))
+        r.wscale, r.gain = float(rgb_bwd["wscale"]), float(rgb_bwd["gain"])
     if rgb is not None:
         d.rgb_w, d.rgb_style, d.rgb_bias, d.rgb_out = _f32(rgb["w"]), _f32(rgb["style"]), _f32(rgb["bias"]), _f32(rgb["out"])
         d.rgb_wscale, d.rgb_skip_y = float(rgb["wscale"]), 1 if rgb.get("skip_y") else 0
@@ -433,6 +443,8 @@
         PROFILE.append((e0, e1, 2.0 * macs * B, (B, H, W, Cin, cout, ksize, up, in_s2d), abytes))
     else:
         check(lib().dge_conv2d(C.byref(d), _stream()), "dge_conv2d")
+    if KERNEL_LOG is not None:
+        KERNEL_LOG.append((last_kernel(), _stream()))
     if partial is not None and not lazy:
         check(lib().dge_sum_slots(_p(partial), _p(stats), nslot, stats.numel(), 1, _stream()), "dge_sum_slots")
     if rgb is not None and rgb.get("skip_y"):
@@ -657,6 +669,8 @@
     check(lib().dge_modconv_bwd_prep(_p(gx), _p(x), _f32(d), _f32(noise), _p(gy), _f32(R), B, H * W, Cc,
                                      1 if noise is None else noise.shape[0], float(gain), dtype_of(x), _stream()),
           "dge_modconv_bwd_prep")
+    if KERNEL_LOG is not None:
+        KERNEL_LOG.append(("modconv_bwd_prep_kernel", _stream()))
     return gy
 
 
@@ -668,6 +682,8 @@
     check(lib().dge_torgb_bwd_prep(_f32(gimg), _p(x), _f32(wrgb), _f32(style), _f32(noise), _f32(ns if noise is not None else None),
                                    1 if noise is None else noise.shape[0], _p(gz), _p(gs), _p(P), B, H * W, Cc, float(wscale),
                                    float(gain), dtype_of(x), _stream()), "dge_torgb_bwd_prep")
+    if KERNEL_LOG is not None:
+        KERNEL_LOG.append(("torgb_bwd_prep_kernel", _stream()))
     return gz, gs, P
 
 
@@ -880,6 +896,10 @@
     return bool(lib().dge_conv_rgb_supported(B, H, W, cin, cout, ksize, dtype))
 
 
+def conv_rgb_bwd_supported(B, H, W, cin, cout, ksize, dtype):
+    return bool(lib().dge_conv_rgb_bwd_supported(int(B), int(H), int(W), int(cin), int(cout), int(ksize), int(dtype)))
+
+
 def rgb_upsample_add(img, prev):
     B, Cc, H, W = img.shape
     check(lib().dge_rgb_upsample_add(_p(img), _f32(prev), B * Cc, H, W, _stream()), "dge_rgb_upsample_add")
diff --git a/include/dge_hip.h b/include/dge_hip.h
--- a/include/dge_hip.h
+++ b/include/dge_hip.h
@@ -73,6 +73,17 @@
     float in_bwd_extra_scale;
     const float* fr_img4;
     float* fr_out;
+    struct {
+        const float* gimg;
+        const float* w;
+        const float* style;
+        const float* noise;
+        const float* ns;
+        float* gs;
+        float* stats;
+        float wscale, gain;
+        int noise_batch;
+    } rgb_bwd;
 } dge_conv_desc;
 int dge_conv2d(const dge_conv_desc* d, dge_stream_t stream);
 int dge_conv_small_supported(int H, int W, int cin, int ntot, int ksize, int in_s2d, int in_up2, int dtype);
@@ -111,6 +122,7 @@
               int B, int H, int W, int cin, float wscale, int dtype, dge_stream_t stream);
 
 int dge_conv_rgb_supported(int B, int H, int W, int Cin, int Cout, int ksize, int dtype);
+int dge_conv_rgb_bwd_supported(int B, int H, int W, int Cin, int Cout, int ksize, int dtype);
 int dge_conv_in_bwd_supported(int B, int H, int W, int Cin, int Cout, int ksize, int dtype);
 int dge_conv_in_bwd_fromrgb_supported(int B, int H, int W, int Cin, int Cout, int ksize, int dtype);
 int dge_conv_in_bwd_x_supported(int B, int H, int W, int Cin, int Cout, int ksize, int dtype);
```
